# weiquan/salt

Measured on AMD Instinct MI355X. Metric: Mreads/s aligned (100 bp SE, GRCh38+snp144) at 1/2/4/8 MI355X vs CPU ref, higher is better.
Workload: dtype u32; 1 GPU; GRCh38-scale synthetic (SURVEY 8d config 3 = BASELINE configs[2]): 3100000000 bp genome in 24 contigs, 14800000 SNPs, k=21, 1000000 x 100 bp SE reads per GPU per step, 8 distinct resident batches rotated, inputs and results resident in HBM; read_len=100, distinct_batches=8, options=default (-s 50 -m 1000, overlap = k), streams_per_gpu=4

## Files before the change

include/salt_gpu.h:

```cpp
#ifndef SALT_GPU_H
#define SALT_GPU_H
#include <stdint.h>
#include <stddef.h>

#ifdef __cplusplus
extern "C" {
#endif

#define SALT_OK              0
#define SALT_E_INVAL        -1
#define SALT_E_HIP          -2
#define SALT_E_NOMEM        -3
#define SALT_E_INDEX        -4
#define SALT_E_CAPACITY     -5
#define SALT_E_DATA         -6

#define SALT_MAX_READ_LEN   512
#define SALT_MAX_HITS       5
#define SALT_MAX_LOCATE     1024
#define SALT_MAX_SEED_SLOTS 512
#define SALT_MAX_CIGAR_OPS  64

typedef struct {
    uint32_t c_primary, c_L2[5], c_seq_len, c_bwt_size;
// ... 80 lines not shown
int  salt_gpu_align_pe(salt_gpu_ws_t *ws, const salt_aln_opt_t *opt, const salt_pe_opt_t *pe, uint32_t n_pairs,
                       const uint8_t *seqs, const uint32_t *offs, salt_result_t *results);
int  salt_gpu_align_pe_resident(salt_gpu_ws_t *ws, const salt_aln_opt_t *opt, const salt_pe_opt_t *pe, uint32_t n_pairs,
                                uint32_t max_read_len, const void *d_seqs, const void *d_offs, void *d_results, void *hip_stream);
int  salt_gpu_ws_pe_overflow(salt_gpu_ws_t *ws, uint32_t *n);
int  salt_gpu_ws_pe_counts(salt_gpu_ws_t *ws, uint32_t out[8]);

int  salt_gpu_index_snp_enable(salt_gpu_index_t *ix, int on, uint32_t min_mapq);
int  salt_gpu_index_snp_sites(salt_gpu_index_t *ix, uint32_t *n_sites, uint32_t *pos, uint64_t cap);
int  salt_gpu_index_snp_counts(salt_gpu_index_t *ix, uint32_t *counts, uint64_t cap_words, int reset);
int  salt_gpu_ws_snp_uncount(salt_gpu_ws_t *ws);

typedef struct {
    uint32_t window;
    uint32_t tile_positions;
    int32_t  bgzf;
} salt_depth_text_opt_t;
int  salt_gpu_index_depth_enable(salt_gpu_index_t *ix, int on, uint32_t min_mapq);
int  salt_gpu_index_depth_reset(salt_gpu_index_t *ix);
int  salt_gpu_index_depth_fetch(salt_gpu_index_t *ix, uint64_t first, uint64_t n, uint32_t *out);
int  salt_gpu_index_depth_add(salt_gpu_index_t *ix, uint64_t first, uint64_t n, const uint32_t *in);
int  salt_gpu_index_depth_text_begin(salt_gpu_index_t *ix, const salt_depth_text_opt_t *opt);
int  salt_gpu_index_depth_text_next(salt_gpu_index_t *ix, const char **data, uint64_t *n_bytes);
int  salt_gpu_ws_depth_uncount(salt_gpu_ws_t *ws);

#define SALT_ERRPROF_Q      95
#define SALT_ERRPROF_CELLS  (2u * SALT_MAX_READ_LEN * SALT_ERRPROF_Q * 16u)
int  salt_gpu_index_errprof_enable(salt_gpu_index_t *ix, int on, uint32_t min_mapq);
int  salt_gpu_index_errprof_fetch(salt_gpu_index_t *ix, uint64_t *cells, uint64_t cap_cells, uint64_t rec[16], int reset);
int  salt_gpu_ws_errprof_uncount(salt_gpu_ws_t *ws);
int  salt_gpu_ws_set_quals(salt_gpu_ws_t *ws, const uint8_t *quals, int on_device);

typedef struct { int32_t print_xa_cigar, print_nm_md; const char *rg_id; } salt_text_opt_t;
int  salt_gpu_index_set_contigs(salt_gpu_index_t *ix, int32_t n, const int64_t *offsets, const char *const *names);
int  salt_gpu_align_pe_text(salt_gpu_ws_t *ws, const salt_aln_opt_t *opt, const salt_pe_opt_t *pe, const salt_text_opt_t *topt,
                            const char *fastq1, uint64_t n1_bytes, const char *fastq2, uint64_t n2_bytes,
                            const char **sam, uint64_t *sam_bytes, uint32_t *n_pairs);
int  salt_gpu_ws_reserve_text(salt_gpu_ws_t *ws, const salt_aln_opt_t *opt, uint64_t max_block_bytes, uint32_t est_reads, uint32_t max_read_len,
                              uint64_t est_sam_bytes, void *host_sam, uint64_t host_sam_bytes);
int  salt_gpu_align_se_text(salt_gpu_ws_t *ws, const salt_aln_opt_t *opt, const salt_text_opt_t *topt, const char *fastq, uint64_t n_bytes,
                            const char **sam, uint64_t *sam_bytes, uint32_t *n_reads);
int  salt_gpu_ws_set_sam_bgzf(salt_gpu_ws_t *ws, int on);
int  salt_gpu_ws_set_sam_bam(salt_gpu_ws_t *ws, int on);
int  salt_gpu_ws_set_polish(salt_gpu_ws_t *ws, int mode);
int  salt_gpu_bgzf_deflate(int device, const void *text, uint64_t n_bytes, void *out, uint64_t out_cap, uint64_t *out_bytes);
int  salt_gpu_bgzf_inflate(int device, const void *bgzf, uint64_t n_bytes, void *out, uint64_t out_cap, uint64_t *out_bytes);
int  salt_gpu_ws_inflate_bgzf(salt_gpu_ws_t *ws, const void *blocks, uint64_t n_cbytes, uint32_t n_blocks, const uint32_t *c_off, const uint32_t *u_off);
int  salt_gpu_ws_text_peek(salt_gpu_ws_t *ws, uint64_t off, uint64_t n, void *dst);
int  salt_gpu_align_se_text_dev(salt_gpu_ws_t *ws, const salt_aln_opt_t *opt, const salt_text_opt_t *topt, uint64_t off, uint64_t n_bytes, int add_newline,
                                const char **sam, uint64_t *sam_bytes, uint32_t *n_reads);
int  salt_gpu_host_alloc(uint64_t bytes, void **ptr);
void salt_gpu_host_free(void *ptr);
int  salt_gpu_device_numa_node(int device, int *node);
int  salt_gpu_device_count(int *n);

int  salt_gpu_align_se_resident(salt_gpu_ws_t *ws, const salt_aln_opt_t *opt, uint32_t n_reads,
                                uint32_t max_read_len, const void *d_seqs, const void *d_offs,
                                void *d_results, void *hip_stream);

#define SALT_N_KERNELS 10
int  salt_gpu_ws_timing(salt_gpu_ws_t *ws, int enable);
int  salt_gpu_ws_kernel_ms(salt_gpu_ws_t *ws, double ms[SALT_N_KERNELS], uint32_t *n_calls);

int  salt_gpu_ws_heavy_reads(salt_gpu_ws_t *ws, uint32_t *ids, uint32_t cap, uint32_t *n);

int  salt_gpu_buffer_alloc(int device, uint64_t bytes, void **dev_ptr);
int  salt_gpu_buffer_free(int device, void *dev_ptr);
int  salt_gpu_buffer_equal(int device, const void *a, const void *b, uint64_t bytes, int *equal);

int  salt_gpu_diag_rule(uint32_t n_cases, const uint32_t *pos, const uint8_t *val, const uint32_t *offs, const uint32_t *bound_in,
                        uint32_t L, uint32_t ref_len, int mode, uint32_t *out);

int  salt_gpu_diag_verify(const uint32_t *ref_words, uint32_t ref_len, uint32_t n_cases, const uint8_t *seqs, const uint32_t *offs,
                          const uint32_t *cand, const uint32_t *cand_offs, int mode, uint8_t *out);

int  salt_gpu_diag_occ(const salt_gpu_index_t *ix, int mode, uint32_t n, const uint32_t *queries, uint32_t *out);

int  salt_gpu_ws_queue_counts(salt_gpu_ws_t *ws, uint32_t out[8]);

int  salt_gpu_ws_counters(salt_gpu_ws_t *ws, uint64_t out[SALT_CTR_N]);

int  salt_gpu_diag_lv(const uint32_t *ref_words, uint32_t ref_len, uint32_t n_cases, const uint32_t *pos,
                      const uint32_t *kdiff, const uint8_t *seqs, const uint32_t *offs, int32_t *out4, uint16_t *cigars);

int  salt_gpu_diag_ssw(uint32_t n_cases, const uint8_t *aware, const uint8_t *ref_syms, const uint32_t *ref_offs,
                       const uint8_t *codes, const uint32_t *read_offs, int32_t *out6, uint16_t *cigars, uint16_t *n_cigar);

typedef struct { uint32_t read, offset, pool; uint16_t tlen; uint8_t strand, k; } salt_polish_item_t;
typedef struct salt_gpu_polish salt_gpu_polish_t;
int  salt_gpu_polish_open(int device, const uint8_t *pac, uint64_t l_pac, salt_gpu_polish_t **out);
void salt_gpu_polish_close(salt_gpu_polish_t *p);
int  salt_gpu_polish_lv(salt_gpu_polish_t *p, const uint8_t *codes, const uint32_t *offs, uint32_t n_reads, const salt_polish_item_t *items,
                        uint32_t n_items, const uint8_t *pool, uint32_t pool_stride, uint32_t n_pool, int want_cigar,
                        int32_t *dist, uint16_t *cigars, uint8_t *n_cigar);

int  salt_gpu_polish_sw(salt_gpu_polish_t *p, const uint8_t *codes, const uint32_t *offs, uint32_t n_reads, const salt_polish_item_t *items,
                        uint32_t n_items, int want_cigar, int32_t *score, int32_t *read_span, uint16_t *cigars, uint16_t *n_cigar);

int  salt_gpu_polish_set_contigs(salt_gpu_polish_t *p, int32_t n, const int64_t *offsets, const char *const *names);
typedef struct { int32_t paired, use_sw; } salt_polish_opt_t;
int  salt_gpu_polish_text(salt_gpu_polish_t *p, const salt_polish_opt_t *opt, const char *sam, uint64_t n_bytes,
                          const char **out, uint64_t *out_bytes, uint32_t *n_records, int *stopped);
int  salt_gpu_polish_text_stats(salt_gpu_polish_t *p, uint64_t out[8]);

int  salt_gpu_suffix_array(int device, const uint8_t *text, uint64_t n, int bits, uint32_t *sa_out);
uint64_t salt_gpu_idx_c_bwt_words(uint64_t n);
int  salt_gpu_idx_build_c(int device, const uint8_t *text, uint64_t n, uint32_t sa_intv, uint32_t *primary, uint32_t L2[5],
                          uint32_t *bwt, uint32_t *sa, uint32_t *lkt, uint32_t lkt_len);
int  salt_gpu_idx_build_r(int device, const uint8_t *rtext, uint64_t n, const uint32_t *sharp_off, const uint32_t *sharp_hdr, uint64_t n_sharp,
                          uint32_t cum4, uint32_t *inv_sa0, uint32_t *code, uint64_t code_words, uint32_t *rsa);
const char *salt_gpu_idx_last_error(void);

const char *salt_gpu_last_error(void);
uint32_t    salt_gpu_result_size(void);

#ifdef __cplusplus
}
#endif
#endif
```

salt_amd/csrc/salt_align.hip:

```cpp
#include <type_traits>
#include "salt_device.h"
#include "salt_kernels.h"

namespace salt {

#define WSYNC() do { __builtin_amdgcn_fence(__ATOMIC_ACQ_REL, "wavefront"); __builtin_amdgcn_wave_barrier(); \
                     __builtin_amdgcn_fence(__ATOMIC_ACQ_REL, "wavefront"); } while (0)

static constexpr int MAXL = SALT_MAX_READ_LEN;
static constexpr int SLOTS = SALT_MAX_SEED_SLOTS;
static constexpr int MAXLOC = SALT_MAX_LOCATE;
static constexpr int LVK = 31;
static_assert(offsetof(salt_result_t, strand) == 4 && offsetof(salt_result_t, mapq) == 7 && offsetof(salt_result_t, b0) == 8 &&
              offsetof(salt_result_t, b1) == 12 && offsetof(salt_result_t, seq_start) == 16 && offsetof(salt_result_t, seq_end) == 18 &&
              offsetof(salt_result_t, n_hits) == 20 && offsetof(salt_result_t, n_cigar) == 22 && offsetof(salt_result_t, skipped) == 23 &&
              offsetof(salt_result_t, hits) == 24 && sizeof(salt_hit_t) == 8, "salt_result_t header layout");
static constexpr int NHIT = 6;
__device__ __forceinline__ uint32_t mapq_quot(uint32_t x, uint32_t b0)
{
    const uint32_t v = 255u * x;
    return b0 == 1u ? v : b0 == 2u ? v / 2u : b0 == 3u ? v / 3u : v / b0;
}
static constexpr uint32_t INF = 255;

// ... 436 lines not shown
    if (pend_r) {
        uint4 *rec = wq + ((size_t)seg * wq_seg_cap + q_base[0] + at_r) * WQ_REC;
        rec[0] = make_uint4((uint32_t)item, pk_r, pl_r, cn0); rec[1] = make_uint4(cw0, cw1, cw2, cn1);
    }
    if (pend_c) {
        uint4 *rec = wq + (((size_t)WQ_SEG + seg) * wq_seg_cap + q_base[1] + at_c) * WQ_REC;
        rec[0] = make_uint4((uint32_t)item, pk_c, pl_c, cn0); rec[1] = make_uint4(cw0, cw1, cw2, cn1);
    }
    if (ctr) {
        for (int o = 32; o > 0; o >>= 1) {
            n_lkt += __shfl_down(n_lkt, o); n_occ_c += __shfl_down(n_occ_c, o); n_occ_r += __shfl_down(n_occ_r, o);
        }
        if (lane_id() == 0) {
            atomicAdd(ctr + SALT_CTR_LKT, n_lkt & 1023u); atomicAdd(ctr + SALT_CTR_OCC_C, n_occ_c); atomicAdd(ctr + SALT_CTR_OCC_R, n_occ_r);
            atomicAdd(ctr + SALT_CTR_D_WLKT, n_lkt & 1023u); atomicAdd(ctr + SALT_CTR_D_COCC_SEED, n_occ_c); atomicAdd(ctr + SALT_CTR_D_ROCC_SEED, n_occ_r);
            atomicAdd(ctr + SALT_CTR_D_SA_SEED, (n_lkt >> 10) & 2047u); atomicAdd(ctr + SALT_CTR_D_TEXT_SEED, n_lkt >> 21);
        }
    }
}

__global__ void __launch_bounds__(256) __attribute__((amdgpu_waves_per_eu(4, 4)))
k_seed_walk(IndexView ix, SeedParams sp, const uint32_t *__restrict__ tb, uint4 *__restrict__ sai_c, uint4 *__restrict__ sai_r,
            const uint4 *__restrict__ wq, const uint32_t *__restrict__ wq_cnt, uint32_t wq_seg_cap, uint32_t r_first, unsigned long long *__restrict__ ctr)
{
    const uint32_t seg = blockIdx.x & (WQ_SEG - 1u);
    const uint32_t wv = (blockIdx.x / WQ_SEG) * 4u + (uint32_t)__builtin_amdgcn_readfirstlane((int)(threadIdx.x >> 6)), nw = (gridDim.x / WQ_SEG) * 4u;
    const uint64_t lt = (1ull << lane_id()) - 1ull;
    const uint32_t la = r_first ? 0u : 1u, lb = la ^ 1u;
    const uint32_t na = wq_cnt[(la * WQ_SEG + seg) * WQ_STRIDE], nb = wq_cnt[(lb * WQ_SEG + seg) * WQ_STRIDE];
    const uint32_t a0 = (uint32_t)((uint64_t)na * wv / nw), a1 = (uint32_t)((uint64_t)na * (wv + 1u) / nw);
    const uint32_t b0 = (uint32_t)((uint64_t)nb * wv / nw), b1 = (uint32_t)((uint64_t)nb * (wv + 1u) / nw);
    const uint4 *qa = wq + (((size_t)la * WQ_SEG + seg) * wq_seg_cap + a0) * WQ_REC, *qb = wq + (((size_t)lb * WQ_SEG + seg) * wq_seg_cap + b0) * WQ_REC;
    const uint32_t tot_a = a1 - a0, tot = tot_a + (b1 - b0);
    const int i_top = (int)((uint32_t)sp.l_seed - ix.r_lkt_len) - 1;
    uint32_t n_aux = 0, n_sa = 0, n_text = 0, n_occ_c = 0, n_occ_r = 0;
    Walk w; w.ph = WK_IDLE; w.k = w.l = w.ext = w.p0 = 0; w.i = 0;
    SeedCtx c = seed_ctx_geom(sp, tb, 0, ix.r_lkt_len);
    uint32_t item = 0, cur = 0;
    bool is_r = false;
    const uint4 *qp = qa;
    for (;;) {
        const uint64_t idle = __ballot(w.ph == WK_IDLE);
        if (cur >= tot && idle == ~0ull) break;
        if (cur < tot) {
            const uint32_t t = cur + (uint32_t)__popcll(idle & lt);
            if (w.ph == WK_IDLE && t < tot) {
                const bool in_a = t < tot_a;
                qp = in_a ? qa + (size_t)t * WQ_REC : qb + (size_t)(t - tot_a) * WQ_REC; is_r = (in_a ? la : lb) == 0u; w.ph = WK_REC;
            }
            const uint32_t nx = cur + (uint32_t)__popcll(idle);
            cur = nx < tot ? nx : tot;
        }
        WalkReq q = walk_req_none();
        if (w.ph == WK_REC) { q.pa = qp; q.na = WQ_REC; }
        else if (w.ph != WK_IDLE) q = is_r ? seed_walk_issue<true>(ix, sp, c, w) : seed_walk_issue<false>(ix, sp, c, w);
        const WalkLoads ld = walk_fetch(q);
        bool done = false;
        uint4 row = make_uint4(1, 0, 0, 0);
        if (w.ph == WK_REC) {
            item = ld.a[0].x;
            c = seed_ctx_geom(sp, tb, item, ix.r_lkt_len);
            c.w0 = ld.a[1].x; c.w1 = ld.a[1].y; c.w2 = ld.a[1].z; c.n0 = ld.a[0].w; c.n1 = ld.a[1].w;
            done = is_r ? seed_walk_begin<true>(sp, c, ld.a[0].y, ld.a[0].z, i_top, w, row) : seed_walk_begin<false>(sp, c, ld.a[0].y, ld.a[0].z, i_top, w, row);
        } else if (w.ph != WK_IDLE) {
            done = is_r ? seed_walk_finish<true>(ix, sp, c, w, ld, row, n_occ_r, n_aux) : seed_walk_finish<false>(ix, sp, c, w, ld, row, n_occ_c, n_aux);
        }
        if (done && row.x <= row.y) { if (is_r) { row.w = sai_r_pack(sp.epoch, row.w); sai_r[item] = row; } else sai_c[item] = row; }
        n_sa += (n_aux >> 10) & 2047u; n_text += n_aux >> 21; n_aux = 0;
    }
    if (ctr) {
        for (int o = 32; o > 0; o >>= 1) { n_sa += __shfl_down(n_sa, o); n_text += __shfl_down(n_text, o); n_occ_c += __shfl_down(n_occ_c, o); n_occ_r += __shfl_down(n_occ_r, o); }
        if (lane_id() == 0) {
            atomicAdd(ctr + SALT_CTR_OCC_C, n_occ_c); atomicAdd(ctr + SALT_CTR_OCC_R, n_occ_r);
            atomicAdd(ctr + SALT_CTR_D_COCC_SEED, n_occ_c); atomicAdd(ctr + SALT_CTR_D_ROCC_SEED, n_occ_r);
            atomicAdd(ctr + SALT_CTR_D_SA_SEED, n_sa); atomicAdd(ctr + SALT_CTR_D_TEXT_SEED, n_text);
        }
    }
}

template <int NS> struct SaiListsT { uint32_t sp[2][NS], ep[2][NS], off[2][NS]; };
struct SaiLists { uint32_t *sp[2], *ep[2], *off[2]; };
template <int NS> __device__ __forceinline__ SaiLists sai_ref(SaiListsT<NS> &a) { return SaiLists{ { a.sp[0], a.sp[1] }, { a.ep[0], a.ep[1] }, { a.off[0], a.off[1] } }; }
struct LvTables { short L[LVK][64]; char A[LVK][64]; };
static constexpr int LLV_K = 12;
static constexpr int LLV_TW = 22;
static constexpr int LLV_N = 64;
static constexpr int LLV_WIN = 4;
static constexpr int LLV_TS = LLV_TW + 2;
static constexpr int LLV_PW = LLV_TW;
static_assert(((8 * (LLV_TW - 1) - LLV_WIN + LLV_K) >> 3) + 2 <= LLV_TS, "text words of the longest window at the widest bound");
static_assert(((8 * (LLV_TW - 1) - LLV_WIN) >> 3) + 2 <= LLV_PW, "pattern words of the longest read");
struct LaneLv { uint32_t T[LLV_TS * LLV_N]; uint32_t P[LLV_PW]; };
struct LvBytes { uint8_t T[MAXL + 4 + 64]; uint8_t P[MAXL + 64]; };
template <int NS, bool LLV>
struct WaveLdsT {
    static constexpr bool HAS_LLV = LLV;
    static constexpr int N_SLOTS = NS;
    uint32_t pm[2][MAXL / 8];
    union U { SaiListsT<NS> sai; typename std::conditional<LLV, LaneLv, uint32_t>::type llv; LvBytes lvb; } u;
    uint8_t  cand_e[MAXLOC];
    uint32_t loci[MAXLOC];
    uint32_t hit_pos[2][NHIT];
    uint8_t  hit_nd[2][NHIT], hit_gap[2][NHIT];
    uint16_t cig[SALT_MAX_CIGAR_OPS];
    int      n_cig;
    alignas(8) uint8_t cargs[128];
};
typedef WaveLdsT<SLOTS, true> WaveLds;
typedef WaveLdsT<32, false> WaveLdsSmall;
typedef WaveLdsT<1, false> WaveLdsCigar;

struct Sai { uint32_t sp, ep, off; };
__device__ __forceinline__ Sai sai_get(const SaiLists &s, int w, int i) { return Sai{ s.sp[w][i], s.ep[w][i], s.off[w][i] }; }
__device__ __forceinline__ void sai_set(SaiLists &s, int w, int i, Sai v) { s.sp[w][i] = v.sp; s.ep[w][i] = v.ep; s.off[w][i] = v.off; }
__device__ __forceinline__ bool sai_ltv(Sai a, Sai b) { return a.ep - a.sp < b.ep - b.sp; }
__device__ __forceinline__ bool sai_lt(const SaiLists &s, int w, int i, int j) { return sai_ltv(sai_get(s, w, i), sai_get(s, w, j)); }
__device__ __forceinline__ void sai_swap(SaiLists &s, int w, int i, int j) { Sai a = sai_get(s, w, i), b = sai_get(s, w, j); sai_set(s, w, i, b); sai_set(s, w, j, a); }

__device__ void sai_insertsort(SaiLists &s, int w, int lo, int hi)
{
    for (int i = lo + 1; i < hi; ++i)
        for (int j = i; j > lo && sai_lt(s, w, j, j - 1); --j) sai_swap(s, w, j, j - 1);
}

__device__ void sai_combsort(SaiLists &s, int w, int base, int n)
{
    const double shrink = 1.2473309501039786540366528676643;
    int gap = n; bool do_swap;
    do {
        if (gap > 2) { gap = (int)(gap / shrink); if (gap == 9 || gap == 10) gap = 11; }
        do_swap = false;
        for (int i = 0; i < n - gap; ++i)
            if (sai_lt(s, w, base + i + gap, base + i)) { sai_swap(s, w, base + i, base + i + gap); do_swap = true; }
    } while (do_swap || gap > 2);
    if (gap != 1) sai_insertsort(s, w, base, base + n);
}

__device__ __attribute__((noinline)) void sai_introsort(SaiLists &s, int w, int n)
{
    if (n < 1) return;
    if (n == 2) { if (sai_lt(s, w, 1, 0)) sai_swap(s, w, 0, 1); return; }
    int d; for (d = 2; (1 << d) < n; ++d) { }
    d <<= 1;
    int st_l[24], st_r[24], st_d[24], top = 0;
    int lo = 0, hi = n - 1;
    for (;;) {
        if (lo < hi) {
            if (--d == 0) { sai_combsort(s, w, lo, hi - lo + 1); hi = lo; continue; }
            int i = lo, j = hi, k = i + ((j - i) >> 1) + 1;
            if (sai_lt(s, w, k, i)) { if (sai_lt(s, w, k, j)) k = j; }
            else k = sai_lt(s, w, j, i) ? i : j;
            Sai rp = sai_get(s, w, k);
            if (k != hi) sai_swap(s, w, k, hi);
            for (;;) {
                do ++i; while (sai_ltv(sai_get(s, w, i), rp));
                do --j; while (i <= j && sai_ltv(rp, sai_get(s, w, j)));
                if (j <= i) break;
                sai_swap(s, w, i, j);
            }
            sai_swap(s, w, i, hi);
            if (i - lo > hi - i) {
                if (i - lo > 16 && top < 24) { st_l[top] = lo; st_r[top] = i - 1; st_d[top] = d; ++top; }
                lo = hi - i > 16 ? i + 1 : hi;
            } else {
                if (hi - i > 16 && top < 24) { st_l[top] = i + 1; st_r[top] = hi; st_d[top] = d; ++top; }
                hi = i - lo > 16 ? i - 1 : lo;
            }
        } else {
            if (top == 0) { sai_insertsort(s, w, 0, n); return; }
            --top; lo = st_l[top]; hi = st_r[top]; d = st_d[top];
        }
    }
}

__device__ void sort_loci(uint32_t *a, uint32_t n)
{
// ... 313 lines not shown
                if (k == q) c = b + bit;
                mm &= mm - 1;
            }
            m = mm;
            const bool act = c != 0xFFFFFFFFu;
            uint32_t pos = act ? cand[c] : 0u;
            if (pos >= ref_len) pos = 0xFFFFFFFFu;
            u32x4_a4 x = { 0u, 0u, 0u, 0u };
            if (act && need && pos != 0xFFFFFFFFu) x = *reinterpret_cast<const u32x4_a4 *>(ref + (pos >> 3) + 4 * sub);
            const uint32_t mism = quad_mismatch<8>(x, pos, pmw, nvalid);
            if (act && sub == 0) out[c] = (uint8_t)((mism > 3 || pos == 0xFFFFFFFFu) ? INF : mism);
        }
    }
}

__device__ __forceinline__ uint32_t popc(uint32_t m) { return (uint32_t)__popc(m); }
__device__ __forceinline__ uint32_t popc(uint64_t m) { return (uint32_t)__popcll(m); }
__device__ __forceinline__ int first_bit(uint32_t m) { return __ffs((int)m) - 1; }
__device__ __forceinline__ int first_bit(uint64_t m) { return __ffsll((long long)m) - 1; }
template <int GW> struct LaneGroup {
    static_assert(GW == 64 || GW == 32 || GW == 16, "a wave, half of one or a quarter");
    typedef std::conditional_t<GW == 64, uint64_t, uint32_t> mask_t;
    static __device__ __forceinline__ uint32_t lane() { return lane_id() & (uint32_t)(GW - 1); }
    static __device__ __forceinline__ mask_t ballot(bool x)
    {
        const uint64_t m = __ballot(x);
        if constexpr (GW == 64) return m;
        else {
            const uint32_t h = (lane_id() & 32u) ? (uint32_t)(m >> 32) : (uint32_t)m;
            if constexpr (GW == 32) return h; else return (h >> (lane_id() & 16u)) & 0xFFFFu;
        }
    }
    static __device__ __forceinline__ uint32_t bcast(uint32_t v, int src)
    {
        if constexpr (GW == 64) return (uint32_t)__builtin_amdgcn_readlane((int)v, src);
        else return (uint32_t)__shfl((int)v, (int)(lane_id() & (uint32_t)(64 - GW)) + src);
    }
    static __device__ __forceinline__ mask_t below() { return ((mask_t)1 << lane()) - (mask_t)1; }
    static __device__ __forceinline__ uint32_t sum(uint32_t v)
    {
        for (int o = GW / 2; o > 0; o >>= 1) v += (uint32_t)__shfl_xor((int)v, o);
        return v;
    }
};

template <int LN = 4, int GW = 64>
__device__ __forceinline__ void verify_quads_2(const uint32_t *__restrict__ ref, uint32_t ref_len, const uint32_t *pm0, const uint32_t *pm1, uint32_t L,
                                               const uint32_t *c0, uint32_t n0, const uint32_t *c1, uint32_t n1, uint8_t *o0, uint8_t *o1)
{
    constexpr uint32_t CPW = (uint32_t)GW / LN;
    const uint32_t lane = LaneGroup<GW>::lane(), sub = lane & (uint32_t)(LN - 1), q = lane / (uint32_t)LN;
    const uint32_t nw = (L + 7) >> 3, n = n0 + n1;
    const uint32_t nvalid = L > 32u * sub ? (L - 32u * sub < 32u ? L - 32u * sub : 32u) : 0u;
    const bool behind = LN == 8 && GW == 32 && !(4u * sub < nw + 1u);
    uint32_t pa[4], pb[4];
#pragma unroll
    for (int t = 0; t < 4; ++t) { const bool in = (4 * sub + t) < nw; pa[t] = in ? pm0[4 * sub + t] : 0u; pb[t] = in ? pm1[4 * sub + t] : 0u; }
    for (uint32_t b = 0; b < n; b += 4u * CPW) {
        uint32_t pos[4]; u32x4_a4 x[4]; bool act[4], rev[4];
#pragma unroll
        for (int g = 0; g < 4; ++g) {
            if (b + CPW * g >= n) break;
            const uint32_t c = b + CPW * g + q;
            act[g] = c < n; rev[g] = c >= n0;
            pos[g] = act[g] ? (rev[g] ? c1[c - n0] : c0[c]) : 0u;
            if (pos[g] >= ref_len) pos[g] = 0xFFFFFFFFu;
            if (behind) x[g] = u32x4_a4{ 0u, 0u, 0u, 0u };
            else x[g] = *reinterpret_cast<const u32x4_a4 *>(ref + ((pos[g] == 0xFFFFFFFFu ? 0u : pos[g]) >> 3) + 4 * sub);
        }
#pragma unroll
        for (int g = 0; g < 4; ++g) {
            if (b + CPW * g >= n) break;
            const uint32_t pw[4] = { rev[g] ? pb[0] : pa[0], rev[g] ? pb[1] : pa[1], rev[g] ? pb[2] : pa[2], rev[g] ? pb[3] : pa[3] };
            const uint32_t mism = quad_mismatch<LN>(x[g], pos[g], pw, nvalid);
            if (act[g] && sub == 0) {
                const uint32_t c = b + CPW * g + q;
                const uint8_t v = (uint8_t)((mism > 3 || pos[g] == 0xFFFFFFFFu) ? INF : mism);
                if (rev[g]) o1[c - n0] = v; else o0[c] = v;
            }
        }
    }
}

__device__ __attribute__((noinline)) int lv_wave(const uint8_t *T, int tlen, const uint8_t *P, int plen, int k, LvTables *tab, int &d_fin)
{
    const int lane = (int)lane_id();
    const int d = lane - 31;
    const int ad = d < 0 ? -d : d;
    int Lprev = -2;
    const int end0 = plen < tlen ? plen : tlen;
    if (d == 0) { int i = 0; while (i < end0 && (P[i] & T[i]) != 0) ++i; Lprev = i; }
    const int r0 = __shfl(Lprev, 31);
    if (tab) tab->L[0][lane] = (short)Lprev;
    d_fin = 0;
    if (r0 == end0) return plen > end0 ? plen - end0 : 0;
    if (k > LVK - 1) k = LVK - 1;
    for (int e = 1; e <= k; ++e) {
        int left = __shfl_up(Lprev, 1), right = __shfl_down(Lprev, 1);
        if (lane == 0) left = -2;
        if (lane == 63) right = -2;
        const bool active = ad <= e && ad <= LVK - 1;
        int best = Lprev + 1; char act = 'X';
        if (left > best) { best = left; act = 'D'; }
        if (right + 1 > best) { best = right + 1; act = 'I'; }
        int cur = -2;
        if (active) {
            if (P[best] == T[d + best]) {
                int end = plen < tlen - d ? plen : tlen - d;
                if (best >= end) best = end;
                else { int i = best; while (i < end && (P[i] & T[d + i]) != 0) ++i; best = i; }
            }
            cur = best;
        }
        if (tab) { tab->L[e][lane] = (short)cur; tab->A[e][lane] = act; }
        uint64_t reach = __ballot(active && cur == plen);
        if (reach) {
            if (tab) {
                int rank = d == 0 ? 0 : (d < 0 ? 2 * ad - 1 : 2 * ad);
                int my = (active && cur == plen) ? rank : 1000;
                for (int o = 32; o > 0; o >>= 1) { int t = __shfl_xor(my, o); my = t < my ? t : my; }
                d_fin = my == 0 ? 0 : ((my & 1) ? -((my + 1) >> 1) : (my >> 1));
            }
            return e;
        }
        Lprev = cur;
    }
    return -1;
}

__device__ __attribute__((noinline)) uint32_t lv_lanes(LaneLv &s, const uint32_t *pm, int plen, int tlen, int k, bool active)
{
    constexpr int LLV_W = 2 * LLV_K + 1;
    const int lane = (int)lane_id() & (LLV_N - 1);
    const lds_u32 T = as_lds(s.T) + lane, P = as_lds(pm);
    auto fetch = [&](int i, int t, uint32_t &p, uint32_t &x) {
        const lds_u32 pp = P + (i >> 3), tt = T + (t >> 3) * LLV_N;
        const uint32_t p0 = pp[0], p1 = pp[1], t0 = tt[0], t1 = tt[LLV_N];
        p = __funnelshift_r(p0, p1, 4u * (uint32_t)(i & 7));
        x = __funnelshift_r(t0, t1, 4u * (uint32_t)(t & 7));
    };
    auto run_of = [](uint32_t p, uint32_t x) -> int {
        const uint32_t y = p & x;
        const uint32_t z = ~(((y & 0x77777777u) + 0x77777777u) | y) & 0x88888888u;
        return z ? __builtin_ctz(z) >> 2 : 8;
    };
    auto reach = [&](int d, int best, bool gated) -> int {
        uint32_t p, x;
        fetch(best, d + best, p, x);
        const int end = plen < tlen - d ? plen : tlen - d;
        const bool open = !gated || ((p ^ x) & 15u) == 0;
        int run = run_of(p, x), i = best + run;
        if (open && run == 8) while (i < end) { fetch(i, d + i, p, x); run = run_of(p, x); i += run; if (run < 8) break; }
        i = i < end ? i : end;
        return open ? i : best;
    };
    int row[LLV_W];
#pragma unroll
    for (int j = 0; j < LLV_W; ++j) row[j] = -2;
    const int end0 = plen < tlen ? plen : tlen;
    uint32_t result = 255;
    bool done = !active;
    if (active) {
        const int i = reach(0, 0, false);
        row[LLV_K] = i;
        if (i == end0) { result = (uint32_t)(plen > end0 ? plen - end0 : 0); done = true; }
    }
    for (int e = 1; e <= k; ++e) {
        if (__ballot(!done) == 0) break;
        int carry = -2;
#pragma unroll
        for (int d = -LLV_K; d <= LLV_K; ++d) {
            if ((d < 0 ? -d : d) > e) continue;
            const int mid = row[d + LLV_K], right = d < LLV_K ? row[d + LLV_K + 1] : -2;
            int best = mid + 1;
            if (carry > best) best = carry;
            if (right + 1 > best) best = right + 1;
            carry = mid;
            if (!done) {
                best = reach(d, best, true);
                if (best == plen) { result = (uint32_t)e; done = true; }
                else row[d + LLV_K] = best;
            }
        }
    }
    return result;
}

template <int VMAX, bool GAPF>
__device__ __forceinline__ void rule_unsorted(const uint32_t *pos, const uint8_t *val, const uint32_t n, const uint32_t L, const uint32_t ref_len,
                                              uint32_t &bound, bool &any, uint32_t &best_pos, uint32_t &best_v,
                                              uint32_t &n_hits, uint32_t &a0, uint32_t *hit_pos, uint8_t *hit_nd)
{
    const uint32_t lane = lane_id();
    const uint32_t NONE = 0xFFFFFFFFu;
    auto in_range = [&](uint32_t p) -> bool { return GAPF ? !(p + L + 4 >= ref_len) : p < ref_len; };
    uint32_t mp[VMAX + 1];
#pragma unroll
    for (int t = 0; t <= VMAX; ++t) mp[t] = NONE;
    uint32_t my_p = 0, my_v = NONE, n_p = 0;
    for (uint32_t b = 0; b < n; b += 64) {
        const uint32_t i = b + lane;
        uint32_t p = 0, v = NONE;
        if (i < n) { p = pos[i]; v = val[i]; }
        const bool in = i < n && v <= bound && in_range(p);
        if (in) {
#pragma unroll
            for (int t = 0; t <= VMAX; ++t) if (v == (uint32_t)t && p < mp[t]) mp[t] = p;
        }
        uint64_t m = __ballot(in);
        if (m && n_p <= 64u) {
            if (n_p + (uint32_t)__popcll(m) > 64u) n_p = 65u;
            else
                while (m) {
                    const int l = __ffsll((long long)m) - 1;
                    const uint32_t pl = (uint32_t)__builtin_amdgcn_readlane((int)p, l), vl = (uint32_t)__builtin_amdgcn_readlane((int)v, l);
                    if (lane == n_p) { my_p = pl; my_v = vl; }
                    ++n_p; m &= m - 1;
                }
        }
    }
#pragma unroll
    for (int t = 0; t <= VMAX; ++t)
        for (int o = 32; o > 0; o >>= 1) { const uint32_t x = (uint32_t)__shfl_xor((int)mp[t], o); mp[t] = x < mp[t] ? x : mp[t]; }
    uint32_t before[VMAX + 1];
    before[0] = NONE;
#pragma unroll
    for (int t = 1; t <= VMAX; ++t) before[t] = mp[t - 1] < before[t - 1] ? mp[t - 1] : before[t - 1];
    any = false; n_hits = 0;
#pragma unroll
    for (int t = VMAX; t >= 0; --t) if (mp[t] != NONE) { any = true; best_v = (uint32_t)t; best_pos = mp[t]; }
    if (!any) return;
    unsigned long long last = 0;
    const bool in_lanes = n_p <= 64u;
    unsigned long long my_key = ~0ull;
    if (in_lanes && lane < n_p) {
        uint32_t lim = NONE;
#pragma unroll
        for (int t = 1; t <= VMAX; ++t) if (my_v == (uint32_t)t) lim = before[t];
        if (my_p < lim) my_key = ((unsigned long long)my_p << 8) | my_v;
    }
    for (uint32_t h = 0; h < (uint32_t)NHIT; ++h) {
        unsigned long long cur = ~0ull;
        if (in_lanes) { if (h == 0 || my_key > last) cur = my_key; }
        else
        for (uint32_t b = 0; b < n; b += 64) {
            const uint32_t i = b + lane;
            if (i < n) {
                const uint32_t p = pos[i], v = val[i];
                if (v <= bound && in_range(p)) {
                    uint32_t lim = NONE;
#pragma unroll
                    for (int t = 1; t <= VMAX; ++t) if (v == (uint32_t)t) lim = before[t];
                    const unsigned long long key = ((unsigned long long)p << 8) | v;
                    if (p < lim && (h == 0 || key > last) && key < cur) cur = key;
                }
            }
        }
        for (int o = 32; o > 0; o >>= 1) {
            const unsigned long long x = ((unsigned long long)(uint32_t)__shfl_xor((int)(cur >> 32), o) << 32) | (uint32_t)__shfl_xor((int)(uint32_t)cur, o);
            cur = x < cur ? x : cur;
        }
        if (cur == ~0ull) break;
        if (lane == 0) { hit_pos[h] = (uint32_t)(cur >> 8); hit_nd[h] = (uint8_t)(cur & 255u); }
        if (h == 0) a0 = (uint32_t)(cur & 255u);
        last = cur; ++n_hits;
    }
    bound = best_v < bound ? best_v : bound;
}

template <int VMAX, bool GAPF, int GW = 64>
__device__ __forceinline__ void rule_sparse(const uint32_t *pos, const uint8_t *val, const uint32_t n, const uint32_t L, const uint32_t ref_len,
                                            uint32_t &bound, bool &any, uint32_t &best_pos, uint32_t &best_v,
                                            uint32_t &n_hits, uint32_t &a0, uint32_t *hit_pos, uint8_t *hit_nd)
{
    typedef LaneGroup<GW> G;
    typedef typename G::mask_t mask_t;
    const uint32_t lane = G::lane();
    const uint32_t NONE = 0xFFFFFFFFu;
    auto in_range = [&](uint32_t p) -> bool { return GAPF ? !(p + L + 4 >= ref_len) : p < ref_len; };
    any = false; n_hits = 0;
    if (n == 0) return;
    if (n <= (uint32_t)GW) {
        uint32_t p = 0, v = NONE;
        if (lane < n) { p = pos[lane]; v = val[lane]; }
        const bool ok = v <= bound && in_range(p);
        const mask_t m = G::ballot(ok);
        if (m == 0) return;
        const int l0 = first_bit(m);
        const uint32_t p0 = G::bcast(p, l0);
        if (G::ballot(ok && p != p0) == 0) {
            const uint32_t v0 = G::bcast(v, l0);
            any = true; best_pos = p0; best_v = v0; n_hits = 1; a0 = v0;
            if (lane == 0) { hit_pos[0] = p0; hit_nd[0] = (uint8_t)v0; }
            bound = v0 < bound ? v0 : bound;
            return;
        }
    }
    uint32_t mp[VMAX + 1];
#pragma unroll
    for (int t = 0; t <= VMAX; ++t) mp[t] = NONE;
    for (uint32_t b = 0; b < n; b += GW) {
        const uint32_t i = b + lane;
        uint32_t p = 0, v = NONE;
        if (i < n) { p = pos[i]; v = val[i]; }
        mask_t m = G::ballot(v <= bound && in_range(p));
        while (m) {
            const int l = first_bit(m);
            const uint32_t pl = G::bcast(p, l), vl = G::bcast(v, l);
#pragma unroll
            for (int t = 0; t <= VMAX; ++t) if (vl == (uint32_t)t && pl < mp[t]) mp[t] = pl;
            m &= m - 1;
        }
    }
    uint32_t before[VMAX + 1];
    before[0] = NONE;
#pragma unroll
    for (int t = 1; t <= VMAX; ++t) before[t] = mp[t - 1] < before[t - 1] ? mp[t - 1] : before[t - 1];
#pragma unroll
    for (int t = VMAX; t >= 0; --t) if (mp[t] != NONE) { any = true; best_v = (uint32_t)t; best_pos = mp[t]; }
    if (!any) return;
    uint32_t last_p = 0;
    for (uint32_t h = 0; h < (uint32_t)NHIT; ++h) {
        uint32_t cur_p = NONE, cur_v = 0;
        for (uint32_t b = 0; b < n; b += GW) {
            const uint32_t i = b + lane;
            uint32_t p = 0, v = NONE;
            if (i < n) { p = pos[i]; v = val[i]; }
            uint32_t lim = NONE;
#pragma unroll
            for (int t = 1; t <= VMAX; ++t) if (v == (uint32_t)t) lim = before[t];
            mask_t m = G::ballot(v <= bound && in_range(p) && p < lim && (h == 0 || p > last_p));
            while (m) {
                const int l = first_bit(m);
                const uint32_t pl = G::bcast(p, l);
                if (pl < cur_p) { cur_p = pl; cur_v = G::bcast(v, l); }
                m &= m - 1;
            }
        }
        if (cur_p == NONE) break;
        if (lane == 0) { hit_pos[h] = cur_p; hit_nd[h] = (uint8_t)cur_v; }
        if (h == 0) a0 = cur_v;
        last_p = cur_p; ++n_hits;
    }
    bound = best_v < bound ? best_v : bound;
}

template <class W>
__device__ void lv_unpack(const uint32_t *ref_generic, W &w, int strand, uint32_t L, uint32_t pos)
{
    const gp_u32 ref = as_global(ref_generic);
    const uint32_t tlen = L + 4;
    for (uint32_t i = lane_id(); i < tlen + 48; i += 64) {
        uint32_t p = pos + i;
        w.u.lvb.T[i] = i < tlen ? (uint8_t)((ref[p >> 3] >> (4 * (p & 7u))) & 15u) : (uint8_t)0;
    }
    for (uint32_t i = lane_id(); i < L + 48; i += 64) {
        w.u.lvb.P[i] = i < L ? (uint8_t)((w.pm[strand][i >> 3] >> (4 * (i & 7u))) & 15u) : (uint8_t)0;
    }
    WSYNC();
}

template <class W>
__device__ __attribute__((noinline)) void lv_cigar(const uint32_t *ref, W &w, LvTables *tabp, int strand, uint32_t L, uint32_t pos, int k)
{
    LvTables &tab = *tabp;
    lv_unpack(ref, w, strand, L, pos);
    int d_fin = 0;
    WSYNC();
    int e = lv_wave(w.u.lvb.T, (int)L + 4, w.u.lvb.P, (int)L, k, &tab, d_fin);
    __threadfence_block();
    WSYNC();
    if (lane_id() == 0) {
        int n = 0;
        uint16_t *cg = w.cig;
        if (e == 0) { cg[n++] = (uint16_t)((L << 4) | 0u); }
        else if (e > 0) {
            char act[LVK + 1]; int matched[LVK + 1];
            int cd = d_fin;
            for (int ce = e; ce >= 1; --ce) {
                char a = tab.A[ce][cd + 31];
                act[ce] = a;
                int cur = tab.L[ce][cd + 31];
                if (a == 'I') { matched[ce] = cur - tab.L[ce - 1][cd + 1 + 31] - 1; cd += 1; }
                else if (a == 'D') { matched[ce] = cur - tab.L[ce - 1][cd - 1 + 31]; cd -= 1; }
                else { matched[ce] = cur - tab.L[ce - 1][cd + 31] - 1; }
            }
            int acc = tab.L[0][31];
            int ce = 1;
            while (ce <= e) {
                char a = act[ce]; int cnt = 1;
                while (ce + 1 <= e && matched[ce] == 0 && act[ce + 1] == a) { ++cnt; ++ce; }
                if (a == 'X') acc += cnt;
                else {
                    if (acc != 0 && n < SALT_MAX_CIGAR_OPS) { cg[n++] = (uint16_t)((acc << 4) | 0); }
                    acc = 0;
                    if (n < SALT_MAX_CIGAR_OPS) cg[n++] = (uint16_t)((cnt << 4) | (a == 'I' ? 1 : 2));
                }
                if (matched[ce] > 0) acc += matched[ce];
                ++ce;
            }
            if (acc != 0 && n < SALT_MAX_CIGAR_OPS) cg[n++] = (uint16_t)((acc << 4) | 0);
        }
        w.n_cig = n;
    }
    WSYNC();
}

__device__ __forceinline__ void lane_text(const uint32_t *__restrict__ ref, uint32_t *T, uint32_t pos, uint32_t tl)
{
    const uint32_t w0 = pos >> 3, sh = (pos & 7u) * 4u, nwt = (tl + 7) >> 3, nst = ((tl - LLV_WIN + LLV_K) >> 3) + 2;
    uint32_t wv[LLV_TW + 1];
#pragma unroll
    for (int j = 0; j <= LLV_TW; ++j) wv[j] = (uint32_t)j <= nwt ? ref[w0 + (uint32_t)j] : 0u;
#pragma unroll
    for (int j = 0; j < LLV_TW; ++j) {
        uint32_t word = 0;
        if ((uint32_t)j < nwt) {
            word = __funnelshift_r(wv[j], wv[j + 1], sh);
            const uint32_t rem = tl - (uint32_t)j * 8;
            if (rem < 8) word &= (1u << (4 * rem)) - 1u;
        }
        if ((uint32_t)j < nst) T[j * LLV_N] = word;
    }
#pragma unroll
    for (int j = LLV_TW; j < LLV_TS; ++j) if ((uint32_t)j < nst) T[j * LLV_N] = 0u;
}
template <class F>
__device__ __forceinline__ void lane_pattern(uint32_t *P, uint32_t nw, uint32_t first, uint32_t step, F word)
{
    for (uint32_t j = first; j < (uint32_t)LLV_PW; j += step) P[j] = j < nw ? word(j) : 0u;
}

__device__ __forceinline__ uint32_t store_gap_list(const uint32_t *loci, uint32_t n, uint32_t L, uint32_t ref_len, uint32_t *__restrict__ dst)
{
    const uint32_t lane = lane_id();
    const uint64_t lt = (1ull << lane) - 1ull;
    uint32_t n_out = 0;
    for (uint32_t b = 0; b < n; b += 64) {
        const uint32_t i = b + lane;
        const uint32_t pos = i < n ? loci[i] : 0u;
        const bool keep = i < n && !(pos + L + 4 >= ref_len);
        const uint64_t m = __ballot(keep);
        if (keep) dst[n_out + (uint32_t)__popcll(m & lt)] = pos;
        n_out += (uint32_t)__popcll(m);
    }
    return n_out;
}

template <bool PE, bool GL, class W>
__device__ __forceinline__ void align_general(const IndexView ix, const AlignParams ap, W &w, const uint32_t r,
                              const uint32_t *__restrict__ pm,
                              const uint4 *__restrict__ sai_c, const uint4 *__restrict__ sai_r,
                              salt_result_t *__restrict__ results, unsigned long long *__restrict__ ctr,
                              unsigned long long *phase, LvTables *lvtab, const GapBufs g, uint32_t *pe_loci, uint8_t *pe_cand)
{
    const uint32_t lane = lane_id();
    const uint64_t lt = (1ull << lane) - 1ull;
    const uint32_t *rec = pm + (uint64_t)r * ap.pg.pm_stride;
    const uint32_t L = rec[2 * ap.pg.nw8];
    salt_result_t *out = results + r;
    uint32_t c_sa_c = 0, c_sa_r = 0, c_verify = 0, c_vwords = 0, c_lv = 0, c_loci = 0, c_ctx_rej = 0, c_ctx_rows = 0;
    PhaseClock pc(phase);
    const uint64_t rt0 = phase ? __builtin_amdgcn_s_memrealtime() : 0;
    constexpr bool glob = GL;
    uint32_t *loci = glob ? pe_loci : w.loci;
    uint8_t *cand_e = glob ? pe_cand : w.cand_e;
    const uint32_t loci_cap = PE ? PE_LOCI_CAP : (uint32_t)MAXLOC;

    const uint32_t nw = (L + 7) >> 3;
    uint32_t n_amb = 0;
    for (uint32_t t = lane; t < 2 * nw; t += 64) {
        const uint32_t s = t >= nw, j = s ? t - nw : t;
        const uint32_t word = rec[s * ap.pg.nw8 + j];
        w.pm[s][j] = word;
        if (!s) n_amb += (uint32_t)__popc(word & (word >> 1) & (word >> 2) & (word >> 3) & 0x11111111u);
    }
    if (ap.max_amb < L) { for (int o = 32; o > 0; o >>= 1) n_amb += (uint32_t)__shfl_xor((int)n_amb, o); }
    else n_amb = 0;
    WSYNC();
    uint32_t q_pos = 0xFFFFFFFFu; uint32_t q_strand = 3, q_ndiff = 255, q_gap = 255;
    const bool too_short = L < (uint32_t)ap.l_seed;
    if (n_amb > ap.max_amb) {
        if (lane == 0) {
            out->pos = q_pos; out->strand = 3; out->n_diff = 255; out->is_gap = 255; out->mapq = 0;
            out->b0 = -1; out->b1 = -1; out->seq_start = 0; out->seq_end = (uint16_t)(L - 1);
            out->n_hits[0] = out->n_hits[1] = 0; out->n_cigar = 0; out->skipped = 1;
        }
        return;
// ... 56 lines not shown
                    if (strand == 0 || ix.c_ctx != nullptr) {
                        WSYNC();
                        const CandStats cs = build_candidates_call<PE, GL>(CandArgs{ ix.c_sa, ix.r_pos, sai_c, sai_r, ix.ref_len, ap.spr, ap.max_locate, r, L, strand, true, phase, pe_loci, loci_cap, ap.pe, false, ap.epoch, nullptr, nullptr, 0 }, w);
                        if (glob) { loci = cs.in_lds ? w.loci : pe_loci; cand_e = cs.in_lds ? w.cand_e : pe_cand; }
                        c_sa_c += cs.n_sa_c; c_sa_r += cs.n_sa_r; c_loci += cs.n_loci;
                        n = cs.n_cand;
                    }
                    if (n > 1024u * LLV_N) { ok = false; break; }
                    uint32_t o = 0;
                    if (lane == 0) o = atomicAdd(&g.gctl->pool_used, n);
                    o = (uint32_t)__shfl((int)o, 0);
                    ok = (uint64_t)o + n <= g.pool;
                    if (ok) for (uint32_t i = lane; i < n; i += 64) g.gloci[o + i] = loci[i];
                    ns[strand] = n; off[strand] = o;
                }
                const uint32_t ch0 = ok ? (ns[0] + LLV_N - 1) / LLV_N : 0, ch1 = ok ? (ns[1] + LLV_N - 1) / LLV_N : 0;
                uint32_t base = 0;
                if (ok && lane == 0) base = atomicAdd(&g.gctl->gap_items, ch0 + ch1);
                base = (uint32_t)__shfl((int)base, 0);
                ok = ok && (uint64_t)base + ch0 + ch1 <= g.items_cap;
                if (lane == 0) {
                    g.gq[slot] = ok ? r : 0xFFFFFFFFu;
                    g.gn[2 * slot] = ok ? ns[0] : 0; g.gn[2 * slot + 1] = ok ? ns[1] : 0;
                    g.goff[2 * slot] = off[0]; g.goff[2 * slot + 1] = off[1];
                }
                if (ok) {
                    for (uint32_t c = lane; c < ch0 + ch1; c += 64) g.gitems[base + c] = (slot << 11) | (c >= ch0 ? (0x400u | (c - ch0)) : c);
                    if (ctr) {
                        for (int o2 = 32; o2 > 0; o2 >>= 1) c_vwords += __shfl_down(c_vwords, o2);
                        if (lane == 0) {
                            atomicAdd(ctr + SALT_CTR_SA_C, c_sa_c); atomicAdd(ctr + SALT_CTR_SA_R, c_sa_r);
                            atomicAdd(ctr + SALT_CTR_VERIFY, c_verify); atomicAdd(ctr + SALT_CTR_VERIFY_WORDS, c_vwords);
                            atomicAdd(ctr + SALT_CTR_LV, ns[0] + ns[1]); atomicAdd(ctr + SALT_CTR_READS, 1ull);
                            atomicAdd(ctr + SALT_CTR_BASES, L); atomicAdd(ctr + SALT_CTR_LOCI, c_loci);
                            atomicAdd(ctr + SALT_CTR_D_SA_HEAVY, c_sa_c + c_sa_r);
                            atomicAdd(ctr + SALT_CTR_D_VERIFY_HEAVY, c_verify * (L <= 248 ? 4u : (((L + 7) >> 3) + 4u) / 4u));
                            atomicAdd(ctr + SALT_CTR_D_OUT_HEAVY, 5u * (ns[0] + ns[1]) + 16u);
                            if (ix.c_ctx) { atomicAdd(ctr + SALT_CTR_D_CTX_ROWS, c_ctx_rows); atomicAdd(ctr + SALT_CTR_D_CTX_REJECTED, c_ctx_rej); }
                        }
                    }
                    return;
                }
                WSYNC();
            }
        }
        if constexpr (!W::HAS_LLV) {
            if (lanes_fit && n_cand_nogap > 0) {
                if (lane == 0) g.ovq[atomicAdd(&g.gctl->ovq_count, 1u)] = r;
                return;
            }
        }
        for (int strand = 0; strand < 2; ++strand) {
            pc.stamp(SALT_CTR_T_GAP);
            const CandStats cs = build_candidates_call<PE, GL>(CandArgs{ ix.c_sa, ix.r_pos, sai_c, sai_r, ix.ref_len, ap.spr, ap.max_locate, r, L, strand, true, phase, pe_loci, loci_cap, ap.pe, true, ap.epoch, nullptr, nullptr, 0 }, w);
            if (glob) { loci = cs.in_lds ? w.loci : pe_loci; cand_e = cs.in_lds ? w.cand_e : pe_cand; }
            pc.t = phase ? __builtin_amdgcn_s_memtime() : 0;
            const uint32_t n_cand = cs.n_cand; c_sa_c += cs.n_sa_c; c_sa_r += cs.n_sa_r; c_loci += cs.n_loci;
            bool any = false;
            const bool lanes_ok = lanes_fit && W::HAS_LLV;
            if constexpr (W::HAS_LLV) if (lanes_ok) {
                const int k0 = gap_k0;
                WSYNC();
                lane_pattern(w.u.llv.P, (L + 7) >> 3, lane, 64u, [&](uint32_t j) { return w.pm[strand][j]; });
                for (uint32_t b = 0; b < n_cand; b += LLV_N) {
                    WSYNC();
                    const uint32_t i = b + lane;
                    bool act = false;
                    if (lane < LLV_N && i < n_cand) {
                        const uint32_t pos = loci[i];
                        act = !(pos > ix.ref_len || pos + L + 4 > ix.ref_len);
                        if (act) lane_text(ix.ref, w.u.llv.T + lane, pos, L + 4);
                    }
                    const uint32_t e = lv_lanes(w.u.llv, w.u.llv.P, (int)L, (int)L + 4, k0, act);
                    if (lane < LLV_N && i < n_cand) cand_e[i] = (uint8_t)e;
                }
                WSYNC();
            }
            for (uint32_t i = 0; i < n_cand; ++i) {
                uint32_t pos = loci[i];
                int e = -1;
                if (lanes_ok) { const uint32_t ev = cand_e[i]; e = (ev != 255 && (int)ev <= maxd) ? (int)ev : -1; }
                else if (!(pos > ix.ref_len || pos + L + 4 > ix.ref_len)) {
                    lv_unpack(ix.ref, w, strand, L, pos);
                    int dd;
                    e = lv_wave(w.u.lvb.T, (int)L + 4, w.u.lvb.P, (int)L, maxd, nullptr, dd);
                    WSYNC();
                }
                ++c_lv;
                if (e >= 0) {
                    if (e < maxd || !any) { maxd = e; q_gap = 1; q_ndiff = (uint32_t)e; q_strand = (uint32_t)strand; q_pos = pos; }
                    if (n_hits_s[strand] < NHIT && lane == 0) {
                        uint32_t h = n_hits_s[strand];
                        w.hit_pos[strand][h] = pos; w.hit_nd[strand][h] = (uint8_t)e; w.hit_gap[strand][h] = 1;
                    }
                    if (n_hits_s[strand] == 0) a0[strand] = (uint32_t)e;
                    if (n_hits_s[strand] < NHIT) ++n_hits_s[strand];
                    any = true;
                }
            }
            found[strand] = any;
            WSYNC();
        }
    }
    WSYNC();
    pc.stamp(SALT_CTR_T_GAP);

    int b0 = (int)q_ndiff, b1 = 100000, tot = 0;
    uint32_t nh[2] = { 0, 0 };
    uint32_t sel_idx[2][SALT_MAX_HITS];
    for (int s = 0; s < 2 && tot < ap.max_hits; ++s) {
        for (uint32_t j = 0; j < n_hits_s[s]; ++j) {
            uint32_t p = w.hit_pos[s][j];
            if (p == 0xFFFFFFFFu || p == q_pos) continue;
            if (a0[s] <= q_ndiff) {
                if ((int)a0[s] <= b1) b1 = (int)a0[s];
                if (nh[s] < SALT_MAX_HITS) sel_idx[s][nh[s]] = j;
                ++nh[s]; ++tot;
            }
            if (tot == ap.max_hits) break;
        }
    }
    uint32_t mapq = 0;
    if (b0 != 0) {
        uint32_t x = (uint32_t)(b0 > b1 ? b0 - b1 : b1 - b0);
        uint64_t q = mapq_quot(x, (uint32_t)b0);
        mapq = q < 254 ? (uint32_t)q : 254u;
    }
    if (lane == 0) {
        out->pos = q_pos; out->strand = (uint8_t)q_strand; out->n_diff = (uint8_t)q_ndiff; out->is_gap = (uint8_t)q_gap;
        out->mapq = (uint8_t)mapq; out->b0 = b0; out->b1 = b1; out->seq_start = 0; out->seq_end = (uint16_t)(L - 1);
        out->n_hits[0] = (uint8_t)nh[0]; out->n_hits[1] = (uint8_t)nh[1]; out->skipped = 0;
        for (int s = 0; s < 2; ++s)
            for (uint32_t j = 0; j < nh[s]; ++j) {
                uint32_t h = sel_idx[s][j];
                out->hits[s][j].pos = w.hit_pos[s][h]; out->hits[s][j].n_diff = w.hit_nd[s][h];
                out->hits[s][j].is_gap = w.hit_gap[s][h]; out->hits[s][j].strand = (uint16_t)s;
            }
    }
    if (q_pos != 0xFFFFFFFFu) {
        if (q_gap) {
            lv_cigar(ix.ref, w, lvtab, (int)q_strand, L, q_pos, (int)q_ndiff);
            if (lane < (uint32_t)w.n_cig) out->cigar[lane] = w.cig[lane];
            if (lane == 0) out->n_cigar = (uint8_t)w.n_cig;
        } else if (lane == 0) { out->cigar[0] = (uint16_t)((L << 4) | 0u); out->n_cigar = 1; }
    } else if (lane == 0) out->n_cigar = 0;
    uint32_t hidx = 0;
    for (int s = 0; s < 2; ++s)
        for (uint32_t j = 0; j < nh[s]; ++j, ++hidx) {
            uint32_t h = sel_idx[s][j];
            if (w.hit_gap[s][h]) {
                WSYNC();
                lv_cigar(ix.ref, w, lvtab, s, L, w.hit_pos[s][h], (int)w.hit_nd[s][h]);
                if (lane < (uint32_t)w.n_cig) out->hit_cigar[hidx][lane] = w.cig[lane];
                if (lane == 0) out->hit_n_cigar[hidx] = (uint8_t)w.n_cig;
            } else if (lane == 0) out->hit_n_cigar[hidx] = 0;
        }

    pc.stamp(SALT_CTR_T_TAIL);
    if (phase) {
        const unsigned long long dt = (unsigned long long)(__builtin_amdgcn_s_memrealtime() - rt0);
        pc.add(SALT_CTR_X3, dt);
        if (ctr && lane == 0) atomicMax(ctr + SALT_CTR_MAX_HEAVY, (dt << 32) | r);
    }
    if (ctr) {
        for (int o = 32; o > 0; o >>= 1) c_vwords += __shfl_down(c_vwords, o);
        if (lane == 0) {
            atomicAdd(ctr + SALT_CTR_SA_C, c_sa_c); atomicAdd(ctr + SALT_CTR_SA_R, c_sa_r);
            atomicAdd(ctr + SALT_CTR_VERIFY, c_verify); atomicAdd(ctr + SALT_CTR_VERIFY_WORDS, c_vwords);
            atomicAdd(ctr + SALT_CTR_LV, c_lv); atomicAdd(ctr + SALT_CTR_READS, 1ull);
            atomicAdd(ctr + SALT_CTR_BASES, L); atomicAdd(ctr + SALT_CTR_LOCI, c_loci);
            atomicAdd(ctr + SALT_CTR_D_SA_HEAVY, c_sa_c + c_sa_r);
            atomicAdd(ctr + SALT_CTR_D_VERIFY_HEAVY, c_verify * (L <= 248 ? 4u : (((L + 7) >> 3) + 4u) / 4u));
            atomicAdd(ctr + SALT_CTR_D_OUT_HEAVY, 128u);
            if (ix.c_ctx) { atomicAdd(ctr + SALT_CTR_D_CTX_ROWS, c_ctx_rows); atomicAdd(ctr + SALT_CTR_D_CTX_REJECTED, c_ctx_rej); }
        }
    }
}

__device__ __forceinline__ uint32_t pop_ranged(QueueRange *ranges, const uint32_t which, const uint32_t n_items, uint32_t &seg, uint32_t &tried)
{
    while (tried < QUEUE_RANGES) {
        const uint32_t lo = (uint32_t)((uint64_t)n_items * seg / QUEUE_RANGES), hi = (uint32_t)((uint64_t)n_items * (seg + 1u) / QUEUE_RANGES);
        uint32_t *h = &ranges[seg].heads[which];
        if (lo < hi && __hip_atomic_load(h, __ATOMIC_RELAXED, __HIP_MEMORY_SCOPE_AGENT) < hi - lo) {
            const uint32_t k = atomicAdd(h, 1u);
            if (k < hi - lo) return lo + k;
        }
        seg = (seg + 1u) & (QUEUE_RANGES - 1u); ++tried;
    }
    return 0xFFFFFFFFu;
}
template <bool PE, bool GL, class W>
__device__ __forceinline__ void heavy_body(const IndexView &ix, const AlignParams &ap, const uint32_t *__restrict__ pm,
                                           const uint4 *__restrict__ sai_c, const uint4 *__restrict__ sai_r,
                                           salt_result_t *__restrict__ results, const uint32_t *__restrict__ queue,
                                           unsigned long long *__restrict__ ctr, LvTables *__restrict__ lvtab, const GapBufs g,
                                           uint8_t *__restrict__ pe_scr, const int overflow_pass)
{
    __shared__ W w;
    __shared__ uint32_t s_item;
    __shared__ unsigned long long s_phase[SALT_CTR_N];
    unsigned long long *phase = ctr ? s_phase : nullptr;
    if (ctr) { for (int i = threadIdx.x; i < SALT_CTR_N; i += 64) s_phase[i] = 0; }
    WSYNC();
    const uint32_t n_items = overflow_pass ? g.gctl->ovq_count : ap.all_heavy ? ap.n_reads : g.gctl->light_queued;
    uint32_t seg = blockIdx.x & (QUEUE_RANGES - 1u), tried = 0;
    for (;;) {
        if (threadIdx.x == 0) {
            uint32_t got = 0xFFFFFFFFu;
            if (overflow_pass) { got = atomicAdd(&g.gctl->ovq_head, 1u); if (got >= n_items) got = 0xFFFFFFFFu; }
            else got = pop_ranged(g.ranges, QueueRange::HEAVY, n_items, seg, tried);
            s_item = got;
        }
        WSYNC();
        const uint32_t it = s_item;
        WSYNC();
        if (it == 0xFFFFFFFFu) break;
        const uint32_t r = overflow_pass ? g.ovq[it] : ap.all_heavy ? it : queue[it];
        align_general<PE, GL>(ix, ap, w, r, pm, sai_c, sai_r, results, ctr, phase, lvtab + blockIdx.x, g,
                          pe_scr ? reinterpret_cast<uint32_t *>(pe_scr + (size_t)blockIdx.x * PE_LOCI_CAP * 5) : nullptr,
                          pe_scr ? pe_scr + (size_t)blockIdx.x * PE_LOCI_CAP * 5 + (size_t)PE_LOCI_CAP * 4 : nullptr);
        if (phase && threadIdx.x == 0) s_phase[SALT_CTR_HEAVY_READS] += 1;
        WSYNC();
    }
    if (phase) {
        WSYNC();
        for (int i = SALT_CTR_T_LOAD + (int)threadIdx.x; i < SALT_CTR_N; i += 64) if (s_phase[i]) atomicAdd(ctr + i, s_phase[i]);
    }
}

#ifndef SALT_HEAVY_WAVES
#define SALT_HEAVY_WAVES 4
#endif
#if SALT_HEAVY_WAVES > 0
#define HEAVY_OCC __attribute__((amdgpu_waves_per_eu(SALT_HEAVY_WAVES, SALT_HEAVY_WAVES)))
#else
#define HEAVY_OCC
#endif
#define HEAVY_KERNEL(NAME, PE, GL, LDS)                                                                                    \
__global__ void __launch_bounds__(64) HEAVY_OCC                                                                         \
NAME(IndexView ix, AlignParams ap, const uint32_t *__restrict__ pm,                                                     \
     const uint4 *__restrict__ sai_c, const uint4 *__restrict__ sai_r, salt_result_t *__restrict__ results,             \
     const uint32_t *__restrict__ queue, unsigned long long *__restrict__ ctr,                                          \
     LvTables *__restrict__ lvtab, GapBufs g, uint8_t *__restrict__ pe_scr, int overflow_pass)                          \
{ heavy_body<PE, GL, LDS>(ix, ap, pm, sai_c, sai_r, results, queue, ctr, lvtab, g, pe_scr, overflow_pass); }
HEAVY_KERNEL(k_heavy, false, false, WaveLdsSmall)
HEAVY_KERNEL(k_heavy_pe, true, true, WaveLdsSmall)
HEAVY_KERNEL(k_heavy_big, false, false, WaveLds)
HEAVY_KERNEL(k_heavy_pe_big, true, true, WaveLds)
HEAVY_KERNEL(k_heavy_glob, false, true, WaveLds)

__global__ void __launch_bounds__(64)
k_gap(IndexView ix, AlignParams ap, const uint32_t *__restrict__ pm, GapBufs g)
{
    __shared__ LaneLv s;
    __shared__ uint32_t s_item;
    const uint32_t lane = lane_id();
    const uint32_t n_items = g.gctl->gap_items < g.items_cap ? g.gctl->gap_items : g.items_cap;
    uint32_t seg = blockIdx.x & (QUEUE_RANGES - 1u), tried = 0;
    for (;;) {
        if (threadIdx.x == 0) s_item = pop_ranged(g.ranges, QueueRange::GAP, n_items, seg, tried);
        WSYNC();
        const uint32_t it = s_item;
        WSYNC();
        if (it == 0xFFFFFFFFu) break;
        const uint32_t item = g.gitems[it], slot = item >> 11, strand = (item >> 10) & 1u, chunk = item & 1023u;
        const uint32_t r = g.gq[slot];
        const uint32_t *rec = pm + (uint64_t)r * ap.pg.pm_stride;
        const uint32_t L = rec[2 * ap.pg.nw8], nw = (L + 7) >> 3;
        lane_pattern(s.P, nw, lane, 64u, [&](uint32_t j) { return rec[strand * ap.pg.nw8 + j]; });
        const uint32_t n = g.gn[2 * slot + strand], i = chunk * LLV_N + lane;
        const size_t row = g.goff[2 * slot + strand];
        bool act = false;
        if (lane < LLV_N && i < n) {
            const uint32_t pos = g.gloci[row + i];
            act = !(pos > ix.ref_len || pos + L + 4 > ix.ref_len);
            if (act) lane_text(ix.ref, s.T + lane, pos, L + 4);
        }
        WSYNC();
        const uint32_t e = lv_lanes(s, s.P, (int)L, (int)L + 4, ap.pe ? 3 : (int)(L / 10), act);
        if (lane < LLV_N && i < n) g.ge[row + i] = (uint8_t)e;
        WSYNC();
    }
}

struct FinLds { uint32_t hit_pos[2][NHIT]; uint8_t hit_nd[2][NHIT]; };
__global__ void __launch_bounds__(64)
k_gapfin(IndexView ix, AlignParams ap, const uint32_t *__restrict__ pm, salt_result_t *__restrict__ results, GapBufs g,
         unsigned long long *__restrict__ ctr)
{
    __shared__ FinLds w;
    __shared__ uint32_t s_item;
    const uint32_t lane = lane_id();
    const uint64_t lt = (1ull << lane) - 1ull;
    const uint32_t n_items = g.gctl->gap_slots < g.cap ? g.gctl->gap_slots : g.cap;
    uint32_t seg = blockIdx.x & (QUEUE_RANGES - 1u), tried = 0;
    for (;;) {
        if (threadIdx.x == 0) s_item = pop_ranged(g.ranges, QueueRange::GAPFIN, n_items, seg, tried);
        WSYNC();
        const uint32_t slot = s_item;
        WSYNC();
        if (slot == 0xFFFFFFFFu) break;
        const uint64_t rt0 = ctr ? __builtin_amdgcn_s_memrealtime() : 0;
        const uint32_t r = g.gq[slot];
        if (r == 0xFFFFFFFFu) continue;
        const uint32_t L = pm[(uint64_t)r * ap.pg.pm_stride + 2 * ap.pg.nw8];
        salt_result_t *out = results + r;
        uint32_t q_pos = 0xFFFFFFFFu, q_strand = 3, q_ndiff = 255, q_gap = 255;
        uint32_t bound = ap.pe ? 3u : L / 10;
        uint32_t n_hits_s[2] = { 0, 0 }, a0[2] = { 0, 0 };
        for (int strand = 0; strand < 2; ++strand) {
            const uint32_t n = g.gn[2 * slot + strand];
            const size_t row = g.goff[2 * slot + strand];
            bool any = false; uint32_t bp = 0, bv = 0;
            rule_unsorted<LLV_K, true>(g.gloci + row, g.ge + row, n, L, ix.ref_len, bound, any, bp, bv, n_hits_s[strand], a0[strand],
                                       w.hit_pos[strand], w.hit_nd[strand]);
            if (any) { q_pos = bp; q_ndiff = bv; q_gap = 1; q_strand = (uint32_t)strand; }
        }
        WSYNC();
        int b0 = (int)q_ndiff, b1 = 100000, tot = 0;
        uint32_t nh[2] = { 0, 0 };
        uint32_t sel_idx[2][SALT_MAX_HITS];
        for (int s = 0; s < 2 && tot < ap.max_hits; ++s)
            for (uint32_t j = 0; j < n_hits_s[s]; ++j) {
                const uint32_t p = w.hit_pos[s][j];
                if (p == 0xFFFFFFFFu || p == q_pos) continue;
                if (a0[s] <= q_ndiff) {
                    if ((int)a0[s] <= b1) b1 = (int)a0[s];
                    if (nh[s] < SALT_MAX_HITS) sel_idx[s][nh[s]] = j;
                    ++nh[s]; ++tot;
                }
                if (tot == ap.max_hits) break;
            }
        uint32_t mapq = 0;
        if (b0 != 0) {
            const uint32_t x = (uint32_t)(b0 > b1 ? b0 - b1 : b1 - b0);
            const uint64_t q = mapq_quot(x, (uint32_t)b0);
            mapq = q < 254 ? (uint32_t)q : 254u;
        }
        const uint32_t n_cig_items = q_pos != 0xFFFFFFFFu ? 1u + nh[0] + nh[1] : 0u;
        const uint32_t first_cig = ap.pe ? 1u : 0u;
        if (lane == 0) {
            out->pos = q_pos; out->strand = (uint8_t)q_strand; out->n_diff = (uint8_t)q_ndiff; out->is_gap = (uint8_t)q_gap;
            out->mapq = (uint8_t)mapq; out->b0 = b0; out->b1 = b1; out->seq_start = 0; out->seq_end = (uint16_t)(L - 1);
            out->n_hits[0] = (uint8_t)nh[0]; out->n_hits[1] = (uint8_t)nh[1]; out->skipped = 0; out->n_cigar = 0;
            for (int s = 0; s < 2; ++s)
                for (uint32_t j = 0; j < nh[s]; ++j) {
                    const uint32_t h = sel_idx[s][j];
                    out->hits[s][j].pos = w.hit_pos[s][h]; out->hits[s][j].n_diff = w.hit_nd[s][h];
                    out->hits[s][j].is_gap = 1; out->hits[s][j].strand = (uint16_t)s;
                }
            if (n_cig_items > first_cig) {
                const uint32_t base = atomicAdd(&g.gctl->cigar_items, n_cig_items - first_cig);
                for (uint32_t c = first_cig; c < n_cig_items; ++c) g.cq[base + c - first_cig] = (r << 3) | c;
            }
            if (ctr) atomicMax(ctr + SALT_CTR_MAX_GAPFIN, ((unsigned long long)(__builtin_amdgcn_s_memrealtime() - rt0) << 32) | r);
        }
        WSYNC();
    }
}

__global__ void __launch_bounds__(64)
k_cigar(IndexView ix, PackGeom pg, const uint32_t *__restrict__ pm, salt_result_t *__restrict__ results,
        const uint32_t *__restrict__ items, const uint32_t *__restrict__ count, uint32_t *__restrict__ head, uint32_t cap_items,
        LvTables *__restrict__ lvtab)
{
    __shared__ WaveLdsCigar w;
    __shared__ uint32_t s_item;
    const uint32_t lane = lane_id();
    const uint32_t n_items = *count < cap_items ? *count : cap_items;
    struct { PackGeom pg; } ap = { pg };
    bool first = true;
    for (;;) {
        if (threadIdx.x == 0) s_item = first ? blockIdx.x : sw_pull(head, 1u, gridDim.x, n_items);
        first = false;
        WSYNC();
        const uint32_t it = s_item;
        WSYNC();
        if (it >= n_items) break;
        const uint32_t item = items[it], which = item & 7u, r = item >> 3;
        salt_result_t *out = results + r;
        const uint32_t *rec = pm + (uint64_t)r * ap.pg.pm_stride;
        const uint32_t L = rec[2 * ap.pg.nw8];
        uint32_t strand, pos, k;
        if (which == 0) { strand = out->strand; pos = out->pos; k = out->n_diff; }
        else {
            const uint32_t h = which - 1, n0 = out->n_hits[0];
            strand = h >= n0; const uint32_t j = strand ? h - n0 : h;
            pos = out->hits[strand][j].pos; k = out->hits[strand][j].n_diff;
        }
        for (uint32_t t = lane; t < (L + 7) >> 3; t += 64) w.pm[strand][t] = rec[strand * ap.pg.nw8 + t];
        WSYNC();
        lv_cigar(ix.ref, w, lvtab + blockIdx.x, (int)strand, L, pos, (int)k);
        uint16_t *dst = which == 0 ? out->cigar : out->hit_cigar[which - 1];
        if (lane < (uint32_t)w.n_cig) dst[lane] = w.cig[lane];
        if (lane == 0) { if (which == 0) out->n_cigar = (uint8_t)w.n_cig; else out->hit_n_cigar[which - 1] = (uint8_t)w.n_cig; }
        WSYNC();
    }
}

__host__ __device__ __forceinline__ uint32_t qseg_cap(uint32_t n_reads) { return n_reads / QUEUE_RANGES + 8u; }
__device__ __forceinline__ void queue_push(uint32_t *__restrict__ qseg, QueueRange *__restrict__ ranges, uint32_t n_reads, uint32_t r)
{
    const uint32_t s = (r >> 2) & (QUEUE_RANGES - 1u);
    qseg[(size_t)s * qseg_cap(n_reads) + atomicAdd(&ranges[s].push, 1u)] = r;
}
__device__ __forceinline__ uint32_t *retry_segs(uint32_t *qseg, uint32_t n_reads) { return qseg + (size_t)QUEUE_RANGES * qseg_cap(n_reads); }
__device__ __forceinline__ void retry_push(uint32_t *__restrict__ qseg, QueueRange *__restrict__ ranges, uint32_t n_reads, uint32_t r)
{
    const uint32_t s = (r >> 2) & (QUEUE_RANGES - 1u);
    retry_segs(qseg, n_reads)[(size_t)s * qseg_cap(n_reads) + atomicAdd(&ranges[s].retry, 1u)] = r;
}
__global__ void __launch_bounds__(256)
k_queue_pack(const uint32_t *__restrict__ qseg, const QueueRange *__restrict__ ranges, uint32_t n_reads, uint32_t *__restrict__ queue, SeCtl *__restrict__ ctl)
{
    __shared__ uint32_t base_s, cnt_s;
    if (threadIdx.x == 0) {
        uint32_t base = 0, total = 0;
        for (uint32_t s = 0; s < QUEUE_RANGES; ++s) { const uint32_t c = ranges[s].push; if (s < blockIdx.x) base += c; total += c; }
        base_s = base; cnt_s = ranges[blockIdx.x].push;
        if (blockIdx.x == 0) ctl->light_queued = total;
    }
    __syncthreads();
    const uint32_t *src = qseg + (size_t)blockIdx.x * qseg_cap(n_reads);
    for (uint32_t i = threadIdx.x; i < cnt_s; i += 256) queue[base_s + i] = src[i];
}

static constexpr int LT_LOCI = 128;
static constexpr int LT_MAXL = 160;
static constexpr int L2_SLOTS = 8;
static constexpr int L4_SLOTS = 4;
#ifndef SALT_L4_ROWS
#define SALT_L4_ROWS 16
#endif
static constexpr int L4_ROWS = SALT_L4_ROWS;

template <int SLOTS, int PMW, int LOCI> struct LightRec {
    uint32_t pm[2][PMW];
    uint32_t sp[4][SLOTS], off[4][SLOTS];
    uint32_t pre[4][SLOTS + 1];
    uint32_t loci[2][LOCI];
    uint32_t hit_pos[2][NHIT];
    uint8_t  hit_nd[2][NHIT];
    uint8_t  val[2][LOCI];
};
template <int GW> using LightLds = LightRec<GW / 4, GW == 64 ? LT_MAXL / 8 : GW == 32 ? 32 : 16, GW == 16 ? 2 * L4_ROWS : LT_LOCI>;
static_assert(sizeof(LightLds<32>) == 1996 && 8 * sizeof(LightLds<16>) <= 4 * sizeof(LightLds<32>), "eight quarter records in the LDS of four half-wave ones");

template <int GW, int LN, bool INSTR>
__device__ __forceinline__ void light_read(const IndexView &ix, const AlignParams &ap, const uint32_t *__restrict__ pm,
                                           const uint4 *__restrict__ sai_c, const uint4 *__restrict__ sai_r, salt_result_t *__restrict__ results,
                                           uint32_t *__restrict__ queue , QueueRange *__restrict__ ranges,
                                           unsigned long long *__restrict__ ctr, LightLds<GW> &w, const uint32_t r)
{
    typedef LaneGroup<GW> G;
    typedef typename G::mask_t mask_t;
    constexpr uint32_t SLOTS = GW / 4, HALF = GW / 2;
    constexpr uint32_t LMAX = LN == 4 ? 120u : LN == 8 ? 248u : (uint32_t)LT_MAXL;
    static_assert(LMAX <= 8 * sizeof(w.pm[0]) / 4 && (LN != 0 || LMAX <= 248u), "the read fits the record and the window check");
    const uint32_t lane = G::lane();
    const mask_t lt = G::below();
    const uint32_t *rec = pm + (uint64_t)r * ap.pg.pm_stride;
    const uint32_t L = rec[2 * ap.pg.nw8];
    bool heavy = L > LMAX || L < (uint32_t)ap.l_seed || ap.spr > SLOTS || ap.max_locate < 2 * 64;
    uint32_t c_sa_c = 0, c_sa_r = 0, c_verify = 0, c_loci = 0;
    const bool prof = INSTR && ctr && (r & 127u) == 0;
    uint64_t tp = prof ? __builtin_amdgcn_s_memtime() : 0;
    auto stamp = [&](int slot) {
        if (!prof) return;
        const uint64_t n = __builtin_amdgcn_s_memtime();
        if (lane == 0) atomicAdd(ctr + slot, (unsigned long long)(n - tp));
        tp = n;
    };
    auto locate = [&](uint32_t l, uint32_t j, uint32_t of, uint32_t &p) -> bool {
        p = ((of >> 31) ? j : (l & 1) ? ix.r_pos[j] : ix.c_sa[j]) - (of & 0x7FFFFFFFu);
        return (l & 1) ? !(p > ix.ref_len || p + L > ix.ref_len) : !(p + L > ix.ref_len);
// ... 259 lines not shown
        if (m == rescued) continue;
        salt_result_t *q = res + 2 * p + m;
        const uint32_t L = pm[(uint64_t)(2 * p + m) * pg.pm_stride + 2 * pg.nw8];
        q->seq_start = 0; q->seq_end = (uint16_t)(L - 1);
        if (q->pos == 0xFFFFFFFFu) q->n_cigar = 0;
        else if (q->is_gap) { q->n_cigar = 0; citems[atomicAdd(ccount, 1u)] = ((2 * p + (uint32_t)m) << 3) | 0u; }
        else { q->cigar[0] = (uint16_t)((L << 4) | 0u); q->n_cigar = 1; }
    }
}

void launch_pe_final(const IndexView &ix, const PackGeom &pg, uint32_t n_pairs, const uint32_t *pm, salt_result_t *res, const PePair *pairs,
                     const PeSwRes *sw, void *lvtab, uint32_t *citems, PeCtl *ctl, uint32_t n_blocks, hipStream_t st)
{
    if (!n_pairs) return;
    hipLaunchKernelGGL(k_pe_final, dim3((n_pairs + 255) / 256), dim3(256), 0, st, pg, n_pairs, pm, res, pairs, sw, citems, &ctl->n_cigar);
    hipLaunchKernelGGL(k_cigar, dim3(n_blocks), dim3(64), 0, st, ix, pg, pm, res, citems, &ctl->n_cigar, &ctl->cigar_head, 2 * n_pairs, static_cast<LvTables *>(lvtab));
}

uint32_t seed_wq_seg_cap(uint64_t items) { return (uint32_t)(((items + 255) / 256 + WQ_SEG - 1) / WQ_SEG) * 256u; }
size_t seed_wq_words(uint64_t items) { return (size_t)2 * WQ_SEG * seed_wq_seg_cap(items) * WQ_REC * 4; }
uint32_t seed_wq_cnt_words() { return 2u * WQ_SEG * WQ_STRIDE; }
void launch_seed(const IndexView &ix, const SeedParams &sp, const uint32_t *tb, uint4 *sai_c, uint4 *sai_r, uint4 *wq, uint32_t *wq_cnt,
                 uint32_t walk_blocks, unsigned long long *ctr, hipStream_t st)
{
    uint64_t items = (uint64_t)sp.n_reads * 2u * sp.spr;
    if (!items) return;
    uint32_t blocks = (uint32_t)((items + 255) / 256);
    const uint32_t cap = seed_wq_seg_cap(items);
    hipLaunchKernelGGL(k_seed, dim3(blocks), dim3(256), 0, st, ix, sp, tb, sai_c, sai_r, wq, wq_cnt, cap, ctr);
    walk_blocks = (walk_blocks + WQ_SEG - 1) / WQ_SEG * WQ_SEG;
    static const uint32_t r_first = getenv("SALT_GPU_WALK_R_FIRST") && atoi(getenv("SALT_GPU_WALK_R_FIRST")) ? 1u : 0u;
    hipLaunchKernelGGL(k_seed_walk, dim3(walk_blocks), dim3(256), 0, st, ix, sp, tb, sai_c, sai_r, wq, wq_cnt, cap, r_first, ctr);
}

void launch_light(const IndexView &ix, const AlignParams &ap, const uint32_t *pm, const uint8_t *, const uint32_t *, const uint4 *sai_c,
                  const uint4 *sai_r, salt_result_t *results, uint32_t *queue, SeCtl *ctl, uint32_t *qseg, QueueRange *ranges, unsigned long long *ctr, hipStream_t st)
{
    if (!ap.n_reads) return;
    static const bool no_half = getenv("SALT_GPU_NO_LIGHT2") && atoi(getenv("SALT_GPU_NO_LIGHT2"));
    static const bool no_quarter = getenv("SALT_GPU_NO_LIGHT4") && atoi(getenv("SALT_GPU_NO_LIGHT4"));
    if (!no_half && !no_quarter && !ctr && !SALT_DIAG_VAL(ap.dbg_stop) && ap.spr <= (uint32_t)L4_SLOTS && ap.pg.nw8 <= 15) {
        static const int wv = getenv("SALT_GPU_L4_WAVES") ? atoi(getenv("SALT_GPU_L4_WAVES")) : 2;
        if (wv == 1) hipLaunchKernelGGL(k_light4<1>, dim3((ap.n_reads + 3) / 4), dim3(64), 0, st, ix, ap, pm, sai_c, sai_r, results, qseg, ranges);
        else if (wv == 4) hipLaunchKernelGGL(k_light4<4>, dim3((ap.n_reads + 15) / 16), dim3(256), 0, st, ix, ap, pm, sai_c, sai_r, results, qseg, ranges);
        else hipLaunchKernelGGL(k_light4<2>, dim3((ap.n_reads + 7) / 8), dim3(128), 0, st, ix, ap, pm, sai_c, sai_r, results, qseg, ranges);
        static const uint32_t retry_blocks = [] {
            int dev = 0, cus = 0, per_cu = getenv("SALT_GPU_L4_RETRY_PER_CU") ? atoi(getenv("SALT_GPU_L4_RETRY_PER_CU")) : 8;
            if (hipGetDevice(&dev) != hipSuccess || hipDeviceGetAttribute(&cus, hipDeviceAttributeMultiprocessorCount, dev) != hipSuccess || cus <= 0) cus = (int)QUEUE_RANGES;
            if (per_cu < 1 || per_cu > 64) per_cu = 8;
            return ((uint32_t)(cus * per_cu) + QUEUE_RANGES - 1u) / QUEUE_RANGES * QUEUE_RANGES;
        }();
        hipLaunchKernelGGL(k_light_retry, dim3(retry_blocks), dim3(128), 0, st, ix, ap, pm, sai_c, sai_r, results, qseg, ranges);
    } else if (!no_half && !ctr && !SALT_DIAG_VAL(ap.dbg_stop) && ap.spr <= (uint32_t)L2_SLOTS && ap.pg.nw8 <= 31) {
        static const int wv = getenv("SALT_GPU_L2_WAVES") ? atoi(getenv("SALT_GPU_L2_WAVES")) : 2;
        if (ap.pg.nw8 > 15) hipLaunchKernelGGL((k_light2<2, 8>), dim3((ap.n_reads + 3) / 4), dim3(128), 0, st, ix, ap, pm, sai_c, sai_r, results, qseg, ranges);
        else if (wv == 1) hipLaunchKernelGGL(k_light2<1>, dim3((ap.n_reads + 1) / 2), dim3(64), 0, st, ix, ap, pm, sai_c, sai_r, results, qseg, ranges);
        else hipLaunchKernelGGL(k_light2<2>, dim3((ap.n_reads + 3) / 4), dim3(128), 0, st, ix, ap, pm, sai_c, sai_r, results, qseg, ranges);
    } else
        hipLaunchKernelGGL(k_light, dim3((ap.n_reads + LT_WAVES - 1) / LT_WAVES), dim3(64 * LT_WAVES), 0, st, ix, ap, pm, sai_c, sai_r, results, qseg, ranges, ctr);
    hipLaunchKernelGGL(k_queue_pack, dim3(QUEUE_RANGES), dim3(256), 0, st, qseg, ranges, ap.n_reads, queue, ctl);
}
size_t queue_words(uint32_t max_reads) { return (size_t)max_reads * 2 + (size_t)2 * QUEUE_RANGES * qseg_cap(max_reads); }

__global__ void __launch_bounds__(64)
k_diag_rule(uint32_t n_cases, const uint32_t *__restrict__ pos, const uint8_t *__restrict__ val, const uint32_t *__restrict__ offs,
            const uint32_t *__restrict__ bound_in, uint32_t L, uint32_t ref_len, int mode, uint32_t *__restrict__ out)
{
    __shared__ uint32_t hit_pos_s[4][NHIT];
    __shared__ uint8_t hit_nd_s[4][NHIT];
    const uint32_t gw = mode == 3 ? 32u : mode == 4 ? 16u : 64u, half = lane_id() / gw, lane = lane_id() & (gw - 1u);
    const uint32_t c = (64u / gw) * blockIdx.x + half;
    if (c >= n_cases) return;
    uint32_t *hit_pos = hit_pos_s[half];
    uint8_t *hit_nd = hit_nd_s[half];
    const uint32_t o = offs[c], n = offs[c + 1] - o;
    uint32_t bound = bound_in[c], bp = 0, bv = 0, nh = 0, a0 = 0;
    bool any = false;
    if (lane < NHIT) { hit_pos[lane] = 0; hit_nd[lane] = 0; }
    WSYNC();
    if (mode == 0) rule_unsorted<3, false>(pos + o, val + o, n, L, ref_len, bound, any, bp, bv, nh, a0, hit_pos, hit_nd);
    else if (mode == 1) rule_sparse<3, false>(pos + o, val + o, n, L, ref_len, bound, any, bp, bv, nh, a0, hit_pos, hit_nd);
    else if (mode == 3) rule_sparse<3, false, 32>(pos + o, val + o, n, L, ref_len, bound, any, bp, bv, nh, a0, hit_pos, hit_nd);
    else if (mode == 4) rule_sparse<3, false, 16>(pos + o, val + o, n, L, ref_len, bound, any, bp, bv, nh, a0, hit_pos, hit_nd);
    else rule_unsorted<LLV_K, true>(pos + o, val + o, n, L, ref_len, bound, any, bp, bv, nh, a0, hit_pos, hit_nd);
    WSYNC();
    uint32_t *w = out + (size_t)c * (6 + 2 * NHIT);
    if (lane == 0) { w[0] = any; w[1] = any ? bp : 0; w[2] = any ? bv : 0; w[3] = nh; w[4] = nh ? a0 : 0; w[5] = bound; }
    if (lane < NHIT) { w[6 + 2 * lane] = lane < nh ? hit_pos[lane] : 0; w[7 + 2 * lane] = lane < nh ? hit_nd[lane] : 0; }
}

void launch_diag_rule(uint32_t n_cases, const uint32_t *pos, const uint8_t *val, const uint32_t *offs, const uint32_t *bound_in,
                      uint32_t L, uint32_t ref_len, int mode, uint32_t *out, hipStream_t st)
{
    const uint32_t blocks = mode == 3 ? (n_cases + 1) / 2 : mode == 4 ? (n_cases + 3) / 4 : n_cases;
    if (n_cases) hipLaunchKernelGGL(k_diag_rule, dim3(blocks), dim3(64), 0, st, n_cases, pos, val, offs, bound_in, L, ref_len, mode, out);
}
uint32_t diag_rule_words() { return 6 + 2 * NHIT; }

__host__ __device__ static inline bool lv_fit_dev(uint32_t L, uint32_t k) { return k <= (uint32_t)LLV_K && L + 4 <= 8u * (LLV_TW - 1); }
bool lv_lanes_fit(uint32_t L, uint32_t k) { return lv_fit_dev(L, k); }

__global__ void __launch_bounds__(64)
k_diag_lv(IndexView ix, uint32_t n_cases, const uint32_t *__restrict__ pos, const uint32_t *__restrict__ kdiff,
          const uint8_t *__restrict__ seqs, const uint32_t *__restrict__ offs, const uint32_t *__restrict__ lane_first,
          const uint32_t *__restrict__ lane_n, const uint32_t *__restrict__ lane_case, int32_t *__restrict__ out ,
          uint16_t *__restrict__ cig_out , LvTables *__restrict__ lvtab)
{
    __shared__ WaveLds w;
    __shared__ uint32_t lane_pm[LLV_N][LLV_PW];
    const uint32_t c = blockIdx.x, lane = lane_id();
    if (c >= n_cases) return;
    const uint32_t off = offs[c], L = offs[c + 1] - off, p = pos[c];
    const uint32_t nw = (L + 7) >> 3;
    auto pm_word = [&](uint32_t o, uint32_t j) -> uint32_t {
        uint32_t word = 0;
        for (uint32_t q = 0; q < 8; ++q) {
            uint32_t i = j * 8 + q, cc = i < L ? seqs[o + i] : 5u;
            word |= (cc < 4 ? (1u << cc) : (cc == 4 ? 15u : 0u)) << (4 * q);
        }
        return word;
    };
    for (uint32_t j = lane; j < nw; j += 64) w.pm[0][j] = pm_word(off, j);
    WSYNC();
    int32_t v = -2, e_wave = -1, n_cig = -2;
    if (p + L <= ix.ref_len) v = (int32_t)mismatch_capped(ix, w.pm[0], L, p);
    const bool in_range = !(p > ix.ref_len || p + L + 4 > ix.ref_len);
    const int k = (int)kdiff[c];
    if (in_range) {
        lv_unpack(ix.ref, w, 0, L, p);
        int dd;
        e_wave = lv_wave(w.u.lvb.T, (int)L + 4, w.u.lvb.P, (int)L, k, nullptr, dd);
        WSYNC();
    }
    const bool fit = lv_fit_dev(L, (uint32_t)k);
    const uint32_t gn = fit ? lane_n[c] : 0u;
    if (gn) {
        const uint32_t m = lane_case[lane_first[c] + lane % gn], mo = offs[m], mp = pos[m];
        lane_pattern(lane_pm[lane], nw, 0u, 1u, [&](uint32_t j) { return pm_word(mo, j); });
        const bool act = !(mp > ix.ref_len || mp + L + 4 > ix.ref_len);
        if (act) lane_text(ix.ref, w.u.llv.T + lane, mp, L + 4);
        WSYNC();
        const uint32_t el = lv_lanes(w.u.llv, lane_pm[lane], (int)L, (int)L + 4, k, act);
        if (lane < gn) out[(size_t)m * 4 + 2] = el == 255 ? -1 : (int32_t)el;
        WSYNC();
    }
    if (in_range && e_wave >= 0 && e_wave < LVK) {
        lv_cigar(ix.ref, w, lvtab + blockIdx.x, 0, L, p, e_wave);
        n_cig = w.n_cig;
        if (lane < (uint32_t)w.n_cig) cig_out[(size_t)c * SALT_MAX_CIGAR_OPS + lane] = w.cig[lane];
    }
    if (lane == 0) {
        out[(size_t)c * 4 + 0] = v; out[(size_t)c * 4 + 1] = e_wave; out[(size_t)c * 4 + 3] = n_cig;
        if (!fit) out[(size_t)c * 4 + 2] = -2;
    }
}

size_t lv_table_bytes() { return sizeof(LvTables); }

void launch_diag_lv(const IndexView &ix, uint32_t n, const uint32_t *pos, const uint32_t *kdiff, const uint8_t *seqs,
                    const uint32_t *offs, const uint32_t *lane_first, const uint32_t *lane_n, const uint32_t *lane_case,
                    int32_t *out, uint16_t *cig, void *lvtab, hipStream_t st)
{
    if (n) hipLaunchKernelGGL(k_diag_lv, dim3(n), dim3(64), 0, st, ix, n, pos, kdiff, seqs, offs, lane_first, lane_n, lane_case, out, cig,
                              static_cast<LvTables *>(lvtab));
}

__global__ void __launch_bounds__(64)
k_diag_verify(const uint32_t *__restrict__ ref, uint32_t ref_len, uint32_t n_cases, const uint8_t *__restrict__ seqs, const uint32_t *__restrict__ offs,
              const uint32_t *__restrict__ cand, const uint32_t *__restrict__ coffs, int mode, uint8_t *__restrict__ out)
{
    __shared__ uint32_t pm_s[4][64];
    __shared__ uint32_t loci_s[4][256];
    __shared__ uint8_t val_s[4][256];
    const uint32_t gw = mode == 7 ? 16u : mode >= 5 ? 32u : 64u, half = lane_id() / gw, lane = lane_id() & (gw - 1u);
    const uint32_t c = (64u / gw) * blockIdx.x + half;
    if (c >= n_cases) return;
    uint32_t *pm = pm_s[half], *loci = loci_s[half];
    uint8_t *val = val_s[half];
    const uint32_t off = offs[c], L = offs[c + 1] - off, c0 = coffs[c];
    uint32_t n = coffs[c + 1] - c0;
    if (n > 256) n = 256;
    const uint32_t nw = (L + 7) >> 3;
    for (uint32_t j = lane; j < 64; j += gw) {
        uint32_t word = 0;
        for (uint32_t q = 0; q < 8 && j < nw; ++q) {
            const uint32_t i = j * 8 + q, cc = i < L ? seqs[off + i] : 5u;
            word |= (cc < 4 ? (1u << cc) : (cc == 4 ? 15u : 0u)) << (4 * q);
        }
        pm[j] = word;
    }
    for (uint32_t i = lane; i < n; i += gw) { loci[i] = cand[c0 + i]; val[i] = 77; }
    WSYNC();
    IndexView ix; ix.ref = ref; ix.ref_len = ref_len;
    if (mode == 0) { for (uint32_t i = lane; i < n; i += 64) val[i] = (uint8_t)mismatch_capped(ix, pm, L, loci[i]); }
    else if (mode == 1) verify_quads<8>(ref, ref_len, pm, L, loci, n, val);
    else if (mode == 2) verify_quads<8, 8>(ref, ref_len, pm, L, loci, n, val);
    else if (mode == 3) verify_quads_2(ref, ref_len, pm, pm, L, loci, n / 2, loci + n / 2, n - n / 2, val, val + n / 2);
    else if (mode == 4) verify_quads_2<8>(ref, ref_len, pm, pm, L, loci, n / 2, loci + n / 2, n - n / 2, val, val + n / 2);
    else if (mode == 5) verify_quads_2<4, 32>(ref, ref_len, pm, pm, L, loci, n / 2, loci + n / 2, n - n / 2, val, val + n / 2);
    else if (mode == 6) verify_quads_2<8, 32>(ref, ref_len, pm, pm, L, loci, n / 2, loci + n / 2, n - n / 2, val, val + n / 2);
    else verify_quads_2<4, 16>(ref, ref_len, pm, pm, L, loci, n / 2, loci + n / 2, n - n / 2, val, val + n / 2);
    WSYNC();
    for (uint32_t i = lane; i < n; i += gw) out[c0 + i] = val[i];
}
void launch_diag_verify(const uint32_t *ref, uint32_t ref_len, uint32_t n_cases, const uint8_t *seqs, const uint32_t *offs, const uint32_t *cand,
                        const uint32_t *coffs, int mode, uint8_t *out, hipStream_t st)
{
    const uint32_t blocks = mode == 7 ? (n_cases + 3) / 4 : mode >= 5 ? (n_cases + 1) / 2 : n_cases;
    if (n_cases) hipLaunchKernelGGL(k_diag_verify, dim3(blocks), dim3(64), 0, st, ref, ref_len, n_cases, seqs, offs, cand, coffs, mode, out);
}

__global__ void __launch_bounds__(64)
k_polish(const uint8_t *__restrict__ pac, const uint8_t *__restrict__ codes, const uint32_t *__restrict__ offs, const salt_polish_item_t *__restrict__ items,
         uint32_t n_items, const uint8_t *__restrict__ pool, uint32_t pool_stride, int want_cigar, int32_t *__restrict__ dist,
         uint16_t *__restrict__ cigars, uint8_t *__restrict__ n_cigar, LvTables *__restrict__ tabs)
{
    __shared__ LvBytes s;
    __shared__ int s_n;
    const uint32_t lane = lane_id();
    for (uint32_t it = blockIdx.x; it < n_items; it += gridDim.x) {
        const salt_polish_item_t x = items[it];
        const uint32_t o = offs[x.read], L = offs[x.read + 1] - o, tl = x.tlen;
        WSYNC();
        for (uint32_t i = lane; i < L + 48; i += 64) {
            uint8_t pv = 1;
            if (i < L) { const uint8_t c = x.strand ? codes[o + L - 1 - i] : codes[o + i]; pv = c < 4 ? (uint8_t)(1u << (x.strand ? 3 - c : c)) : (uint8_t)(x.strand ? 0x20 : 0x10); }
            s.P[i] = pv;
        }
        for (uint32_t i = lane; i < L + 48; i += 64) {
            uint8_t tv = 1;
            if (x.pool != 0xFFFFFFFFu) { if (i < pool_stride) tv = (uint8_t)(1u << (pool[(uint64_t)x.pool * pool_stride + i] & 3u)); }
            else if (i < tl) { const uint64_t l = (uint64_t)x.offset + i; tv = (uint8_t)(1u << ((pac[l >> 2] >> ((~l & 3u) << 1)) & 3u)); }
            s.T[i] = tv;
        }
        WSYNC();
        int d_fin = 0;
        LvTables *tab = want_cigar ? tabs + blockIdx.x : nullptr;
        const int e = lv_wave(s.T, (int)tl, s.P, (int)L, (int)x.k, tab, d_fin);
        if (lane == 0) dist[it] = e;
        if (want_cigar) {
            __threadfence_block();
            WSYNC();
            const int end0 = (int)(L < tl ? L : tl);
            int straight = 0;
            for (int i = (int)lane; i < end0; i += 64) straight += s.P[i] != s.T[i];
            for (int w = 32; w > 0; w >>= 1) straight += __shfl_xor(straight, w);
            straight += (int)L - end0;
            if (lane == 0) {
                int n = 0;
                uint16_t *cg = cigars + (uint64_t)it * SALT_MAX_CIGAR_OPS;
                if (e == 0 || (e > 0 && straight == e)) cg[n++] = (uint16_t)((L << 4) | 0u);
                else if (e > 0) {
                    char act[LVK + 1]; int matched[LVK + 1];
                    int cd = d_fin;
                    for (int ce = e; ce >= 1; --ce) {
                        const char a = tab->A[ce][cd + 31];
                        act[ce] = a;
                        const int cur = tab->L[ce][cd + 31];
                        if (a == 'I') { matched[ce] = cur - tab->L[ce - 1][cd + 1 + 31] - 1; cd += 1; }
                        else if (a == 'D') { matched[ce] = cur - tab->L[ce - 1][cd - 1 + 31]; cd -= 1; }
                        else { matched[ce] = cur - tab->L[ce - 1][cd + 31] - 1; }
                    }
                    int acc = tab->L[0][31];
                    int ce = 1;
                    while (ce <= e) {
                        const char a = act[ce]; int cnt = 1;
                        while (ce + 1 <= e && matched[ce] == 0 && act[ce + 1] == a) { ++cnt; ++ce; }
                        if (a == 'X') acc += cnt;
                        else {
                            if (acc != 0 && n < SALT_MAX_CIGAR_OPS) cg[n++] = (uint16_t)((acc << 4) | 0);
                            acc = 0;
                            if (n < SALT_MAX_CIGAR_OPS) cg[n++] = (uint16_t)((cnt << 4) | (a == 'I' ? 1 : 2));
                        }
                        if (matched[ce] > 0) acc += matched[ce];
                        ++ce;
                    }
                    if (acc != 0 && n < SALT_MAX_CIGAR_OPS) cg[n++] = (uint16_t)((acc << 4) | 0);
                }
                n_cigar[it] = (uint8_t)n;
                s_n = n;
            }
            WSYNC();
        }
    }
}
void launch_polish(const uint8_t *pac, const uint8_t *codes, const uint32_t *offs, const salt_polish_item_t *items, uint32_t n_items, const uint8_t *pool,
                   uint32_t pool_stride, int want_cigar, int32_t *dist, uint16_t *cigars, uint8_t *n_cigar, void *tabs, uint32_t n_blocks, hipStream_t st)
{
    if (n_items) hipLaunchKernelGGL(k_polish, dim3(n_blocks), dim3(64), 0, st, pac, codes, offs, items, n_items, pool, pool_stride, want_cigar, dist, cigars, n_cigar,
                                    static_cast<LvTables *>(tabs));
}

__global__ void __launch_bounds__(256)
k_heads(const salt_result_t *__restrict__ res, uint32_t n, uint4 *__restrict__ heads)
{
    const uint64_t t = (uint64_t)blockIdx.x * blockDim.x + threadIdx.x;
    if (t >= (uint64_t)n * 8u) return;
    const uint32_t i = (uint32_t)(t >> 3), c = (uint32_t)t & 7u;
    heads[t] = reinterpret_cast<const uint4 *>(res + i)[c];
}
void launch_heads(const salt_result_t *res, uint32_t n, uint8_t *heads, hipStream_t st)
{
    if (n) hipLaunchKernelGGL(k_heads, dim3((uint32_t)(((uint64_t)n * 8u + 255) / 256)), dim3(256), 0, st, res, n, reinterpret_cast<uint4 *>(heads));
}

uint32_t heavy_blocks_per_cu()
{
    static int cached = 0;
    if (!cached) {
        int n = 0;
        if (hipOccupancyMaxActiveBlocksPerMultiprocessor(&n, k_heavy, 64, 0) != hipSuccess || n < 1) n = 8;
        cached = n;
    }
    return (uint32_t)cached;
}

void launch_heavy(const IndexView &ix, const AlignParams &ap, const uint32_t *pm, const uint4 *sai_c,
                  const uint4 *sai_r, salt_result_t *results, const uint32_t *queue, unsigned long long *ctr,
                  uint32_t n_blocks, uint32_t gap_blocks, void *lvtab, const GapBufs &g_in, uint32_t *ovq, QueueRange *ranges, uint8_t *pe_scr, hipEvent_t *ev3, hipStream_t st)
{
    if (!ap.n_reads) { if (ev3) for (int i = 0; i < 3; ++i) hipEventRecord(ev3[i], st); return; }
    uint32_t blocks = n_blocks < ap.n_reads ? n_blocks : ap.n_reads;
    LvTables *tab = static_cast<LvTables *>(lvtab);
    GapBufs g = g_in; g.ovq = ovq; g.ranges = ranges;
    static const bool force_big = getenv("SALT_GPU_HEAVY_BIG") && atoi(getenv("SALT_GPU_HEAVY_BIG"));
    const bool se_glob = !ap.pe && pe_scr != nullptr;
    if (se_glob) {
        hipLaunchKernelGGL(k_heavy_glob, dim3(blocks), dim3(64), 0, st, ix, ap, pm, sai_c, sai_r, results, queue, ctr, tab, g, pe_scr, 0);
    }
    const bool small = !se_glob && !force_big && g.cap > 0 && ovq != nullptr && ap.spr <= (uint32_t)WaveLdsSmall::N_SLOTS;
    if (small) {
        if (ap.pe) hipLaunchKernelGGL(k_heavy_pe, dim3(blocks), dim3(64), 0, st, ix, ap, pm, sai_c, sai_r, results, queue, ctr, tab, g, pe_scr, 0);
        else     hipLaunchKernelGGL(k_heavy, dim3(blocks), dim3(64), 0, st, ix, ap, pm, sai_c, sai_r, results, queue, ctr, tab, g, pe_scr, 0);
    }
    const uint32_t big_blocks = small && blocks > 256u ? 256u : blocks;
    if (se_glob) { }
    else if (ap.pe) hipLaunchKernelGGL(k_heavy_pe_big, dim3(big_blocks), dim3(64), 0, st, ix, ap, pm, sai_c, sai_r, results, queue, ctr, tab, g, pe_scr, small ? 1 : 0);
    else     hipLaunchKernelGGL(k_heavy_big, dim3(big_blocks), dim3(64), 0, st, ix, ap, pm, sai_c, sai_r, results, queue, ctr, tab, g, pe_scr, small ? 1 : 0);
    if (ev3) hipEventRecord(ev3[0], st);
    if (!g.cap) { if (ev3) { hipEventRecord(ev3[1], st); hipEventRecord(ev3[2], st); } return; }
    hipLaunchKernelGGL(k_gap, dim3(gap_blocks), dim3(64), 0, st, ix, ap, pm, g);
    if (ev3) hipEventRecord(ev3[1], st);
    hipLaunchKernelGGL(k_gapfin, dim3((n_blocks + 3) / 4), dim3(64), 0, st, ix, ap, pm, results, g, ctr);
    if (ev3) hipEventRecord(ev3[2], st);
    hipLaunchKernelGGL(k_cigar, dim3((n_blocks + 1) / 2), dim3(64), 0, st, ix, ap.pg, pm, results, g.cq, &g.gctl->cigar_items, &g.gctl->cigar_head, g.cap * (1u + SALT_MAX_HITS), tab);
}

GapBufs gap_bufs_layout(uint8_t *base, uint32_t cap, SeCtl *gctl, size_t *bytes)
{
    GapBufs g; size_t off = 0;
    auto take = [&](size_t n) { size_t o = off; off = (off + n + 255) & ~(size_t)255; return base ? base + o : nullptr; };
    { const uint64_t want = (uint64_t)cap * 2u * (uint64_t)MAXLOC; g.pool = (uint32_t)(want < (1ull << 26) ? want : (1ull << 26)); }
    g.items_cap = g.pool / LLV_N + 2u * cap;
    g.gq = reinterpret_cast<uint32_t *>(take((size_t)cap * 4));
    g.gn = reinterpret_cast<uint32_t *>(take((size_t)cap * 2 * 4));
    g.goff = reinterpret_cast<uint32_t *>(take((size_t)cap * 2 * 4));
    g.gloci = reinterpret_cast<uint32_t *>(take((size_t)g.pool * 4));
    g.ge = take((size_t)g.pool);
    g.gitems = reinterpret_cast<uint32_t *>(take((size_t)g.items_cap * 4));
    g.cq = reinterpret_cast<uint32_t *>(take((size_t)cap * (1 + SALT_MAX_HITS) * 4));
    g.gctl = gctl; g.cap = cap; g.ovq = nullptr;
    if (bytes) *bytes = off;
    return g;
}


}
```

salt_amd/csrc/salt_gpu.hip:

```cpp
#include <hip/hip_runtime.h>
#include <stdio.h>
#include <stdlib.h>
#include <string.h>
#include <time.h>
#include <cstddef>
#include <cctype>
#include <map>
#include <utility>
#include <string>
#include <thread>
#include <vector>
#include <algorithm>
#include "salt_kernels.h"
#include "salt_inflate_block.h"
#include <rccl/rccl.h>

using namespace salt;

static thread_local std::string g_err;
static int fail(int code, const std::string &msg) { g_err = msg; return code; }

#define HIPCHK(x) do { hipError_t e_ = (x); if (e_ != hipSuccess) \
    return fail(SALT_E_HIP, std::string(#x) + ": " + hipGetErrorString(e_)); } while (0)
#define DONECHK(x) do { hipError_t e_ = (x); if (e_ != hipSuccess) return done(fail(SALT_E_HIP, std::string(#x) + ": " + hipGetErrorString(e_))); } while (0)

template <class T> struct DevBuf {
    T *p = nullptr; uint64_t cap = 0;
    DevBuf() = default; DevBuf(const DevBuf &) = delete; DevBuf &operator=(const DevBuf &) = delete;
    ~DevBuf() { hipFree(p); }
    operator T *() const { return p; }
    T *operator->() const { return p; }
    void release() { hipFree(p); p = nullptr; cap = 0; }
    void take(DevBuf &o) { release(); p = o.p; cap = o.cap; o.p = nullptr; o.cap = 0; }
    hipError_t alloc(uint64_t n) { release(); const hipError_t e = hipMalloc((void **)&p, n * sizeof(T)); if (e == hipSuccess) cap = n; else p = nullptr; return e; }
    int reserve(uint64_t need, hipStream_t st)
    {
        if (need <= cap) return SALT_OK;
        HIPCHK(hipStreamSynchronize(st));
        HIPCHK(alloc(need + need / 4));
        return SALT_OK;
    }
};
template <class T> struct PinBuf {
    T *p = nullptr; uint64_t cap = 0; bool owned = true;
    PinBuf() = default; PinBuf(const PinBuf &) = delete; PinBuf &operator=(const PinBuf &) = delete;
    ~PinBuf() { release(); }
    operator T *() const { return p; }
    void release() { if (p && owned) hipHostFree(p); p = nullptr; cap = 0; owned = true; }
    void adopt(T *q, uint64_t n) { release(); p = q; cap = n; owned = false; }
    hipError_t alloc(uint64_t n) { release(); const hipError_t e = hipHostMalloc((void **)&p, n * sizeof(T), hipHostMallocDefault); if (e == hipSuccess) cap = n; else p = nullptr; return e; }
};

struct salt_gpu_index {
    int device = 0;
    uint8_t *image = nullptr;
    uint64_t bytes = 0;
    bool owns = true;
    ImageHeader hdr;
    IndexView view;
    uint8_t *d_pac = nullptr; uint64_t l_pac = 0;
    uint4 *d_rctx = nullptr;
    int64_t *d_c_off = nullptr; uint32_t *d_c_name_off = nullptr; char *d_c_names = nullptr; int32_t n_contigs = 0;
    struct Tally { uint32_t min_mapq = 0; bool on = false; } snp, depth, errprof;
    DevBuf<SnpWin> d_snp_tab; DevBuf<uint32_t> d_snp_counts; uint64_t snp_win = 0; uint32_t snp_sites = 0;
    DevBuf<uint32_t> d_depth; DepthText *depth_text = nullptr;
    std::vector<int64_t> h_c_off; uint32_t c_name_max = 0;
    DevBuf<unsigned long long> d_errprof;
};

struct salt_gpu_ws {
    salt_gpu_index *ix = nullptr;
    uint32_t max_reads = 0; uint64_t max_bases = 0;
    DevBuf<uint8_t> d_seqs; DevBuf<uint32_t> d_offs; DevBuf<salt_result_t> d_results;
    DevBuf<uint4> d_sai_c, d_sai_r;
    uint32_t epoch = 1;
    DevBuf<uint32_t> d_wq; uint32_t *d_wq_cnt = nullptr; uint32_t walk_blocks = 512; bool no_unique = false;
    DevBuf<uint32_t> d_pm, d_tb;
    DevBuf<uint8_t> d_heads; PinBuf<uint8_t> h_heads;
    DevBuf<unsigned long long> d_ctr;
    DevBuf<uint32_t> d_queue; SeCtl *d_qctl = nullptr;
    DevBuf<uint8_t> d_lvtab;
    DevBuf<uint8_t> d_gap; uint32_t gcap = 0; GapBufs gap{};
    DevBuf<uint8_t> d_pe_scr;
    DevBuf<PePair> d_pairs; DevBuf<PeSwReq> d_req; DevBuf<PeSwRes> d_swres; DevBuf<PeCtl> d_pctl;
    DevBuf<uint8_t> d_sw_scr; uint32_t sw_blocks = 0;
    DevBuf<uint32_t> d_pcq;
    DevBuf<uint8_t> d_raw; DevBuf<uint32_t> d_tile, d_lines;
    DevBuf<FqRec> d_rec; DevBuf<uint32_t> d_tctl, d_samoff; DevBuf<uint8_t> d_scan;
    DevBuf<char> d_sam; PinBuf<char> h_sam; DevBuf<char> d_rg; std::string rg;
    DevBuf<char> d_samslot; DevBuf<SamSeg> d_samseg;
    bool sam_bgzf = false;
    bool sam_bam = false;
    int polish = 0; PolishText *pl = nullptr; DevBuf<uint8_t> d_pl_tabs; uint32_t pl_blocks = 0;
    DevBuf<uint32_t> d_bz_slots, d_bz_sizes; DevBuf<unsigned long long> d_bz_offs; DevBuf<uint8_t> d_bz_out;
    PinBuf<char> h_bz;
    DevBuf<uint8_t> d_zin; DevBuf<unsigned long long> d_zoff; DevBuf<uint32_t> d_zstat;
    DevBuf<uint8_t> d_text; uint64_t text_bytes = 0;
    std::vector<unsigned long long> h_zoff; std::vector<uint32_t> h_zstat;
    uint32_t text_calls = 0;
    uint32_t heavy_blocks = 2048, gap_blocks = 2048;
    QueueRange *d_ranges = nullptr;
    DevBuf<uint8_t> d_zero;
    int all_heavy = 0;
    hipStream_t stream = nullptr;
    bool timing = false;
    std::vector<hipEvent_t> ev;
    std::vector<uint8_t> ev_pe;
    uint32_t n_timed = 0;
    template <class Job> struct LastJob { Job job{}; hipStream_t st = nullptr; };
    LastJob<SnpCount> snp_last; LastJob<DepthMark> depth_last; LastJob<ErrProf> ep_last;
    void forget_last() { snp_last.job.n_rec = 0; depth_last.job.n_rec = 0; ep_last.job.n_rec = 0; }
    const uint8_t *q_next = nullptr; bool q_next_dev = false;
    struct { const uint8_t *quals = nullptr; const FqRec *rec = nullptr; uint64_t bytes = 0; } q_cur;
    DevBuf<uint8_t> d_quals;
};
static const uint32_t MAX_TIMED = 256, EV_PER_CALL = 12;

static inline uint64_t align_up(uint64_t x, uint64_t a) { return (x + a - 1) / a * a; }

static void make_view(salt_gpu_index *ix)
{
    const ImageHeader &h = ix->hdr;
    IndexView &v = ix->view;
    uint8_t *b = ix->image;
    v.c_occ = reinterpret_cast<const COcc *>(b + h.off_c_occ);
    v.c_sa = reinterpret_cast<const uint32_t *>(b + h.off_c_sa);
    v.lkt = reinterpret_cast<const uint32_t *>(b + h.off_lkt);
    v.r_occ = reinterpret_cast<const ROcc *>(b + h.off_r_occ);
    v.r_pos = reinterpret_cast<const uint32_t *>(b + h.off_r_pos);
    v.wlkt = reinterpret_cast<const uint4 *>(b + h.off_wlkt);
    v.ref = reinterpret_cast<const uint32_t *>(b + h.off_ref);
    v.text = reinterpret_cast<const uint32_t *>(b + h.off_text);
    v.c_ctx = h.off_ctx ? reinterpret_cast<const uint4 *>(b + h.off_ctx) : nullptr; v.ctx_k = h.ctx_k;
    v.r_ctx = ix->d_rctx;
    v.c_primary = h.c_primary; memcpy(v.c_L2, h.c_L2, sizeof v.c_L2); v.c_seq_len = h.c_seq_len;
    v.r_text_len = h.r_text_len; v.r_inv_sa0 = h.r_inv_sa0; memcpy(v.r_cum, h.r_cum, sizeof v.r_cum);
    v.ref_len = h.ref_len; v.lkt_len = h.lkt_len; v.r_lkt_len = h.r_lkt_len;
}

extern "C" const char *salt_gpu_last_error(void) { return g_err.c_str(); }
extern "C" uint32_t salt_gpu_result_size(void) { return (uint32_t)sizeof(salt_result_t); }

static const uint64_t R_CTX_RESERVE_ATTACH = 40ull << 30;
static const uint64_t R_CTX_RESERVE_PAC = 32ull << 30;
static int attach_r_ctx(salt_gpu_index *ix, const uint64_t R_CTX_RESERVE)
{
    if (!ix->view.c_ctx || ix->d_rctx || (getenv("SALT_GPU_NO_RCTX") && atoi(getenv("SALT_GPU_NO_RCTX")))) return SALT_OK;
    const uint64_t rbytes = ((uint64_t)ix->hdr.r_text_len + 1) * 16;
    size_t free_b = 0, total_b = 0;
    if (hipMemGetInfo(&free_b, &total_b) == hipSuccess && (uint64_t)free_b >= rbytes + R_CTX_RESERVE && hipMalloc((void **)&ix->d_rctx, rbytes) == hipSuccess) {
        launch_build_r_ctx(ix->view, ix->hdr.ctx_k, ix->d_rctx, nullptr);
        if (hipGetLastError() != hipSuccess || hipDeviceSynchronize() != hipSuccess) { hipFree(ix->d_rctx); ix->d_rctx = nullptr; return fail(SALT_E_HIP, "building the R context records failed"); }
        ix->view.r_ctx = ix->d_rctx;
    } else { (void)hipGetLastError(); ix->d_rctx = nullptr; }
    return SALT_OK;
}

extern "C" int salt_gpu_index_attach(const salt_host_index_t *h, int device, salt_gpu_index_t **out)
{
    if (!h || !out) return fail(SALT_E_INVAL, "null argument");
    if (!h->c_bwt || !h->c_sa || !h->lkt || !h->r_bwt || !h->r_sa || !h->ref) return fail(SALT_E_INDEX, "missing index array");
    if (h->c_sa_intv == 0 || h->c_n_sa != (h->c_seq_len + h->c_sa_intv) / h->c_sa_intv) return fail(SALT_E_INDEX, "inconsistent C suffix-array sampling");
    if (h->lkt_len < 1 || h->lkt_len > 14 || h->lkt_n != (1u << (2 * h->lkt_len)) + 1) return fail(SALT_E_INDEX, "unsupported lookup-table length");
    if (h->r_n_sa != h->r_text_len - h->r_cum[4] + 1) return fail(SALT_E_INDEX, "R suffix array size does not match '#' count");
    if ((uint64_t)h->r_bwt_words * 8 < h->r_text_len) return fail(SALT_E_INDEX, "R BWT shorter than its text length");
    int n_dev = 0;
    HIPCHK(hipGetDeviceCount(&n_dev));
    if (n_dev <= 0) return fail(SALT_E_HIP, "no HIP device visible: the salt GPU path cannot run (there is no CPU fallback)");
    HIPCHK(hipSetDevice(device));

    salt_gpu_index *ix = new salt_gpu_index();
    ix->device = device;
    ImageHeader &hd = ix->hdr;
    memset(&hd, 0, sizeof hd);
    hd.magic = IMAGE_MAGIC;
    hd.c_primary = h->c_primary; memcpy(hd.c_L2, h->c_L2, sizeof hd.c_L2); hd.c_seq_len = h->c_seq_len; hd.c_sa_intv = h->c_sa_intv;
    hd.lkt_len = h->lkt_len; hd.lkt_n = h->lkt_n;
    hd.r_text_len = h->r_text_len; hd.r_inv_sa0 = h->r_inv_sa0; memcpy(hd.r_cum, h->r_cum, sizeof hd.r_cum);
    hd.ref_len = h->ref_len;
    const uint64_t ctx_bytes = (((uint64_t)h->c_seq_len + 1) * 16 + 255) / 256 * 256;
    bool want_ctx = h->l_seed > 0 && !(getenv("SALT_GPU_NO_CTX") && atoi(getenv("SALT_GPU_NO_CTX")));
    {
        uint32_t w = 14;
// ... 108 lines not shown
    ix->device = device; ix->image = static_cast<uint8_t *>(dev_ptr); ix->bytes = bytes; ix->owns = false;
    hipError_t e = hipMemcpy(&ix->hdr, dev_ptr, sizeof(ImageHeader), hipMemcpyDeviceToHost);
    if (e != hipSuccess) { delete ix; return fail(SALT_E_HIP, std::string("hipMemcpy(image header): ") + hipGetErrorString(e)); }
    if (ix->hdr.magic != IMAGE_MAGIC || ix->hdr.bytes != bytes) { delete ix; return fail(SALT_E_INDEX, "not a salt device-index image"); }
    make_view(ix);
    *out = ix;
    return SALT_OK;
}

extern "C" int salt_gpu_index_image_compact(const salt_gpu_index_t *ix, void **dev_ptr, uint64_t *bytes)
{
    if (!ix || !dev_ptr || !bytes) return fail(SALT_E_INVAL, "null argument");
    *dev_ptr = ix->image; *bytes = ix->hdr.off_wlkt;
    return SALT_OK;
}

static int rebuild_wlkt(salt_gpu_index *ix)
{
    launch_build_wlkt(ix->view, ix->hdr.r_lkt_len, reinterpret_cast<uint4 *>(ix->image + ix->hdr.off_wlkt), nullptr);
    if (ix->hdr.off_ctx) launch_build_c_ctx(ix->view, ix->hdr.ctx_k, reinterpret_cast<uint4 *>(ix->image + ix->hdr.off_ctx), nullptr);
    HIPCHK(hipGetLastError());
    HIPCHK(hipDeviceSynchronize());
    if (attach_r_ctx(ix, R_CTX_RESERVE_ATTACH)) g_err.clear();
    return SALT_OK;
}

extern "C" int salt_gpu_index_attach_compact(const void *dev_ptr, uint64_t bytes, int device, salt_gpu_index_t **out)
{
    if (!dev_ptr || !out || bytes < sizeof(ImageHeader)) return fail(SALT_E_INVAL, "bad image");
    HIPCHK(hipSetDevice(device));
    ImageHeader hd;
    HIPCHK(hipMemcpy(&hd, dev_ptr, sizeof hd, hipMemcpyDeviceToHost));
    if (hd.magic != IMAGE_MAGIC || hd.off_wlkt != bytes || hd.bytes < bytes) return fail(SALT_E_INDEX, "not a compact salt device-index image");
    salt_gpu_index *ix = new salt_gpu_index();
    ix->device = device; ix->bytes = hd.bytes; ix->owns = true; ix->hdr = hd;
    hipError_t e = hipMalloc((void **)&ix->image, hd.bytes);
    if (e != hipSuccess) { delete ix; return fail(SALT_E_NOMEM, std::string("hipMalloc(index image): ") + hipGetErrorString(e)); }
    e = hipMemcpy(ix->image, dev_ptr, bytes, hipMemcpyDeviceToDevice);
    if (e != hipSuccess) { hipFree(ix->image); delete ix; return fail(SALT_E_HIP, std::string("hipMemcpy(compact image): ") + hipGetErrorString(e)); }
    make_view(ix);
    int rc = rebuild_wlkt(ix);
    if (rc) { hipFree(ix->image); delete ix; return rc; }
    *out = ix;
    return SALT_OK;
}

extern "C" int salt_gpu_ws_create(salt_gpu_index_t *ix, uint32_t max_reads, uint64_t max_bases, salt_gpu_ws_t **out)
{
    if (!ix || !out || max_reads == 0) return fail(SALT_E_INVAL, "bad workspace size");
    HIPCHK(hipSetDevice(ix->device));
    salt_gpu_ws *ws = new salt_gpu_ws();
    ws->ix = ix; ws->max_reads = max_reads; ws->max_bases = max_bases;
#define CHKW(x) do { hipError_t e2 = (x); if (e2 != hipSuccess) { salt_gpu_ws_destroy(ws); \
    return fail(SALT_E_NOMEM, std::string(#x) + ": " + hipGetErrorString(e2)); } } while (0)
    CHKW(ws->d_seqs.alloc(max_bases + 64));
    CHKW(ws->d_offs.alloc((uint64_t)max_reads + 1));
    CHKW(ws->d_results.alloc(max_reads));
    CHKW(hipMemset(ws->d_results, 0, (uint64_t)max_reads * sizeof(salt_result_t)));
    CHKW(ws->d_queue.alloc(queue_words(max_reads)));
    {
        const size_t a = 256, n_ranges = (QUEUE_RANGES * sizeof(QueueRange) + a - 1) / a * a, n_ctl = (sizeof(SeCtl) + a - 1) / a * a;
        const size_t n_cnt = ((size_t)seed_wq_cnt_words() * 4 + a - 1) / a * a;
        CHKW(ws->d_zero.alloc(n_ranges + n_ctl + n_cnt));
        ws->d_ranges = reinterpret_cast<QueueRange *>(ws->d_zero.p); ws->d_qctl = reinterpret_cast<SeCtl *>(ws->d_zero + n_ranges);
        ws->d_wq_cnt = reinterpret_cast<uint32_t *>(ws->d_zero + n_ranges + n_ctl);
    }
    ws->gcap = max_reads < (1u << 20) ? max_reads : (1u << 20);
    if (const char *e3 = getenv("SALT_GPU_NO_GAP_DEFER")) if (atoi(e3)) ws->gcap = 0;
    if (const char *e3 = getenv("SALT_GPU_GAP_SLOTS")) { const int v = atoi(e3); if (v > 0 && (uint32_t)v < ws->gcap) ws->gcap = (uint32_t)v; }
    if (ws->gcap) {
        size_t gbytes = 0;
        gap_bufs_layout(nullptr, ws->gcap, nullptr, &gbytes);
        CHKW(ws->d_gap.alloc(gbytes));
    }
    {
        hipDeviceProp_t prop;
        CHKW(hipGetDeviceProperties(&prop, ix->device));
        uint32_t per_cu = heavy_blocks_per_cu();
        if (const char *e2 = getenv("SALT_GPU_HEAVY_PER_CU")) { int v = atoi(e2); if (v > 0 && (uint32_t)v <= heavy_blocks_per_cu()) per_cu = (uint32_t)v; }
        ws->heavy_blocks = (uint32_t)prop.multiProcessorCount * per_cu;
        uint32_t gap_per_cu = 16;
        if (const char *e2 = getenv("SALT_GPU_GAP_PER_CU")) { int v = atoi(e2); if (v > 0 && v <= 16) gap_per_cu = (uint32_t)v; }
        ws->gap_blocks = (uint32_t)prop.multiProcessorCount * gap_per_cu;
        ws->walk_blocks = (uint32_t)prop.multiProcessorCount * 2u;
        if (const char *e2 = getenv("SALT_GPU_WALK_PER_CU")) { int v = atoi(e2); if (v > 0 && v <= 16) ws->walk_blocks = (uint32_t)prop.multiProcessorCount * (uint32_t)v; }
        if (const char *e2 = getenv("SALT_GPU_SAI_EPOCH")) { const long long v = atoll(e2); if (v >= 1 && v <= (long long)SAI_EPOCH_MAX) ws->epoch = (uint32_t)v; }
        if (const char *e2 = getenv("SALT_GPU_NO_UNIQUE")) ws->no_unique = atoi(e2) != 0;
        if (const char *e2 = getenv("SALT_GPU_WALK_BLOCKS")) { int v = atoi(e2); if (v > 0 && v <= 65536) ws->walk_blocks = (uint32_t)v; }
        CHKW(ws->d_lvtab.alloc((uint64_t)ws->heavy_blocks * lv_table_bytes()));
        const char *e = getenv("SALT_GPU_ALL_HEAVY");
        ws->all_heavy = e && atoi(e) != 0;
    }
    CHKW(ws->d_ctr.alloc(SALT_CTR_N));
    CHKW(hipMemset(ws->d_ctr, 0, SALT_CTR_N * sizeof(unsigned long long)));
    CHKW(hipStreamCreate(&ws->stream));
#undef CHKW
    *out = ws;
    return SALT_OK;
}

extern "C" void salt_gpu_ws_destroy(salt_gpu_ws_t *ws)
{
    if (!ws) return;
    hipSetDevice(ws->ix->device);
    if (ws->stream) hipStreamDestroy(ws->stream);
    for (auto &e : ws->ev) if (e) hipEventDestroy(e);
    polish_text_free(ws->pl);
    delete ws;
}

static int check_opt(const salt_gpu_index *ix, const salt_aln_opt_t *o, uint32_t max_len, uint32_t *spr_out)
{
    if (o->l_seed < (int32_t)ix->hdr.r_lkt_len) return fail(SALT_E_INVAL, "l_seed shorter than the device k-mer table (set SALT_GPU_LKT_LEN or pass l_seed at attach)");
    if (o->l_overlap <= 0) return fail(SALT_E_INVAL, "l_overlap must be positive (aln.c:223 sets it to l_seed when -r is absent)");
    if (o->max_locate == 0 || o->max_locate > PE_LOCI_CAP) return fail(SALT_E_INVAL, "max_locate (-m) must be in 1..262144");
    if (o->max_hits != SALT_MAX_HITS) return fail(SALT_E_INVAL, "max_hits is fixed at 5 (aln.h:133)");
    if (max_len > SALT_MAX_READ_LEN) return fail(SALT_E_INVAL, "read longer than SALT_MAX_READ_LEN (512)");
    uint32_t spr = 1;
    if (max_len >= (uint32_t)o->l_seed) spr = (max_len - (uint32_t)o->l_seed) / (uint32_t)o->l_overlap + 1;
    if (spr > SALT_MAX_SEED_SLOTS) return fail(SALT_E_INVAL, "more seeds per strand than SALT_MAX_SEED_SLOTS (512): raise -r or shorten the reads");
    *spr_out = spr;
    return SALT_OK;
}

static int align_resident_impl(salt_gpu_ws_t *ws, const salt_aln_opt_t *o, uint32_t n_reads, uint32_t max_read_len,
                               const void *d_seqs, const void *d_offs, void *d_results, void *hip_stream, int pe);

template <class Job> static int tally_launch(salt_gpu_ws::LastJob<Job> &last, hipError_t (*launch)(const Job &, hipStream_t), const Job &c, hipStream_t st)
{
    HIPCHK(launch(c, st));
    last.job = c; last.st = st;
    return SALT_OK;
}
static int rows_hooks(salt_gpu_ws_t *ws, uint32_t n_rec, const void *d_seqs, const void *d_offs, const void *d_results, int pe, hipStream_t st)
{
    const salt_gpu_index *ix = ws->ix;
    const salt_result_t *res = static_cast<const salt_result_t *>(d_results);
    const uint8_t *seqs = static_cast<const uint8_t *>(d_seqs); const uint32_t *offs = static_cast<const uint32_t *>(d_offs);
    if (ix->snp.on) {
        SnpCount c{};
        c.res = res; c.seqs = seqs; c.offs = offs; c.n_rec = n_rec;
        c.tab = ix->d_snp_tab; c.n_win = ix->snp_win; c.counts = ix->d_snp_counts; c.min_mapq = ix->snp.min_mapq; c.pe = pe; c.delta = 1u;
        if (const int rc = tally_launch(ws->snp_last, launch_snp_count, c, st)) return rc;
    }
    if (ix->depth.on) {
        DepthMark c{};
        c.res = res; c.n_rec = n_rec; c.diff = ix->d_depth; c.ref_len = ix->view.ref_len; c.min_mapq = ix->depth.min_mapq; c.delta = 1u;
        if (const int rc = tally_launch(ws->depth_last, launch_depth_mark, c, st)) return rc;
    }
    if (ix->errprof.on) {
        ErrProf c{};
        c.res = res; c.seqs = seqs; c.offs = offs; c.n_rec = n_rec;
        c.quals = ws->q_cur.quals; c.rec = ws->q_cur.rec; c.q_bytes = ws->q_cur.bytes;
        c.ref = ix->view.ref; c.ref_len = ix->view.ref_len; c.cells = ix->d_errprof; c.min_mapq = ix->errprof.min_mapq; c.pe = pe; c.delta = 1ull;
        if (const int rc = tally_launch(ws->ep_last, launch_errprof, c, st)) return rc;
    }
    return SALT_OK;
}
static int quals_upload(salt_gpu_ws_t *ws, uint64_t bases, hipStream_t st)
{
    if (!ws->q_next || ws->q_next_dev) return SALT_OK;
    if (!ws->ix->errprof.on) { ws->q_next = nullptr; return SALT_OK; }
    if (int rc = ws->d_quals.reserve(bases + 64, st)) { ws->q_next = nullptr; return rc; }
    const hipError_t e = hipMemcpyAsync(ws->d_quals, ws->q_next, bases, hipMemcpyHostToDevice, st);
    ws->q_next = ws->d_quals; ws->q_next_dev = true;
    if (e != hipSuccess) { ws->q_next = nullptr; return fail(SALT_E_HIP, std::string("hipMemcpyAsync(quality bytes): ") + hipGetErrorString(e)); }
// ... 2 lines not shown
static int quals_take(salt_gpu_ws_t *ws)
{
    ws->q_cur = {};
    const uint8_t *q = ws->q_next; ws->q_next = nullptr;
    if (!q) return SALT_OK;
    if (!ws->q_next_dev) return fail(SALT_E_INVAL, "salt_gpu_ws_set_quals: host quality bytes cannot serve a resident call (pass a device pointer, on_device = 1)");
    ws->q_cur.quals = q; ws->q_cur.bytes = ~0ull;
    return SALT_OK;
}

static int reserve_seed(salt_gpu_ws_t *ws, uint64_t items, hipStream_t st, bool settle)
{
    if (items <= ws->d_sai_c.cap) return SALT_OK;
    HIPCHK(hipStreamSynchronize(st));
    ws->d_sai_c.release(); ws->d_sai_r.release(); ws->d_wq.release();
    HIPCHK(ws->d_sai_r.alloc(items));
    HIPCHK(hipMemsetAsync(ws->d_sai_r, 0, items * sizeof(uint4), st));
    if (settle) HIPCHK(hipStreamSynchronize(st));
    HIPCHK(ws->d_wq.alloc(seed_wq_words(items)));
    HIPCHK(ws->d_sai_c.alloc(items));
    return SALT_OK;
}

static int reserve_pack(salt_gpu_ws_t *ws, uint32_t n_reads, const PackGeom &pg, hipStream_t st)
{
    if ((uint64_t)n_reads * pg.pm_stride <= ws->d_pm.cap && (uint64_t)n_reads * pg.tb_stride <= ws->d_tb.cap) return SALT_OK;
    HIPCHK(hipStreamSynchronize(st));
    const uint64_t nr = n_reads > ws->max_reads ? n_reads : ws->max_reads;
    ws->d_tb.release();
    HIPCHK(ws->d_pm.alloc(nr * pg.pm_stride));
    HIPCHK(ws->d_tb.alloc(nr * pg.tb_stride));
    return SALT_OK;
}

extern "C" int salt_gpu_align_se_resident(salt_gpu_ws_t *ws, const salt_aln_opt_t *o, uint32_t n_reads, uint32_t max_read_len,
                                          const void *d_seqs, const void *d_offs, void *d_results, void *hip_stream)
{
    if (!ws) return fail(SALT_E_INVAL, "null argument");
    if (int rc = quals_take(ws)) return rc;
    return align_resident_impl(ws, o, n_reads, max_read_len, d_seqs, d_offs, d_results, hip_stream, 0);
}

static int align_resident_impl(salt_gpu_ws_t *ws, const salt_aln_opt_t *o, uint32_t n_reads, uint32_t max_read_len,
                               const void *d_seqs, const void *d_offs, void *d_results, void *hip_stream, int pe)
{
    if (!ws || !o || !d_seqs || !d_offs || !d_results) return fail(SALT_E_INVAL, "null argument");
    ws->forget_last();
    if (n_reads == 0) return SALT_OK;
    uint32_t spr = 0;
    int rc = check_opt(ws->ix, o, max_read_len, &spr);
    if (rc) return rc;
    HIPCHK(hipSetDevice(ws->ix->device));
    hipStream_t st = static_cast<hipStream_t>(hip_stream);
    if (int rc2 = reserve_seed(ws, (uint64_t)n_reads * 2u * spr, st, false)) return rc2;
    const PackGeom pg = PackGeom::make(max_read_len);
    if (int rc2 = reserve_pack(ws, n_reads, pg, st)) return rc2;
    SeedParams sp; sp.pg = pg; sp.n_reads = n_reads; sp.spr = spr; sp.l_seed = o->l_seed; sp.l_overlap = o->l_overlap;
    sp.max_seed = o->max_seed; sp.seed_only_ref = o->seed_only_ref;
    sp.resolve_unique = !ws->no_unique;
    if (n_reads > ws->max_reads) return fail(SALT_E_CAPACITY, "more reads than the workspace holds");
    if (ws->epoch > SAI_EPOCH_MAX) { HIPCHK(hipMemsetAsync(ws->d_sai_r, 0, ws->d_sai_r.cap * sizeof(uint4), st)); ws->epoch = 1; }
    sp.epoch = ws->epoch++;
    AlignParams ap; ap.pg = pg; ap.n_reads = n_reads; ap.spr = spr; ap.l_seed = o->l_seed; ap.max_locate = o->max_locate; ap.max_hits = o->max_hits;
    ap.all_heavy = ws->all_heavy; ap.pe = pe; ap.dbg_stop = 0; ap.heavy_stop = 0; ap.max_amb = pe ? 5u : 200u; ap.epoch = sp.epoch;
#ifdef SALT_DIAG
    { const char *e = getenv("SALT_GPU_LIGHT_STOP"); ap.dbg_stop = e ? atoi(e) : 0; } { static const int hs = getenv("SALT_GPU_HEAVY_STOP") ? atoi(getenv("SALT_GPU_HEAVY_STOP")) : 0; ap.heavy_stop = hs; }
#endif
    const bool glob_loci = pe || o->max_locate > SALT_MAX_LOCATE;
    if (glob_loci && !ws->d_pe_scr) HIPCHK(ws->d_pe_scr.alloc((uint64_t)ws->heavy_blocks * PE_LOCI_CAP * 5));
    unsigned long long *ctr = o->collect_counters ? ws->d_ctr.p : nullptr;
    const bool timed = ws->timing && ws->n_timed < MAX_TIMED;
    hipEvent_t *ev = timed ? &ws->ev[(size_t)ws->n_timed * EV_PER_CALL] : nullptr;
    HIPCHK(hipMemsetAsync(ws->d_zero, 0, ws->d_zero.cap, st));
    if (timed) HIPCHK(hipEventRecord(ev[0], st));
    launch_pack(pg, n_reads, static_cast<const uint8_t *>(d_seqs), static_cast<const uint32_t *>(d_offs), ws->d_pm, ws->d_tb, st);
    if (timed) HIPCHK(hipEventRecord(ev[1], st));
    launch_seed(ws->ix->view, sp, ws->d_tb, ws->d_sai_c, ws->d_sai_r, reinterpret_cast<uint4 *>(ws->d_wq.p), ws->d_wq_cnt, ws->walk_blocks, ctr, st);
    if (timed) HIPCHK(hipEventRecord(ev[2], st));
    if (!ap.all_heavy)
        launch_light(ws->ix->view, ap, ws->d_pm, static_cast<const uint8_t *>(d_seqs), static_cast<const uint32_t *>(d_offs), ws->d_sai_c, ws->d_sai_r,
                     static_cast<salt_result_t *>(d_results), ws->d_queue, ws->d_qctl, ws->d_queue + 2 * (size_t)ws->max_reads, ws->d_ranges, ctr, st);
    if (timed) HIPCHK(hipEventRecord(ev[3], st));
    launch_heavy(ws->ix->view, ap, ws->d_pm, ws->d_sai_c, ws->d_sai_r,
                 static_cast<salt_result_t *>(d_results), ws->d_queue, ctr, ws->heavy_blocks, ws->gap_blocks, ws->d_lvtab,
                 gap_bufs_layout(ws->d_gap, ws->gcap, ws->d_qctl, nullptr), ws->d_queue + ws->max_reads, ws->d_ranges, glob_loci ? ws->d_pe_scr.p : nullptr, timed ? ev + 4 : nullptr, st);
    if (timed) { HIPCHK(hipEventRecord(ev[7], st)); ws->ev_pe[ws->n_timed] = 0; ++ws->n_timed; }
    HIPCHK(hipGetLastError());
    if (!pe) return rows_hooks(ws, n_reads, d_seqs, d_offs, d_results, 0, st);
    return SALT_OK;
}

static const uint32_t HEAD_BYTES = 128;
static_assert(offsetof(salt_result_t, cigar) + 8 * sizeof(uint16_t) == HEAD_BYTES, "result head");
static int fetch_results(salt_gpu_ws_t *ws, uint32_t n_reads, salt_result_t *results, hipStream_t st)
{
    if (!ws->d_heads) {
        HIPCHK(ws->h_heads.alloc((uint64_t)ws->max_reads * HEAD_BYTES));
        HIPCHK(ws->d_heads.alloc((uint64_t)ws->max_reads * HEAD_BYTES));
    }
    launch_heads(ws->d_results, n_reads, ws->d_heads, st);
    HIPCHK(hipMemcpyAsync(ws->h_heads, ws->d_heads, (uint64_t)n_reads * HEAD_BYTES, hipMemcpyDeviceToHost, st));
    HIPCHK(hipStreamSynchronize(st));
    std::vector<uint32_t> full;
    const uint32_t n_thr = n_reads >= 262144 ? 4u : 1u;
    std::vector<std::vector<uint32_t>> full_t(n_thr);
    auto scatter = [&](uint32_t t) {
        const uint32_t lo = (uint32_t)((uint64_t)n_reads * t / n_thr), hi = (uint32_t)((uint64_t)n_reads * (t + 1) / n_thr);
        for (uint32_t i = lo; i < hi; ++i) {
            memcpy(&results[i], ws->h_heads + (uint64_t)i * HEAD_BYTES, HEAD_BYTES);
            const salt_result_t &r = results[i];
            bool more = r.n_cigar > 8;
            for (int h = 0; h < SALT_MAX_HITS; ++h) more |= r.hit_n_cigar[h] != 0;
            if (more) full_t[t].push_back(i);
        }
    };
    {
        std::vector<std::thread> th;
        for (uint32_t t = 1; t < n_thr; ++t) th.emplace_back(scatter, t);
        scatter(0);
        for (auto &x : th) x.join();
    }
    for (auto &v : full_t) full.insert(full.end(), v.begin(), v.end());
    if (full.size() > 4096) {
        HIPCHK(hipMemcpyAsync(results, ws->d_results, (uint64_t)n_reads * sizeof(salt_result_t), hipMemcpyDeviceToHost, st));
    } else {
        for (uint32_t i : full) HIPCHK(hipMemcpyAsync(&results[i], ws->d_results + i, sizeof(salt_result_t), hipMemcpyDeviceToHost, st));
    }
    HIPCHK(hipStreamSynchronize(st));
    return SALT_OK;
}

extern "C" int salt_gpu_align_se(salt_gpu_ws_t *ws, const salt_aln_opt_t *o, uint32_t n_reads, const uint8_t *seqs,
                                 const uint32_t *offs, salt_result_t *results)
{
    if (!ws || !o || !seqs || !offs || !results) return fail(SALT_E_INVAL, "null argument");
    if (n_reads == 0) return SALT_OK;
    if (n_reads > ws->max_reads) return fail(SALT_E_CAPACITY, "more reads than the workspace holds");
    if (offs[0] != 0) return fail(SALT_E_INVAL, "offs[0] must be 0");
    uint64_t bases = offs[n_reads];
    if (bases > ws->max_bases) return fail(SALT_E_CAPACITY, "more bases than the workspace holds");
    uint32_t max_len = 0;
    for (uint32_t i = 0; i < n_reads; ++i) {
        if (offs[i + 1] < offs[i]) return fail(SALT_E_INVAL, "offs must be non-decreasing");
        uint32_t l = offs[i + 1] - offs[i];
        if (l == 0) return fail(SALT_E_INVAL, "empty read");
        max_len = l > max_len ? l : max_len;
    }
    HIPCHK(hipSetDevice(ws->ix->device));
    HIPCHK(hipMemcpyAsync(ws->d_seqs, seqs, bases, hipMemcpyHostToDevice, ws->stream));
    HIPCHK(hipMemcpyAsync(ws->d_offs, offs, ((uint64_t)n_reads + 1) * 4, hipMemcpyHostToDevice, ws->stream));
    if (int rc2 = quals_upload(ws, bases, ws->stream)) return rc2;
    int rc = salt_gpu_align_se_resident(ws, o, n_reads, max_len, ws->d_seqs, ws->d_offs, ws->d_results, ws->stream);
    if (rc) return rc;
    return fetch_results(ws, n_reads, results, ws->stream);
}

extern "C" int salt_gpu_index_set_contigs(salt_gpu_index_t *ix, int32_t n, const int64_t *offsets, const char *const *names)
{
    if (!ix || n <= 0 || !offsets || !names) return fail(SALT_E_INVAL, "bad contig table");
    HIPCHK(hipSetDevice(ix->device));
    std::vector<uint32_t> noff((size_t)n + 1, 0); std::string blob;
    for (int i = 0; i < n; ++i) { if (!names[i]) return fail(SALT_E_INVAL, "contig without a name"); blob += names[i]; noff[(size_t)i + 1] = (uint32_t)blob.size(); }
    if (ix->d_c_off) { hipFree(ix->d_c_off); hipFree(ix->d_c_name_off); hipFree(ix->d_c_names); ix->d_c_off = nullptr; ix->d_c_name_off = nullptr; ix->d_c_names = nullptr; ix->n_contigs = 0; }
    HIPCHK(hipMalloc((void **)&ix->d_c_off, (size_t)n * 8));
    HIPCHK(hipMalloc((void **)&ix->d_c_name_off, ((size_t)n + 1) * 4));
    HIPCHK(hipMalloc((void **)&ix->d_c_names, blob.size() + 1));
    HIPCHK(hipMemcpy(ix->d_c_off, offsets, (size_t)n * 8, hipMemcpyHostToDevice));
// ... 688 lines not shown
            if (failed && i > 0) {
                if (out[i]) { salt_gpu_index_detach(out[i]); out[i] = nullptr; }
                else if (buf[i]) hipFree(buf[i]);
            }
        }
        hipSetDevice(devices[0]);
    };
#define REPCHK(x) do { hipError_t e_ = (x); if (e_ != hipSuccess) { cleanup(true); \
    return fail(SALT_E_HIP, std::string(#x) + ": " + hipGetErrorString(e_)); } } while (0)
    buf[0] = src->image;
    for (int i = 1; i < n; ++i) { REPCHK(hipSetDevice(devices[i])); REPCHK(hipMalloc(&buf[i], src->bytes)); }
    ncclResult_t rc = ncclCommInitAll(comm.data(), n, devices);
    if (rc != ncclSuccess) { cleanup(true); return fail(SALT_E_HIP, std::string("ncclCommInitAll: ") + ncclGetErrorString(rc)); }
    comm_ok = true;
    for (int i = 0; i < n; ++i) { REPCHK(hipSetDevice(devices[i])); REPCHK(hipStreamCreate(&st[i])); }
    ncclGroupStart();
    for (int i = 0; i < n; ++i) {
        rc = ncclBroadcast(buf[i], buf[i], src->hdr.off_wlkt, ncclUint8, 0, comm[i], st[i]);
        if (rc != ncclSuccess) { ncclGroupEnd(); cleanup(true); return fail(SALT_E_HIP, std::string("ncclBroadcast: ") + ncclGetErrorString(rc)); }
    }
    rc = ncclGroupEnd();
    if (rc != ncclSuccess) { cleanup(true); return fail(SALT_E_HIP, std::string("ncclGroupEnd: ") + ncclGetErrorString(rc)); }
    for (int i = 0; i < n; ++i) { REPCHK(hipSetDevice(devices[i])); REPCHK(hipStreamSynchronize(st[i])); }
    for (int i = 1; i < n; ++i) {
        int r2 = salt_gpu_index_attach_image(buf[i], src->bytes, devices[i], &out[i]);
        if (r2) { out[i] = nullptr; const std::string m = g_err; cleanup(true); return fail(r2, m); }
        out[i]->owns = true;
        REPCHK(hipSetDevice(devices[i]));
        r2 = rebuild_wlkt(out[i]);
        if (r2) { const std::string m = g_err; cleanup(true); return fail(r2, m); }
    }
#undef REPCHK
    cleanup(false);
    return SALT_OK;
}

extern "C" int salt_gpu_index_image_copy(const salt_gpu_index_t *ix, void *dst, uint64_t dst_bytes)
{
    if (!ix || !dst) return fail(SALT_E_INVAL, "null argument");
    const uint64_t n = dst_bytes >= ix->bytes ? ix->bytes : ix->hdr.off_wlkt;
    if (dst_bytes < n) return fail(SALT_E_INVAL, "destination too small for the (compact) index image");
    HIPCHK(hipSetDevice(ix->device));
    HIPCHK(hipMemcpy(dst, ix->image, n, hipMemcpyDeviceToDevice));
    return SALT_OK;
}

extern "C" int salt_gpu_ws_timing(salt_gpu_ws_t *ws, int enable)
{
    if (!ws) return fail(SALT_E_INVAL, "null argument");
    HIPCHK(hipSetDevice(ws->ix->device));
    if (enable && ws->ev.empty()) {
        ws->ev.resize((size_t)MAX_TIMED * EV_PER_CALL);
        ws->ev_pe.assign(MAX_TIMED, 0);
        for (auto &e : ws->ev) HIPCHK(hipEventCreate(&e));
    }
    ws->timing = enable != 0; ws->n_timed = 0;
    return SALT_OK;
}

extern "C" int salt_gpu_ws_kernel_ms(salt_gpu_ws_t *ws, double ms[SALT_N_KERNELS], uint32_t *n_calls)
{
    if (!ws || !ms || !n_calls) return fail(SALT_E_INVAL, "null argument");
    HIPCHK(hipSetDevice(ws->ix->device));
    for (int k = 0; k < SALT_N_KERNELS; ++k) ms[k] = 0;
    *n_calls = ws->n_timed;
    for (uint32_t i = 0; i < ws->n_timed; ++i) {
        hipEvent_t *ev = &ws->ev[(size_t)i * EV_PER_CALL];
        const int n_k = ws->ev_pe[i] ? SALT_N_KERNELS : 7;
        HIPCHK(hipEventSynchronize(ev[n_k]));
        for (int k = 0; k < n_k; ++k) {
            float a = 0;
            HIPCHK(hipEventElapsedTime(&a, ev[k], ev[k + 1]));
            ms[k] += a;
        }
    }
    ws->n_timed = 0;
    return SALT_OK;
}

extern "C" int salt_gpu_diag_lv(const uint32_t *ref_words, uint32_t ref_len, uint32_t n_cases, const uint32_t *pos,
                                const uint32_t *kdiff, const uint8_t *seqs, const uint32_t *offs, int32_t *out4,
                                uint16_t *cigars)
{
    if (!ref_words || !pos || !kdiff || !seqs || !offs || !out4 || !cigars) return fail(SALT_E_INVAL, "null argument");
    int n_dev = 0;
    HIPCHK(hipGetDeviceCount(&n_dev));
    if (n_dev <= 0) return fail(SALT_E_HIP, "no HIP device visible");
    const uint64_t nw = ((uint64_t)ref_len + 7) / 8 + 4;
    uint32_t *d_ref = nullptr, *d_pos = nullptr, *d_k = nullptr, *d_offs = nullptr; uint8_t *d_seqs = nullptr;
    int32_t *d_out = nullptr; uint16_t *d_cig = nullptr;
    const uint64_t bases = offs[n_cases];
    HIPCHK(hipMalloc((void **)&d_ref, nw * 4)); HIPCHK(hipMemset(d_ref, 0, nw * 4));
    HIPCHK(hipMemcpy(d_ref, ref_words, (nw - 4) * 4, hipMemcpyHostToDevice));
    HIPCHK(hipMalloc((void **)&d_pos, (uint64_t)n_cases * 4)); HIPCHK(hipMemcpy(d_pos, pos, (uint64_t)n_cases * 4, hipMemcpyHostToDevice));
    HIPCHK(hipMalloc((void **)&d_k, (uint64_t)n_cases * 4)); HIPCHK(hipMemcpy(d_k, kdiff, (uint64_t)n_cases * 4, hipMemcpyHostToDevice));
    HIPCHK(hipMalloc((void **)&d_offs, ((uint64_t)n_cases + 1) * 4)); HIPCHK(hipMemcpy(d_offs, offs, ((uint64_t)n_cases + 1) * 4, hipMemcpyHostToDevice));
    HIPCHK(hipMalloc((void **)&d_seqs, bases + 64)); HIPCHK(hipMemcpy(d_seqs, seqs, bases, hipMemcpyHostToDevice));
    HIPCHK(hipMalloc((void **)&d_out, (uint64_t)n_cases * 16)); HIPCHK(hipMemset(d_out, 0xFD, (uint64_t)n_cases * 16));
    HIPCHK(hipMalloc((void **)&d_cig, (uint64_t)n_cases * SALT_MAX_CIGAR_OPS * 2)); HIPCHK(hipMemset(d_cig, 0, (uint64_t)n_cases * SALT_MAX_CIGAR_OPS * 2));
    IndexView v; memset(&v, 0, sizeof v);
    v.ref = d_ref; v.ref_len = ref_len;
    void *d_tab = nullptr;
    HIPCHK(hipMalloc(&d_tab, (uint64_t)n_cases * lv_table_bytes()));
    std::vector<uint32_t> lane_first(n_cases + 1, 0u), lane_n(n_cases + 1, 0u), lane_case;
    {
        std::map<std::pair<uint32_t, uint32_t>, std::vector<uint32_t>> by_shape;
        for (uint32_t c = 0; c < n_cases; ++c) {
            if (offs[c + 1] < offs[c]) return fail(SALT_E_INVAL, "offsets must not decrease");
            if (lv_lanes_fit(offs[c + 1] - offs[c], kdiff[c])) by_shape[std::make_pair(offs[c + 1] - offs[c], kdiff[c])].push_back(c);
        }
        for (const auto &kv : by_shape) {
            const std::vector<uint32_t> &cs = kv.second;
            for (size_t i = 0; i < cs.size();) {
                const uint32_t take = cs.size() - i >= 64 ? 64u : 1u;
                lane_first[cs[i]] = (uint32_t)lane_case.size(); lane_n[cs[i]] = take;
                lane_case.insert(lane_case.end(), cs.begin() + i, cs.begin() + i + take);
                i += take;
            }
        }
        lane_case.push_back(0u);
    }
    uint32_t *d_lf = nullptr, *d_ln = nullptr, *d_lc = nullptr;
    HIPCHK(hipMalloc((void **)&d_lf, lane_first.size() * 4)); HIPCHK(hipMemcpy(d_lf, lane_first.data(), lane_first.size() * 4, hipMemcpyHostToDevice));
    HIPCHK(hipMalloc((void **)&d_ln, lane_n.size() * 4)); HIPCHK(hipMemcpy(d_ln, lane_n.data(), lane_n.size() * 4, hipMemcpyHostToDevice));
    HIPCHK(hipMalloc((void **)&d_lc, lane_case.size() * 4)); HIPCHK(hipMemcpy(d_lc, lane_case.data(), lane_case.size() * 4, hipMemcpyHostToDevice));
    launch_diag_lv(v, n_cases, d_pos, d_k, d_seqs, d_offs, d_lf, d_ln, d_lc, d_out, d_cig, d_tab, nullptr);
    HIPCHK(hipGetLastError());
    HIPCHK(hipDeviceSynchronize());
    HIPCHK(hipMemcpy(out4, d_out, (uint64_t)n_cases * 16, hipMemcpyDeviceToHost));
    HIPCHK(hipMemcpy(cigars, d_cig, (uint64_t)n_cases * SALT_MAX_CIGAR_OPS * 2, hipMemcpyDeviceToHost));
    hipFree(d_ref); hipFree(d_pos); hipFree(d_k); hipFree(d_offs); hipFree(d_seqs); hipFree(d_out); hipFree(d_cig); hipFree(d_tab);
    hipFree(d_lf); hipFree(d_ln); hipFree(d_lc);
    return SALT_OK;
}

extern "C" int salt_gpu_diag_ssw(uint32_t n_cases, const uint8_t *aware, const uint8_t *ref_syms, const uint32_t *ref_offs,
                                 const uint8_t *codes, const uint32_t *read_offs, int32_t *out6, uint16_t *cigars, uint16_t *n_cigar)
{
    if (!aware || !ref_syms || !ref_offs || !codes || !read_offs || !out6 || !cigars || !n_cigar) return fail(SALT_E_INVAL, "null argument");
    if (n_cases == 0) return SALT_OK;
    const uint64_t n_sym = ref_offs[n_cases], n_base = read_offs[n_cases];
    std::vector<uint32_t> h_ref(n_sym / 8 + 8, 0u);
    std::vector<uint8_t> h_pac(n_sym / 4 + 8, 0);
    std::vector<PeSwReq> h_req(n_cases);
    uint32_t diag_max_len = 1;
    for (uint32_t i = 0; i < n_cases; ++i) {
        if (ref_offs[i + 1] <= ref_offs[i] || read_offs[i + 1] <= read_offs[i]) return fail(SALT_E_INVAL, "empty case");
        for (uint64_t p = ref_offs[i]; p < ref_offs[i + 1]; ++p) {
            h_ref[p >> 3] |= (uint32_t)(ref_syms[p] & 15u) << (4 * (p & 7u));
            h_pac[p >> 2] |= (uint8_t)((ref_syms[p] & 3u) << ((~p & 3u) << 1));
        }
        h_req[i] = PeSwReq{ ref_offs[i], ref_offs[i + 1] - 1, i, 0, (uint8_t)(aware[i] ? 1 : 0), 0 };
        if (read_offs[i + 1] - read_offs[i] > diag_max_len) diag_max_len = read_offs[i + 1] - read_offs[i];
    }
    if (diag_max_len > SALT_MAX_READ_LEN) return fail(SALT_E_INVAL, "read longer than SALT_MAX_READ_LEN");
    uint64_t diag_max_win = 1;
    for (uint32_t i = 0; i < n_cases; ++i) if (ref_offs[i + 1] - ref_offs[i] > diag_max_win) diag_max_win = ref_offs[i + 1] - ref_offs[i];
    uint32_t *d_ref = nullptr, *d_offs = nullptr; uint8_t *d_pac = nullptr, *d_codes = nullptr;
    auto done = [&](int rc) { hipFree(d_ref); hipFree(d_pac); hipFree(d_codes); hipFree(d_offs); return rc; };
    DONECHK(hipMalloc((void **)&d_ref, h_ref.size() * 4)); DONECHK(hipMemcpy(d_ref, h_ref.data(), h_ref.size() * 4, hipMemcpyHostToDevice));
    DONECHK(hipMalloc((void **)&d_pac, h_pac.size())); DONECHK(hipMemcpy(d_pac, h_pac.data(), h_pac.size(), hipMemcpyHostToDevice));
    DONECHK(hipMalloc((void **)&d_codes, n_base + 16)); DONECHK(hipMemcpy(d_codes, codes, n_base, hipMemcpyHostToDevice));
    DONECHK(hipMalloc((void **)&d_offs, ((uint64_t)n_cases + 1) * 4)); DONECHK(hipMemcpy(d_offs, read_offs, ((uint64_t)n_cases + 1) * 4, hipMemcpyHostToDevice));
    const uint32_t blocks = n_cases / 8 + 1 < 256 ? n_cases / 8 + 1 : 256;
    SwGeom geom = sw_geom(diag_max_len, diag_max_win, 1);
    geom.n_blocks = blocks; geom.tb_blocks = blocks;
    IndexView v; memset(&v, 0, sizeof v);
    v.ref = d_ref; v.ref_len = (uint32_t)n_sym;
    std::vector<PeSwRes> h_res; uint32_t n_over = 0;
    if (int rc = sw_run(v, d_pac, d_codes, d_offs, h_req, geom, diag_max_len, h_res, &n_over)) return done(rc);
    for (uint32_t i = 0; i < n_cases; ++i) {
        const PeSwRes &r = h_res[i];
        int32_t *o = out6 + 6 * (uint64_t)i;
        o[0] = r.score1; o[1] = r.score2; o[2] = r.ref_begin; o[3] = r.ref_end; o[4] = r.read_begin; o[5] = r.read_end;
        n_cigar[i] = r.n_cigar;
        memcpy(cigars + (uint64_t)i * SALT_MAX_CIGAR_OPS, r.cigar, sizeof r.cigar);
    }
    if (n_over) return done(fail(SALT_E_CAPACITY, std::to_string(n_over) + " case(s) need a band wider than SW_BAND_W or a CIGAR of more than "
                                 "SALT_MAX_CIGAR_OPS operations: their rows hold the scores and end points, and no CIGAR"));
    return done(SALT_OK);
}

extern "C" int salt_gpu_buffer_alloc(int device, uint64_t bytes, void **dev_ptr)
{
    if (!dev_ptr || !bytes) return fail(SALT_E_INVAL, "null argument");
    HIPCHK(hipSetDevice(device));
    HIPCHK(hipMalloc(dev_ptr, bytes));
    return SALT_OK;
}

extern "C" int salt_gpu_buffer_free(int device, void *dev_ptr)
{
    if (!dev_ptr) return SALT_OK;
    HIPCHK(hipSetDevice(device));
    HIPCHK(hipFree(dev_ptr));
    return SALT_OK;
}

__global__ void k_buffer_diff(const uint32_t *a, const uint32_t *b, uint64_t n_words, unsigned long long *n_diff)
{
    unsigned long long d = 0;
    for (uint64_t i = (uint64_t)blockIdx.x * blockDim.x + threadIdx.x; i < n_words; i += (uint64_t)gridDim.x * blockDim.x) d += a[i] != b[i];
    if (d) atomicAdd(n_diff, d);
}

extern "C" int salt_gpu_buffer_equal(int device, const void *a, const void *b, uint64_t bytes, int *equal)
{
    if (!a || !b || !equal || (bytes & 3u)) return fail(SALT_E_INVAL, "bad buffer compare arguments (bytes must be a multiple of 4)");
    HIPCHK(hipSetDevice(device));
// ... 503 lines not shown
```

salt_amd/csrc/salt_kernels.h:

```cpp
#pragma once
#include <hip/hip_runtime.h>
#include <cstddef>
#include <string>
#include <vector>
#include "../../include/salt_gpu.h"
#include "salt_device.h"

#ifdef SALT_DIAG
#define SALT_DIAG_VAL(x) (x)
#else
#define SALT_DIAG_VAL(x) 0
#endif

namespace salt {

struct PackGeom {
    uint32_t nw8, nw16, nw32, pm_stride, tb_stride;
    __host__ __device__ static PackGeom make(uint32_t max_len)
    {
        if (max_len < 1) max_len = 1;
        PackGeom g; g.nw8 = (max_len + 7) / 8; g.nw16 = (max_len + 15) / 16; g.nw32 = (max_len + 31) / 32;
        g.pm_stride = (2 * g.nw8 + 1 + 3) & ~3u; g.tb_stride = (2 * g.nw16 + 2 * g.nw32 + 1 + 3) & ~3u;
        return g;
    }
};

struct SeedParams {
    uint32_t n_reads, spr;
    int32_t  l_seed, l_overlap;
    uint32_t max_seed;
    int32_t  seed_only_ref;
    int32_t  resolve_unique;
    uint32_t epoch;
    PackGeom pg;
};

struct AlignParams {
    uint32_t n_reads, spr;
    int32_t  l_seed;
    uint32_t max_locate;
    int32_t  max_hits;
    PackGeom pg;
    int32_t  dbg_stop;
    int32_t  heavy_stop;
    int32_t  all_heavy;
    int32_t  pe;
    uint32_t max_amb;
    uint32_t epoch;
};
static const uint32_t PE_LOCI_CAP = 0x40000;

void launch_pack(const PackGeom &pg, uint32_t n_reads, const uint8_t *seqs, const uint32_t *offs, uint32_t *pm, uint32_t *tb, hipStream_t st);
void launch_seed(const IndexView &ix, const SeedParams &sp, const uint32_t *tb, uint4 *sai_c, uint4 *sai_r, uint4 *wq, uint32_t *wq_cnt,
                 uint32_t walk_blocks, unsigned long long *ctr, hipStream_t st);
size_t seed_wq_words(uint64_t items);
uint32_t seed_wq_cnt_words();
__device__ __forceinline__ uint32_t sw_pull(uint32_t *head, const uint32_t step, const uint32_t n_first, const uint32_t n_items)
{
    if (n_first >= n_items || n_first + __hip_atomic_load(head, __ATOMIC_RELAXED, __HIP_MEMORY_SCOPE_AGENT) >= n_items) return 0xFFFFFFFFu;
    return n_first + atomicAdd(head, step);
}
struct SeCtl {
    alignas(128) uint32_t light_queued;
    alignas(128) uint32_t gap_slots;
    alignas(128) uint32_t gap_items;
    alignas(128) uint32_t cigar_items;
    alignas(128) uint32_t cigar_head;
    alignas(128) uint32_t pool_used;
    alignas(128) uint32_t ovq_count;
    alignas(128) uint32_t ovq_head;
};
static_assert(sizeof(SeCtl) == 8 * 128 && alignof(SeCtl) == 128, "one control word per 128-byte line");
static const uint32_t QUEUE_RANGES = 64;
struct QueueRange {
    enum { HEAVY, GAP, GAPFIN };
    uint32_t push, pad0[31], heads[3], retry, pad1[28];
};
static_assert(sizeof(QueueRange) == 256 && offsetof(QueueRange, push) == 0 && offsetof(QueueRange, heads) == 128, "k_light's counter, then the heads");
void launch_light(const IndexView &ix, const AlignParams &ap, const uint32_t *pm, const uint8_t *seqs, const uint32_t *offs, const uint4 *sai_c,
                  const uint4 *sai_r, salt_result_t *results, uint32_t *queue, SeCtl *ctl, uint32_t *qseg, QueueRange *ranges, unsigned long long *ctr, hipStream_t st);
size_t queue_words(uint32_t max_reads);
struct GapBufs {
    uint32_t *gq;
    uint32_t *gn;
    uint32_t *goff;
    uint32_t *gloci;
    uint8_t  *ge;
    uint32_t *gitems;
    uint32_t *cq;
    SeCtl *gctl;
    uint32_t cap, pool, items_cap;
    uint32_t *ovq;
    QueueRange *ranges;
};
GapBufs gap_bufs_layout(uint8_t *base, uint32_t cap, SeCtl *gctl, size_t *bytes);
void launch_heavy(const IndexView &ix, const AlignParams &ap, const uint32_t *pm, const uint4 *sai_c,
                  const uint4 *sai_r, salt_result_t *results, const uint32_t *queue, unsigned long long *ctr,
                  uint32_t n_blocks, uint32_t gap_blocks, void *lvtab, const GapBufs &g, uint32_t *ovq, QueueRange *ranges, uint8_t *pe_scr, hipEvent_t *ev3, hipStream_t st);
size_t lv_table_bytes();

static const uint32_t SW_MAX_SEG = 64;
static const uint32_t SW_BAND_W = 1100;
struct SwGeom {
    uint32_t maxcol_bytes, n_blocks;
    uint32_t tb_group_bytes, tb_blocks;
};
SwGeom sw_geom(uint32_t max_len, uint64_t max_window, uint32_t cus);
void sw_geom_limit(SwGeom &g, uint32_t blocks);
uint64_t sw_scratch_bytes(const SwGeom &g);
struct PeSwReq { uint32_t start, end, mate; uint8_t strand, aware; uint16_t pad; };
struct PeSwRes { int32_t score1, score2, ref_begin, ref_end, read_begin, read_end; uint32_t start, strand; uint16_t n_cigar, ok; uint16_t cigar[SALT_MAX_CIGAR_OPS]; };
struct PePair { uint32_t req0; uint8_t n_req; uint8_t rescued[2]; uint8_t pad; };
struct PeCtl {
    uint32_t n_req, unused1;
    uint32_t n_cigar, cigar_head;
    uint32_t overflow;
    uint32_t diag_cols, diag_clk, unused7;
    uint32_t tb_clk[4];
    uint32_t sw_heads[4];
    uint32_t swf1_pending;
};
static_assert(offsetof(PeCtl, n_cigar) == 8 && offsetof(PeCtl, overflow) == 16 && offsetof(PeCtl, diag_cols) == 20 && offsetof(PeCtl, tb_clk) == 32 &&
              offsetof(PeCtl, sw_heads) == 48 && offsetof(PeCtl, swf1_pending) == 64 && sizeof(PeCtl) == 68, "paired-end control words");
void launch_pair(uint32_t n_pairs, uint32_t min_tlen, uint32_t max_tlen, uint32_t l_pac, const uint32_t *offs, salt_result_t *res,
                 PePair *pairs, PeSwReq *req, PeCtl *ctl, hipStream_t st);
void launch_sw(const IndexView &ix, const uint8_t *pac, const uint8_t *seqs, const uint32_t *offs, const PeSwReq *req, PeCtl *ctl,
               PeSwRes *res, uint8_t *scratch, SwGeom g, uint32_t max_len, hipStream_t st);
static const uint32_t SW_MAX_BLOCKS_PER_CU = 16;
static const uint64_t SW_SCRATCH_TOTAL = 2ull << 30;
uint32_t sw_blocks_per_cu(uint32_t max_len);
void launch_pe_final(const IndexView &ix, const PackGeom &pg, uint32_t n_pairs, const uint32_t *pm, salt_result_t *res, const PePair *pairs,
                     const PeSwRes *sw, void *lvtab, uint32_t *citems, PeCtl *ctl, uint32_t n_blocks, hipStream_t st);

uint32_t heavy_blocks_per_cu();
void launch_polish(const uint8_t *pac, const uint8_t *codes, const uint32_t *offs, const salt_polish_item_t *items, uint32_t n_items, const uint8_t *pool,
                   uint32_t pool_stride, int want_cigar, int32_t *dist, uint16_t *cigars, uint8_t *n_cigar, void *tabs, uint32_t n_blocks, hipStream_t st);
void launch_heads(const salt_result_t *res, uint32_t n, uint8_t *heads, hipStream_t st);
void launch_diag_rule(uint32_t n_cases, const uint32_t *pos, const uint8_t *val, const uint32_t *offs, const uint32_t *bound_in,
                      uint32_t L, uint32_t ref_len, int mode, uint32_t *out, hipStream_t st);
uint32_t diag_rule_words();
void launch_diag_verify(const uint32_t *ref, uint32_t ref_len, uint32_t n_cases, const uint8_t *seqs, const uint32_t *offs, const uint32_t *cand,
                        const uint32_t *coffs, int mode, uint8_t *out, hipStream_t st);
void launch_diag_lv(const IndexView &ix, uint32_t n, const uint32_t *pos, const uint32_t *kdiff, const uint8_t *seqs,
                    const uint32_t *offs, const uint32_t *lane_first, const uint32_t *lane_n, const uint32_t *lane_case,
                    int32_t *out, uint16_t *cig, void *lvtab, hipStream_t st);
bool lv_lanes_fit(uint32_t L, uint32_t k);

struct FqRec { uint32_t name_off, name_len, seq_off, len, qual_off; };
static const uint32_t SAM_HEAD_CAP = 96, SAM_TAIL_CAP = 224, SAM_SLOT = SAM_HEAD_CAP + SAM_TAIL_CAP;
struct SamSeg { uint16_t head_len, tail_len; uint8_t what, strand, over, pad; };
struct SamDev {
    const uint8_t *raw; const FqRec *rec; const uint8_t *seqs; const uint32_t *offs; const salt_result_t *res;
    const int64_t *c_off; const uint32_t *c_name_off; const char *c_names; int32_t n_contigs;
    const uint32_t *text, *ref;
    int32_t xa_cigar, nm_md; const char *rg; int32_t rg_len;
    int32_t pe; uint32_t min_tlen, max_tlen;
    char *slot; SamSeg *seg;
    const uint32_t *tb; PackGeom pg;
};
hipError_t text_warm();
size_t text_scan_bytes(uint64_t max_items);
hipError_t launch_fq_count(const uint8_t *raw, uint64_t n, uint32_t *tile_cnt, void *tmp, size_t tmp_bytes, hipStream_t st);
hipError_t launch_fq_lines(const uint8_t *raw, uint64_t n, const uint32_t *tile_off, uint32_t *line_start, hipStream_t st);
hipError_t launch_fq_ctl_init(uint32_t *ctl, hipStream_t st);
hipError_t launch_fq_parse(const uint8_t *raw, const uint32_t *line_start, uint32_t n_rec, FqRec *rec, uint32_t *offs, uint32_t *ctl,
                           void *tmp, size_t tmp_bytes, hipStream_t st);
hipError_t launch_fq_parse_mate(const uint8_t *raw, uint32_t base, const uint32_t *line_start, uint32_t n_rec, uint32_t which, FqRec *rec, uint32_t *len,
                                uint32_t *ctl, hipStream_t st);
hipError_t launch_text_scan(uint32_t *v, uint32_t n_plus_1, void *tmp, size_t tmp_bytes, hipStream_t st);
hipError_t launch_fq_codes(const uint8_t *raw, const FqRec *rec, const uint32_t *offs, uint32_t n_rec, uint8_t *seqs, hipStream_t st);
hipError_t launch_sam_len(const SamDev &d, uint32_t n, uint32_t *off, unsigned long long *total64, void *tmp, size_t tmp_bytes, hipStream_t st);
hipError_t launch_sam_write(const SamDev &d, uint32_t n, const uint32_t *off, char *out, hipStream_t st);
hipError_t launch_bam_len(const SamDev &d, uint32_t n, uint32_t *off, unsigned long long *total64, uint32_t *err, void *tmp, size_t tmp_bytes, hipStream_t st);
hipError_t launch_bam_write(const SamDev &d, uint32_t n, const uint32_t *off, char *out, hipStream_t st);
static const uint32_t FQ_TILE = 1024;

struct PolishText;
PolishText *polish_text_new();
void polish_text_free(PolishText *t);
const uint64_t *polish_text_stats(const PolishText *t);
int polish_text_set_contigs(PolishText *t, int32_t n, const int64_t *offsets, const char *const *names, std::string &err);
int polish_text_run(PolishText *t, const uint8_t *d_pac, uint64_t l_pac, void *d_tabs, uint32_t n_blocks, int paired, int use_sw, const char *sam, uint64_t n_bytes,
                    const char **out, uint64_t *out_bytes, uint32_t *n_records, int *stopped, std::string &err);
struct PolishRows {
    const uint8_t *raw; const FqRec *fq; const uint8_t *codes; const uint32_t *offs; const salt_result_t *res; uint32_t n_rec, max_len;
    const int64_t *c_off; const uint32_t *c_name_off; const char *c_names; int32_t n_contigs;
    const uint8_t *pac; uint64_t l_pac; void *tabs; uint32_t n_blocks; int paired, use_sw; hipStream_t st;
};
int polish_rows_len(PolishText *t, const PolishRows &in, uint64_t *total, std::string &err);
int polish_rows_write(PolishText *t, char *d_out, hipStream_t st, std::string &err);

static const uint32_t BGZF_CUT_BYTES = 32640, BGZF_SLOT_BYTES = 32768;
inline uint64_t bgzf_blocks(uint64_t n) { return (n + BGZF_CUT_BYTES - 1) / BGZF_CUT_BYTES; }
inline uint64_t bgzf_bound(uint64_t n) { return n + 31 * bgzf_blocks(n); }
hipError_t launch_bgzf_deflate(const uint8_t *text, uint64_t n, uint32_t *slots, uint32_t *sizes, unsigned long long *offs, uint8_t *out, hipStream_t st);

hipError_t launch_bgzf_inflate(const uint8_t *members, const unsigned long long *c_off, const unsigned long long *u_off, uint32_t n_blocks,
                               uint8_t *text, uint32_t *status, hipStream_t st);

struct SnpWin { unsigned long long bits; uint32_t rank, pad; };
static_assert(sizeof(SnpWin) == 16, "one request per window");
struct SnpCount {
    const salt_result_t *res; const uint8_t *seqs; const uint32_t *offs; uint32_t n_rec;
    const SnpWin *tab; uint64_t n_win; uint32_t *counts;
    uint32_t min_mapq; int32_t pe;
    uint32_t delta;
};
size_t snp_scan_bytes(uint64_t n_win);
hipError_t launch_snp_table(const uint32_t *ref, uint32_t ref_len, uint64_t n_win, SnpWin *tab, uint32_t *cnt, void *tmp, size_t tmp_bytes, hipStream_t st);
hipError_t launch_snp_pos(const SnpWin *tab, uint64_t n_win, uint32_t *pos, hipStream_t st);
hipError_t launch_snp_count(const SnpCount &c, hipStream_t st);

struct DepthMark {
    const salt_result_t *res; uint32_t n_rec;
    uint32_t *diff; uint32_t ref_len;
    uint32_t min_mapq;
    uint32_t delta;
};
hipError_t launch_depth_mark(const DepthMark &c, hipStream_t st);
hipError_t launch_depth_add(uint32_t *diff, const uint32_t *in, uint64_t n, hipStream_t st);
struct DepthText;
DepthText *depth_text_new();
void depth_text_free(DepthText *t);
int depth_text_begin(DepthText *t, const uint32_t *d_diff, uint32_t ref_len, const int64_t *d_c_off, const uint32_t *d_c_name_off, const char *d_c_names,
                     const std::vector<int64_t> &h_c_off, uint32_t max_name, uint32_t window, uint32_t tile_positions, int bgzf, std::string &err);
int depth_text_next(DepthText *t, const char **data, uint64_t *n_bytes, std::string &err);

static constexpr uint32_t SALT_EP_CHUNK = 1024;
// ... 23 lines not shown
```

Baseline: 558.9 Mreads/s.

## Batch and prefetch gap-finalize rows, wave-wide queue pops, LDS LV tables for cigars

k_gapfin now pops work with a wave-wide ballot over 64 queue ranges rather than lane-0 popping and broadcasting through LDS. It also prefetches loci rows in batches of 8 per lane, double-buffered, and makes per-item scalars uniform with readfirstlane. The LV traceback tables can now sit in LDS through a pointer-pair abstraction, and the traceback scratch moves from stack arrays into shared text bytes. It also adds a separate cigar-kernel block count and a waves_per_eu hint on k_gapfin, which trade register budget and occupancy for better latency hiding.

```diff
diff --git a/include/salt_gpu.h b/include/salt_gpu.h
--- a/include/salt_gpu.h
+++ b/include/salt_gpu.h
@@ -186,6 +186,8 @@
 
 int  salt_gpu_diag_lv(const uint32_t *ref_words, uint32_t ref_len, uint32_t n_cases, const uint32_t *pos,
                       const uint32_t *kdiff, const uint8_t *seqs, const uint32_t *offs, int32_t *out4, uint16_t *cigars);
+int  salt_gpu_diag_lv_tab(const uint32_t *ref_words, uint32_t ref_len, uint32_t n_cases, const uint32_t *pos,
+                          const uint32_t *kdiff, const uint8_t *seqs, const uint32_t *offs, int32_t *out4, uint16_t *cigars, int lds_tab);
 
 int  salt_gpu_diag_ssw(uint32_t n_cases, const uint8_t *aware, const uint8_t *ref_syms, const uint32_t *ref_offs,
                        const uint8_t *codes, const uint32_t *read_offs, int32_t *out6, uint16_t *cigars, uint16_t *n_cigar);
diff --git a/salt_amd/csrc/salt_align.hip b/salt_amd/csrc/salt_align.hip
--- a/salt_amd/csrc/salt_align.hip
+++ b/salt_amd/csrc/salt_align.hip
@@ -542,6 +542,7 @@
 struct SaiLists { uint32_t *sp[2], *ep[2], *off[2]; };
 template <int NS> __device__ __forceinline__ SaiLists sai_ref(SaiListsT<NS> &a) { return SaiLists{ { a.sp[0], a.sp[1] }, { a.ep[0], a.ep[1] }, { a.off[0], a.off[1] } }; }
 struct LvTables { short L[LVK][64]; char A[LVK][64]; };
+struct LvTabRef { short *L; char *A; };
 static constexpr int LLV_K = 12;
 static constexpr int LLV_TW = 22;
 static constexpr int LLV_N = 64;
@@ -552,6 +553,11 @@
 static_assert(((8 * (LLV_TW - 1) - LLV_WIN) >> 3) + 2 <= LLV_PW, "pattern words of the longest read");
 struct LaneLv { uint32_t T[LLV_TS * LLV_N]; uint32_t P[LLV_PW]; };
 struct LvBytes { uint8_t T[MAXL + 4 + 64]; uint8_t P[MAXL + 64]; };
+struct LvTablesLds { short L[LLV_K + 1][64]; char A[LLV_K + 1][64]; };
+__device__ __forceinline__ LvTabRef lv_tab(LvTables *t) { return t ? LvTabRef{ &t->L[0][0], &t->A[0][0] } : LvTabRef{ nullptr, nullptr }; }
+__device__ __forceinline__ LvTabRef lv_tab(LvTablesLds &t) { return LvTabRef{ &t.L[0][0], &t.A[0][0] }; }
+struct LvTrace { int matched[LVK + 1]; char act[LVK + 1]; };
+static_assert(sizeof(LvTrace) <= sizeof(LvBytes::T), "the traceback's levels fit the text bytes");
 template <int NS, bool LLV>
 struct WaveLdsT {
     static constexpr bool HAS_LLV = LLV;
@@ -1031,8 +1037,10 @@
     }
 }
 
-__device__ __attribute__((noinline)) int lv_wave(const uint8_t *T, int tlen, const uint8_t *P, int plen, int k, LvTables *tab, int &d_fin)
-{
+struct LvEnd { int e, d_fin; };
+__device__ __attribute__((noinline)) LvEnd lv_wave(const uint8_t *T, int tlen, const uint8_t *P, int plen, int k, const LvTabRef tab)
+{
+    int d_fin = 0;
     const int lane = (int)lane_id();
     const int d = lane - 31;
     const int ad = d < 0 ? -d : d;
@@ -1040,9 +1048,8 @@
     const int end0 = plen < tlen ? plen : tlen;
     if (d == 0) { int i = 0; while (i < end0 && (P[i] & T[i]) != 0) ++i; Lprev = i; }
     const int r0 = __shfl(Lprev, 31);
-    if (tab) tab->L[0][lane] = (short)Lprev;
-    d_fin = 0;
-    if (r0 == end0) return plen > end0 ? plen - end0 : 0;
+    if (tab.L) tab.L[lane] = (short)Lprev;
+    if (r0 == end0) return LvEnd{ plen > end0 ? plen - end0 : 0, 0 };
     if (k > LVK - 1) k = LVK - 1;
     for (int e = 1; e <= k; ++e) {
         int left = __shfl_up(Lprev, 1), right = __shfl_down(Lprev, 1);
@@ -1061,20 +1068,20 @@
             }
             cur = best;
         }
-        if (tab) { tab->L[e][lane] = (short)cur; tab->A[e][lane] = act; }
+        if (tab.L) { tab.L[e * 64 + lane] = (short)cur; tab.A[e * 64 + lane] = act; }
         uint64_t reach = __ballot(active && cur == plen);
         if (reach) {
-            if (tab) {
+            if (tab.L) {
                 int rank = d == 0 ? 0 : (d < 0 ? 2 * ad - 1 : 2 * ad);
                 int my = (active && cur == plen) ? rank : 1000;
                 for (int o = 32; o > 0; o >>= 1) { int t = __shfl_xor(my, o); my = t < my ? t : my; }
                 d_fin = my == 0 ? 0 : ((my & 1) ? -((my + 1) >> 1) : (my >> 1));
             }
-            return e;
+            return LvEnd{ e, d_fin };
         }
         Lprev = cur;
     }
-    return -1;
+    return LvEnd{ -1, 0 };
 }
 
 __device__ __attribute__((noinline)) uint32_t lv_lanes(LaneLv &s, const uint32_t *pm, int plen, int tlen, int k, bool active)
@@ -1135,10 +1142,49 @@
     return result;
 }
 
-template <int VMAX, bool GAPF>
+template <int B> struct RowBatch { uint32_t p[B], v[B]; };
+static constexpr int GAPFIN_B = 8;
+template <int B>
+__device__ __forceinline__ void rows_fetch(RowBatch<B> &r, const uint32_t *pos, const uint8_t *val, const uint32_t n, const uint32_t b)
+{
+    const uint32_t lane = lane_id();
+#pragma unroll
+    for (int j = 0; j < B; ++j) {
+        const uint32_t i = b + 64u * (uint32_t)j + lane;
+        r.p[j] = 0; r.v[j] = 0xFFFFFFFFu;
+        if (i < n) { r.p[j] = pos[i]; r.v[j] = val[i]; }
+    }
+}
+template <int B, bool TWO, class F>
+__device__ __forceinline__ void list_trips(const uint32_t *pos, const uint8_t *val, const uint32_t n, const RowBatch<B> *first, F trip)
+{
+    const uint32_t lane = lane_id();
+    if constexpr (B == 1) {
+        for (uint32_t b = 0; b < n; b += 64) {
+            const uint32_t i = b + lane;
+            uint32_t p = 0, v = 0xFFFFFFFFu;
+            if (i < n) { p = pos[i]; v = val[i]; }
+            trip(i, p, v);
+        }
+    } else {
+        if (n == 0) return;
+        RowBatch<B> cur;
+        if (first) cur = *first; else rows_fetch<B>(cur, pos, val, n, 0u);
+        for (uint32_t b = 0; b < n; b += 64u * B) {
+            RowBatch<B> nxt;
+            const bool more = b + 64u * B < n;
+            if (TWO && more) rows_fetch<B>(nxt, pos, val, n, b + 64u * B);
+#pragma unroll
+            for (int j = 0; j < B; ++j) if (b + 64u * (uint32_t)j < n) trip(b + 64u * (uint32_t)j + lane, cur.p[j], cur.v[j]);
+            if (more) { if (TWO) cur = nxt; else rows_fetch<B>(cur, pos, val, n, b + 64u * B); }
+        }
+    }
+}
+template <int VMAX, bool GAPF, int B = 1>
 __device__ __forceinline__ void rule_unsorted(const uint32_t *pos, const uint8_t *val, const uint32_t n, const uint32_t L, const uint32_t ref_len,
                                               uint32_t &bound, bool &any, uint32_t &best_pos, uint32_t &best_v,
-                                              uint32_t &n_hits, uint32_t &a0, uint32_t *hit_pos, uint8_t *hit_nd)
+                                              uint32_t &n_hits, uint32_t &a0, uint32_t *hit_pos, uint8_t *hit_nd,
+                                              const RowBatch<B> *first = nullptr)
 {
     const uint32_t lane = lane_id();
     const uint32_t NONE = 0xFFFFFFFFu;
@@ -1147,10 +1193,7 @@
 #pragma unroll
     for (int t = 0; t <= VMAX; ++t) mp[t] = NONE;
     uint32_t my_p = 0, my_v = NONE, n_p = 0;
-    for (uint32_t b = 0; b < n; b += 64) {
-        const uint32_t i = b + lane;
-        uint32_t p = 0, v = NONE;
-        if (i < n) { p = pos[i]; v = val[i]; }
+    list_trips<B, true>(pos, val, n, first, [&](const uint32_t i, const uint32_t p, const uint32_t v) {
         const bool in = i < n && v <= bound && in_range(p);
         if (in) {
 #pragma unroll
@@ -1167,7 +1210,7 @@
                     ++n_p; m &= m - 1;
                 }
         }
-    }
+    });
 #pragma unroll
     for (int t = 0; t <= VMAX; ++t)
         for (int o = 32; o > 0; o >>= 1) { const uint32_t x = (uint32_t)__shfl_xor((int)mp[t], o); mp[t] = x < mp[t] ? x : mp[t]; }
@@ -1192,19 +1235,15 @@
         unsigned long long cur = ~0ull;
         if (in_lanes) { if (h == 0 || my_key > last) cur = my_key; }
         else
-        for (uint32_t b = 0; b < n; b += 64) {
-            const uint32_t i = b + lane;
-            if (i < n) {
-                const uint32_t p = pos[i], v = val[i];
-                if (v <= bound && in_range(p)) {
-                    uint32_t lim = NONE;
-#pragma unroll
-                    for (int t = 1; t <= VMAX; ++t) if (v == (uint32_t)t) lim = before[t];
-                    const unsigned long long key = ((unsigned long long)p << 8) | v;
-                    if (p < lim && (h == 0 || key > last) && key < cur) cur = key;
-                }
-            }
-        }
+        list_trips<B, false>(pos, val, n, (const RowBatch<B> *)nullptr, [&](const uint32_t i, const uint32_t p, const uint32_t v) {
+            if (i < n && v <= bound && in_range(p)) {
+                uint32_t lim = NONE;
+#pragma unroll
+                for (int t = 1; t <= VMAX; ++t) if (v == (uint32_t)t) lim = before[t];
+                const unsigned long long key = ((unsigned long long)p << 8) | v;
+                if (p < lim && (h == 0 || key > last) && key < cur) cur = key;
+            }
+        });
         for (int o = 32; o > 0; o >>= 1) {
             const unsigned long long x = ((unsigned long long)(uint32_t)__shfl_xor((int)(cur >> 32), o) << 32) | (uint32_t)__shfl_xor((int)(uint32_t)cur, o);
             cur = x < cur ? x : cur;
@@ -1310,13 +1349,12 @@
 }
 
 template <class W>
-__device__ __attribute__((noinline)) void lv_cigar(const uint32_t *ref, W &w, LvTables *tabp, int strand, uint32_t L, uint32_t pos, int k)
-{
-    LvTables &tab = *tabp;
+__device__ __forceinline__ void lv_cigar_here(const uint32_t *ref, W &w, const LvTabRef tab, int strand, uint32_t L, uint32_t pos, int k)
+{
     lv_unpack(ref, w, strand, L, pos);
-    int d_fin = 0;
     WSYNC();
-    int e = lv_wave(w.u.lvb.T, (int)L + 4, w.u.lvb.P, (int)L, k, &tab, d_fin);
+    const LvEnd fin = lv_wave(w.u.lvb.T, (int)L + 4, w.u.lvb.P, (int)L, k, tab);
+    const int e = fin.e, d_fin = fin.d_fin;
     __threadfence_block();
     WSYNC();
     if (lane_id() == 0) {
@@ -1324,17 +1362,18 @@
         uint16_t *cg = w.cig;
         if (e == 0) { cg[n++] = (uint16_t)((L << 4) | 0u); }
         else if (e > 0) {
-            char act[LVK + 1]; int matched[LVK + 1];
+            LvTrace &tr = *reinterpret_cast<LvTrace *>(w.u.lvb.T);
+            char *act = tr.act; int *matched = tr.matched;
             int cd = d_fin;
             for (int ce = e; ce >= 1; --ce) {
-                char a = tab.A[ce][cd + 31];
+                char a = tab.A[ce * 64 + cd + 31];
                 act[ce] = a;
-                int cur = tab.L[ce][cd + 31];
-                if (a == 'I') { matched[ce] = cur - tab.L[ce - 1][cd + 1 + 31] - 1; cd += 1; }
-                else if (a == 'D') { matched[ce] = cur - tab.L[ce - 1][cd - 1 + 31]; cd -= 1; }
-                else { matched[ce] = cur - tab.L[ce - 1][cd + 31] - 1; }
-            }
-            int acc = tab.L[0][31];
+                int cur = tab.L[ce * 64 + cd + 31];
+                if (a == 'I') { matched[ce] = cur - tab.L[(ce - 1) * 64 + cd + 1 + 31] - 1; cd += 1; }
+                else if (a == 'D') { matched[ce] = cur - tab.L[(ce - 1) * 64 + cd - 1 + 31]; cd -= 1; }
+                else { matched[ce] = cur - tab.L[(ce - 1) * 64 + cd + 31] - 1; }
+            }
+            int acc = tab.L[31];
             int ce = 1;
             while (ce <= e) {
                 char a = act[ce]; int cnt = 1;
@@ -1353,6 +1392,11 @@
         w.n_cig = n;
     }
     WSYNC();
+}
+template <class W>
+__device__ __attribute__((noinline)) void lv_cigar(const uint32_t *ref, W &w, const LvTabRef tab, int strand, uint32_t L, uint32_t pos, int k)
+{
+    lv_cigar_here(ref, w, tab, strand, L, pos, k);
 }
 
 __device__ __forceinline__ void lane_text(const uint32_t *__restrict__ ref, uint32_t *T, uint32_t pos, uint32_t tl)
@@ -1575,8 +1619,7 @@
                 if (lanes_ok) { const uint32_t ev = cand_e[i]; e = (ev != 255 && (int)ev <= maxd) ? (int)ev : -1; }
                 else if (!(pos > ix.ref_len || pos + L + 4 > ix.ref_len)) {
                     lv_unpack(ix.ref, w, strand, L, pos);
-                    int dd;
-                    e = lv_wave(w.u.lvb.T, (int)L + 4, w.u.lvb.P, (int)L, maxd, nullptr, dd);
+                    e = lv_wave(w.u.lvb.T, (int)L + 4, w.u.lvb.P, (int)L, maxd, LvTabRef{ nullptr, nullptr }).e;
                     WSYNC();
                 }
                 ++c_lv;
@@ -1632,7 +1675,7 @@
     }
     if (q_pos != 0xFFFFFFFFu) {
         if (q_gap) {
-            lv_cigar(ix.ref, w, lvtab, (int)q_strand, L, q_pos, (int)q_ndiff);
+            lv_cigar(ix.ref, w, lv_tab(lvtab), (int)q_strand, L, q_pos, (int)q_ndiff);
             if (lane < (uint32_t)w.n_cig) out->cigar[lane] = w.cig[lane];
             if (lane == 0) out->n_cigar = (uint8_t)w.n_cig;
         } else if (lane == 0) { out->cigar[0] = (uint16_t)((L << 4) | 0u); out->n_cigar = 1; }
@@ -1643,7 +1686,7 @@
             uint32_t h = sel_idx[s][j];
             if (w.hit_gap[s][h]) {
                 WSYNC();
-                lv_cigar(ix.ref, w, lvtab, s, L, w.hit_pos[s][h], (int)w.hit_nd[s][h]);
+                lv_cigar(ix.ref, w, lv_tab(lvtab), s, L, w.hit_pos[s][h], (int)w.hit_nd[s][h]);
                 if (lane < (uint32_t)w.n_cig) out->hit_cigar[hidx][lane] = w.cig[lane];
                 if (lane == 0) out->hit_n_cigar[hidx] = (uint8_t)w.n_cig;
             } else if (lane == 0) out->hit_n_cigar[hidx] = 0;
@@ -1680,6 +1723,24 @@
             if (k < hi - lo) return lo + k;
         }
         seg = (seg + 1u) & (QUEUE_RANGES - 1u); ++tried;
+    }
+    return 0xFFFFFFFFu;
+}
+__device__ __forceinline__ uint32_t pop_ranged_wave(QueueRange *ranges, const uint32_t which, const uint32_t n_items, uint32_t &seg, uint64_t &live)
+{
+    static_assert(QUEUE_RANGES == 64, "a range a lane");
+    const uint32_t lane = lane_id();
+    const uint32_t my_size = (uint32_t)((uint64_t)n_items * (lane + 1u) / QUEUE_RANGES) - (uint32_t)((uint64_t)n_items * lane / QUEUE_RANGES);
+    while (live) {
+        const uint64_t rot = seg ? (live >> seg) | (live << (64u - seg)) : live;
+        const uint32_t s = (seg + (uint32_t)__builtin_ctzll(rot)) & (QUEUE_RANGES - 1u);
+        const uint32_t lo = (uint32_t)((uint64_t)n_items * s / QUEUE_RANGES), hi = (uint32_t)((uint64_t)n_items * (s + 1u) / QUEUE_RANGES);
+        uint32_t k = 0;
+        if (lane == 0) k = atomicAdd(&ranges[s].heads[which], 1u);
+        k = (uint32_t)__builtin_amdgcn_readfirstlane((int)k);
+        seg = s;
+        if (k < hi - lo) return lo + k;
+        live = __ballot(__hip_atomic_load(&ranges[lane].heads[which], __ATOMIC_RELAXED, __HIP_MEMORY_SCOPE_AGENT) < my_size);
     }
     return 0xFFFFFFFFu;
 }
@@ -1778,36 +1839,43 @@
 }
 
 struct FinLds { uint32_t hit_pos[2][NHIT]; uint8_t hit_nd[2][NHIT]; };
-__global__ void __launch_bounds__(64)
+__global__ void __launch_bounds__(64) __attribute__((amdgpu_waves_per_eu(4, 4)))
 k_gapfin(IndexView ix, AlignParams ap, const uint32_t *__restrict__ pm, salt_result_t *__restrict__ results, GapBufs g,
          unsigned long long *__restrict__ ctr)
 {
     __shared__ FinLds w;
-    __shared__ uint32_t s_item;
     const uint32_t lane = lane_id();
-    const uint64_t lt = (1ull << lane) - 1ull;
     const uint32_t n_items = g.gctl->gap_slots < g.cap ? g.gctl->gap_slots : g.cap;
-    uint32_t seg = blockIdx.x & (QUEUE_RANGES - 1u), tried = 0;
+    uint32_t seg = blockIdx.x & (QUEUE_RANGES - 1u);
+    uint64_t live = ~0ull;
     for (;;) {
-        if (threadIdx.x == 0) s_item = pop_ranged(g.ranges, QueueRange::GAPFIN, n_items, seg, tried);
-        WSYNC();
-        const uint32_t slot = s_item;
-        WSYNC();
+        const uint32_t slot = pop_ranged_wave(g.ranges, QueueRange::GAPFIN, n_items, seg, live);
         if (slot == 0xFFFFFFFFu) break;
         const uint64_t rt0 = ctr ? __builtin_amdgcn_s_memrealtime() : 0;
-        const uint32_t r = g.gq[slot];
+        auto uni = [](uint32_t x) -> uint32_t { return (uint32_t)__builtin_amdgcn_readfirstlane((int)x); };
+        const uint32_t r_v = g.gq[slot];
+        const uint2 n2 = *reinterpret_cast<const uint2 *>(g.gn + 2 * slot), off2 = *reinterpret_cast<const uint2 *>(g.goff + 2 * slot);
+        const uint32_t r = uni(r_v);
         if (r == 0xFFFFFFFFu) continue;
-        const uint32_t L = pm[(uint64_t)r * ap.pg.pm_stride + 2 * ap.pg.nw8];
+        const uint32_t L_v = pm[(uint64_t)r * ap.pg.pm_stride + 2 * ap.pg.nw8];
+        const uint32_t n_s[2] = { uni(n2.x), uni(n2.y) };
+        const size_t row_s[2] = { uni(off2.x), uni(off2.y) };
+        RowBatch<GAPFIN_B> first[2];
+#pragma unroll
+        for (int strand = 0; strand < 2; ++strand)
+            if (n_s[strand]) rows_fetch<GAPFIN_B>(first[strand], g.gloci + row_s[strand], g.ge + row_s[strand], n_s[strand], 0u);
+        const uint32_t L = uni(L_v);
         salt_result_t *out = results + r;
         uint32_t q_pos = 0xFFFFFFFFu, q_strand = 3, q_ndiff = 255, q_gap = 255;
         uint32_t bound = ap.pe ? 3u : L / 10;
         uint32_t n_hits_s[2] = { 0, 0 }, a0[2] = { 0, 0 };
+#pragma unroll
         for (int strand = 0; strand < 2; ++strand) {
-            const uint32_t n = g.gn[2 * slot + strand];
-            const size_t row = g.goff[2 * slot + strand];
+            const uint32_t n = n_s[strand];
+            const size_t row = row_s[strand];
             bool any = false; uint32_t bp = 0, bv = 0;
-            rule_unsorted<LLV_K, true>(g.gloci + row, g.ge + row, n, L, ix.ref_len, bound, any, bp, bv, n_hits_s[strand], a0[strand],
-                                       w.hit_pos[strand], w.hit_nd[strand]);
+            rule_unsorted<LLV_K, true, GAPFIN_B>(g.gloci + row, g.ge + row, n, L, ix.ref_len, bound, any, bp, bv, n_hits_s[strand], a0[strand],
+                                                 w.hit_pos[strand], w.hit_nd[strand], &first[strand]);
             if (any) { q_pos = bp; q_ndiff = bv; q_gap = 1; q_strand = (uint32_t)strand; }
         }
         WSYNC();
@@ -1859,6 +1927,7 @@
         LvTables *__restrict__ lvtab)
 {
     __shared__ WaveLdsCigar w;
+    __shared__ LvTablesLds tl;
     __shared__ uint32_t s_item;
     const uint32_t lane = lane_id();
     const uint32_t n_items = *count < cap_items ? *count : cap_items;
@@ -1884,7 +1953,7 @@
         }
         for (uint32_t t = lane; t < (L + 7) >> 3; t += 64) w.pm[strand][t] = rec[strand * ap.pg.nw8 + t];
         WSYNC();
-        lv_cigar(ix.ref, w, lvtab + blockIdx.x, (int)strand, L, pos, (int)k);
+        lv_cigar_here(ix.ref, w, k <= (uint32_t)LLV_K ? lv_tab(tl) : lv_tab(lvtab + blockIdx.x), (int)strand, L, pos, (int)k);
         uint16_t *dst = which == 0 ? out->cigar : out->hit_cigar[which - 1];
         if (lane < (uint32_t)w.n_cig) dst[lane] = w.cig[lane];
         if (lane == 0) { if (which == 0) out->n_cigar = (uint8_t)w.n_cig; else out->hit_n_cigar[which - 1] = (uint8_t)w.n_cig; }
@@ -2310,6 +2379,11 @@
     else if (mode == 1) rule_sparse<3, false>(pos + o, val + o, n, L, ref_len, bound, any, bp, bv, nh, a0, hit_pos, hit_nd);
     else if (mode == 3) rule_sparse<3, false, 32>(pos + o, val + o, n, L, ref_len, bound, any, bp, bv, nh, a0, hit_pos, hit_nd);
     else if (mode == 4) rule_sparse<3, false, 16>(pos + o, val + o, n, L, ref_len, bound, any, bp, bv, nh, a0, hit_pos, hit_nd);
+    else if (mode == 5) {
+        RowBatch<GAPFIN_B> first;
+        if (n) rows_fetch<GAPFIN_B>(first, pos + o, val + o, n, 0u);
+        rule_unsorted<LLV_K, true, GAPFIN_B>(pos + o, val + o, n, L, ref_len, bound, any, bp, bv, nh, a0, hit_pos, hit_nd, &first);
+    }
     else rule_unsorted<LLV_K, true>(pos + o, val + o, n, L, ref_len, bound, any, bp, bv, nh, a0, hit_pos, hit_nd);
     WSYNC();
     uint32_t *w = out + (size_t)c * (6 + 2 * NHIT);
@@ -2332,9 +2406,10 @@
 k_diag_lv(IndexView ix, uint32_t n_cases, const uint32_t *__restrict__ pos, const uint32_t *__restrict__ kdiff,
           const uint8_t *__restrict__ seqs, const uint32_t *__restrict__ offs, const uint32_t *__restrict__ lane_first,
           const uint32_t *__restrict__ lane_n, const uint32_t *__restrict__ lane_case, int32_t *__restrict__ out ,
-          uint16_t *__restrict__ cig_out , LvTables *__restrict__ lvtab)
+          uint16_t *__restrict__ cig_out , LvTables *__restrict__ lvtab, int lds_tab)
 {
     __shared__ WaveLds w;
+    __shared__ LvTablesLds tl;
     __shared__ uint32_t lane_pm[LLV_N][LLV_PW];
     const uint32_t c = blockIdx.x, lane = lane_id();
     if (c >= n_cases) return;
@@ -2356,8 +2431,7 @@
     const int k = (int)kdiff[c];
     if (in_range) {
         lv_unpack(ix.ref, w, 0, L, p);
-        int dd;
-        e_wave = lv_wave(w.u.lvb.T, (int)L + 4, w.u.lvb.P, (int)L, k, nullptr, dd);
+        e_wave = lv_wave(w.u.lvb.T, (int)L + 4, w.u.lvb.P, (int)L, k, LvTabRef{ nullptr, nullptr }).e;
         WSYNC();
     }
     const bool fit = lv_fit_dev(L, (uint32_t)k);
@@ -2373,7 +2447,7 @@
         WSYNC();
     }
     if (in_range && e_wave >= 0 && e_wave < LVK) {
-        lv_cigar(ix.ref, w, lvtab + blockIdx.x, 0, L, p, e_wave);
+        lv_cigar(ix.ref, w, lds_tab && e_wave <= LLV_K ? lv_tab(tl) : lv_tab(lvtab + blockIdx.x), 0, L, p, e_wave);
         n_cig = w.n_cig;
         if (lane < (uint32_t)w.n_cig) cig_out[(size_t)c * SALT_MAX_CIGAR_OPS + lane] = w.cig[lane];
     }
@@ -2387,10 +2461,10 @@
 
 void launch_diag_lv(const IndexView &ix, uint32_t n, const uint32_t *pos, const uint32_t *kdiff, const uint8_t *seqs,
                     const uint32_t *offs, const uint32_t *lane_first, const uint32_t *lane_n, const uint32_t *lane_case,
-                    int32_t *out, uint16_t *cig, void *lvtab, hipStream_t st)
+                    int32_t *out, uint16_t *cig, void *lvtab, int lds_tab, hipStream_t st)
 {
     if (n) hipLaunchKernelGGL(k_diag_lv, dim3(n), dim3(64), 0, st, ix, n, pos, kdiff, seqs, offs, lane_first, lane_n, lane_case, out, cig,
-                              static_cast<LvTables *>(lvtab));
+                              static_cast<LvTables *>(lvtab), lds_tab);
 }
 
 __global__ void __launch_bounds__(64)
@@ -2462,9 +2536,9 @@
             s.T[i] = tv;
         }
         WSYNC();
-        int d_fin = 0;
         LvTables *tab = want_cigar ? tabs + blockIdx.x : nullptr;
-        const int e = lv_wave(s.T, (int)tl, s.P, (int)L, (int)x.k, tab, d_fin);
+        const LvEnd fin = lv_wave(s.T, (int)tl, s.P, (int)L, (int)x.k, lv_tab(tab));
+        const int e = fin.e, d_fin = fin.d_fin;
         if (lane == 0) dist[it] = e;
         if (want_cigar) {
             __threadfence_block();
@@ -2545,7 +2619,7 @@
 
 void launch_heavy(const IndexView &ix, const AlignParams &ap, const uint32_t *pm, const uint4 *sai_c,
                   const uint4 *sai_r, salt_result_t *results, const uint32_t *queue, unsigned long long *ctr,
-                  uint32_t n_blocks, uint32_t gap_blocks, void *lvtab, const GapBufs &g_in, uint32_t *ovq, QueueRange *ranges, uint8_t *pe_scr, hipEvent_t *ev3, hipStream_t st)
+                  uint32_t n_blocks, uint32_t gap_blocks, uint32_t cigar_blocks, void *lvtab, const GapBufs &g_in, uint32_t *ovq, QueueRange *ranges, uint8_t *pe_scr, hipEvent_t *ev3, hipStream_t st)
 {
     if (!ap.n_reads) { if (ev3) for (int i = 0; i < 3; ++i) hipEventRecord(ev3[i], st); return; }
     uint32_t blocks = n_blocks < ap.n_reads ? n_blocks : ap.n_reads;
@@ -2567,11 +2641,12 @@
     else     hipLaunchKernelGGL(k_heavy_big, dim3(big_blocks), dim3(64), 0, st, ix, ap, pm, sai_c, sai_r, results, queue, ctr, tab, g, pe_scr, small ? 1 : 0);
     if (ev3) hipEventRecord(ev3[0], st);
     if (!g.cap) { if (ev3) { hipEventRecord(ev3[1], st); hipEventRecord(ev3[2], st); } return; }
+    if (cigar_blocks == 0 || cigar_blocks > n_blocks) cigar_blocks = n_blocks;
     hipLaunchKernelGGL(k_gap, dim3(gap_blocks), dim3(64), 0, st, ix, ap, pm, g);
     if (ev3) hipEventRecord(ev3[1], st);
     hipLaunchKernelGGL(k_gapfin, dim3((n_blocks + 3) / 4), dim3(64), 0, st, ix, ap, pm, results, g, ctr);
     if (ev3) hipEventRecord(ev3[2], st);
-    hipLaunchKernelGGL(k_cigar, dim3((n_blocks + 1) / 2), dim3(64), 0, st, ix, ap.pg, pm, results, g.cq, &g.gctl->cigar_items, &g.gctl->cigar_head, g.cap * (1u + SALT_MAX_HITS), tab);
+    hipLaunchKernelGGL(k_cigar, dim3(cigar_blocks), dim3(64), 0, st, ix, ap.pg, pm, results, g.cq, &g.gctl->cigar_items, &g.gctl->cigar_head, g.cap * (1u + SALT_MAX_HITS), tab);
 }
 
 GapBufs gap_bufs_layout(uint8_t *base, uint32_t cap, SeCtl *gctl, size_t *bytes)
diff --git a/salt_amd/csrc/salt_gpu.hip b/salt_amd/csrc/salt_gpu.hip
--- a/salt_amd/csrc/salt_gpu.hip
+++ b/salt_amd/csrc/salt_gpu.hip
@@ -98,7 +98,7 @@
     DevBuf<uint8_t> d_text; uint64_t text_bytes = 0;
     std::vector<unsigned long long> h_zoff; std::vector<uint32_t> h_zstat;
     uint32_t text_calls = 0;
-    uint32_t heavy_blocks = 2048, gap_blocks = 2048;
+    uint32_t heavy_blocks = 2048, gap_blocks = 2048, cigar_blocks = 2048;
     QueueRange *d_ranges = nullptr;
     DevBuf<uint8_t> d_zero;
     int all_heavy = 0;
@@ -373,6 +373,8 @@
         uint32_t gap_per_cu = 16;
         if (const char *e2 = getenv("SALT_GPU_GAP_PER_CU")) { int v = atoi(e2); if (v > 0 && v <= 16) gap_per_cu = (uint32_t)v; }
         ws->gap_blocks = (uint32_t)prop.multiProcessorCount * gap_per_cu;
+        ws->cigar_blocks = ws->heavy_blocks;
+        if (const char *e2 = getenv("SALT_GPU_CIGAR_BLOCKS")) { int v = atoi(e2); if (v > 0 && (uint32_t)v < ws->heavy_blocks) ws->cigar_blocks = (uint32_t)v; }
         ws->walk_blocks = (uint32_t)prop.multiProcessorCount * 2u;
         if (const char *e2 = getenv("SALT_GPU_WALK_PER_CU")) { int v = atoi(e2); if (v > 0 && v <= 16) ws->walk_blocks = (uint32_t)prop.multiProcessorCount * (uint32_t)v; }
         if (const char *e2 = getenv("SALT_GPU_SAI_EPOCH")) { const long long v = atoll(e2); if (v >= 1 && v <= (long long)SAI_EPOCH_MAX) ws->epoch = (uint32_t)v; }
@@ -541,7 +543,7 @@
                      static_cast<salt_result_t *>(d_results), ws->d_queue, ws->d_qctl, ws->d_queue + 2 * (size_t)ws->max_reads, ws->d_ranges, ctr, st);
     if (timed) HIPCHK(hipEventRecord(ev[3], st));
     launch_heavy(ws->ix->view, ap, ws->d_pm, ws->d_sai_c, ws->d_sai_r,
-                 static_cast<salt_result_t *>(d_results), ws->d_queue, ctr, ws->heavy_blocks, ws->gap_blocks, ws->d_lvtab,
+                 static_cast<salt_result_t *>(d_results), ws->d_queue, ctr, ws->heavy_blocks, ws->gap_blocks, ws->cigar_blocks, ws->d_lvtab,
                  gap_bufs_layout(ws->d_gap, ws->gcap, ws->d_qctl, nullptr), ws->d_queue + ws->max_reads, ws->d_ranges, glob_loci ? ws->d_pe_scr.p : nullptr, timed ? ev + 4 : nullptr, st);
     if (timed) { HIPCHK(hipEventRecord(ev[7], st)); ws->ev_pe[ws->n_timed] = 0; ++ws->n_timed; }
     HIPCHK(hipGetLastError());
@@ -1396,6 +1398,12 @@
                                 const uint32_t *kdiff, const uint8_t *seqs, const uint32_t *offs, int32_t *out4,
                                 uint16_t *cigars)
 {
+    return salt_gpu_diag_lv_tab(ref_words, ref_len, n_cases, pos, kdiff, seqs, offs, out4, cigars, 0);
+}
+extern "C" int salt_gpu_diag_lv_tab(const uint32_t *ref_words, uint32_t ref_len, uint32_t n_cases, const uint32_t *pos,
+                                    const uint32_t *kdiff, const uint8_t *seqs, const uint32_t *offs, int32_t *out4,
+                                    uint16_t *cigars, int lds_tab)
+{
     if (!ref_words || !pos || !kdiff || !seqs || !offs || !out4 || !cigars) return fail(SALT_E_INVAL, "null argument");
     int n_dev = 0;
     HIPCHK(hipGetDeviceCount(&n_dev));
@@ -1438,7 +1446,7 @@
     HIPCHK(hipMalloc((void **)&d_lf, lane_first.size() * 4)); HIPCHK(hipMemcpy(d_lf, lane_first.data(), lane_first.size() * 4, hipMemcpyHostToDevice));
     HIPCHK(hipMalloc((void **)&d_ln, lane_n.size() * 4)); HIPCHK(hipMemcpy(d_ln, lane_n.data(), lane_n.size() * 4, hipMemcpyHostToDevice));
     HIPCHK(hipMalloc((void **)&d_lc, lane_case.size() * 4)); HIPCHK(hipMemcpy(d_lc, lane_case.data(), lane_case.size() * 4, hipMemcpyHostToDevice));
-    launch_diag_lv(v, n_cases, d_pos, d_k, d_seqs, d_offs, d_lf, d_ln, d_lc, d_out, d_cig, d_tab, nullptr);
+    launch_diag_lv(v, n_cases, d_pos, d_k, d_seqs, d_offs, d_lf, d_ln, d_lc, d_out, d_cig, d_tab, lds_tab, nullptr);
     HIPCHK(hipGetLastError());
     HIPCHK(hipDeviceSynchronize());
     HIPCHK(hipMemcpy(out4, d_out, (uint64_t)n_cases * 16, hipMemcpyDeviceToHost));
diff --git a/salt_amd/csrc/salt_kernels.h b/salt_amd/csrc/salt_kernels.h
--- a/salt_amd/csrc/salt_kernels.h
+++ b/salt_amd/csrc/salt_kernels.h
@@ -96,7 +96,7 @@
 GapBufs gap_bufs_layout(uint8_t *base, uint32_t cap, SeCtl *gctl, size_t *bytes);
 void launch_heavy(const IndexView &ix, const AlignParams &ap, const uint32_t *pm, const uint4 *sai_c,
                   const uint4 *sai_r, salt_result_t *results, const uint32_t *queue, unsigned long long *ctr,
-                  uint32_t n_blocks, uint32_t gap_blocks, void *lvtab, const GapBufs &g, uint32_t *ovq, QueueRange *ranges, uint8_t *pe_scr, hipEvent_t *ev3, hipStream_t st);
+                  uint32_t n_blocks, uint32_t gap_blocks, uint32_t cigar_blocks, void *lvtab, const GapBufs &g, uint32_t *ovq, QueueRange *ranges, uint8_t *pe_scr, hipEvent_t *ev3, hipStream_t st);
 size_t lv_table_bytes();
 
 static const uint32_t SW_MAX_SEG = 64;
@@ -143,7 +143,7 @@
                         const uint32_t *coffs, int mode, uint8_t *out, hipStream_t st);
 void launch_diag_lv(const IndexView &ix, uint32_t n, const uint32_t *pos, const uint32_t *kdiff, const uint8_t *seqs,
                     const uint32_t *offs, const uint32_t *lane_first, const uint32_t *lane_n, const uint32_t *lane_case,
-                    int32_t *out, uint16_t *cig, void *lvtab, hipStream_t st);
+                    int32_t *out, uint16_t *cig, void *lvtab, int lds_tab, hipStream_t st);
 bool lv_lanes_fit(uint32_t L, uint32_t k);
 
 struct FqRec { uint32_t name_off, name_len, seq_off, len, qual_off; };
```

After: 565.6 Mreads/s, median of 6. 1.01x the previous value.
